# EloDoyard/movie-recommender-system

Hardware: AMD Instinct MI355X
Metric: test-set predictions/sec (kNN k=300, fit+predict+MAE) (higher is better)
Workload: dtype fp16 MFMA similarity filter (fp32 acc) + f64 exact re-rank/prediction

## Files before the change

### movie-recommender-system_amd/csrc/api.cpp

```cpp
#include <math.h>
#include <stdio.h>
#include <string.h>

#include <algorithm>
#include <vector>

#include "engine.h"

using namespace knncf;

namespace knncf {
void launch_first_rows(int64_t n, const int32_t* d_du, const int32_t* d_di, int32_t own_lo, int32_t own_hi,
                       uint32_t* d_first, hipStream_t st);
void launch_length_keys(int32_t count, const int32_t* d_list, const int64_t* d_u_ptr, int32_t max_len, uint64_t* d_key, hipStream_t st);
void launch_collect_new(int32_t U, const uint32_t* d_first, int64_t* d_seq, int64_t epoch, int32_t own_lo, int32_t own_hi,
                        int32_t* d_list, int32_t* d_count, hipStream_t st);
void launch_fallback_keys(int32_t U, const double* d_exact, uint64_t* d_keys, uint32_t* d_vals, hipStream_t st);
void launch_fallback_write(int32_t user, int32_t take, int32_t kcap, const uint32_t* d_sorted_vals,
                           const double* d_exact, int32_t* nbr_idx, double* nbr_sim, int32_t* nbr_cnt,
                           hipStream_t st);
void launch_jaccard_pair(const Train& tr, int32_t u, int32_t v, double* d_out, hipStream_t st);
}

struct StageTimer {
    hipEvent_t a, b;
    double* acc;
};

struct knncf_handle {
    knncf_config cfg{};
    hipStream_t stream = nullptr;
    std::string err;
    Train tr;
    PrepScratch prep;
    bool fitted = false, committed = false;
    int8_t short_rows = -1;
    NeighborTable nt;
    int64_t epoch = 1;
    int64_t U_pad = 0, K_pad = 0;
    DArr<bf16_t> Bpanel;
    bool b_ready = false;
    int32_t head = 0;
    double tail_pairs_full = 0.0;
    DArr<int32_t> colmap;
    DArr<int32_t> te_cnt, te_item;
    DArr<float> te_x, row_tail_abs, row_head_sq;
    DArr<float> row_len;
    hipStream_t stream2 = nullptr;
    DArr<bf16_t> Apanel[2];
    DArr<float> S[2];
    DArr<float> S_full;
    DArr<uint32_t> sym_tiles;
    DArr<int32_t> redo_rows;
    int32_t sym_tiles_n = 0;
    hipEvent_t ev_produced[2] = {nullptr, nullptr}, ev_consumed[2] = {nullptr, nullptr}, ev_ready = nullptr;
    int32_t* pinned_cnt = nullptr;
    size_t pinned_cap = 0;
    SelectScratch sel;
    SliceScratch slices;
    NeighborTable pt;
    bool pt_ready = false;
    PersonalRows prow;
    bool prow_ready = false;
    DArr<int32_t> reco_users, reco_items, reco_out_items;
    DArr<double> reco_pred, reco_out_preds;
    DArr<uint8_t> reco_rated;
    QueryBatchScratch query_batch;
    RecoBatchScratch reco_batch;
    DArr<int32_t> build_list, build_count;
    DArr<uint32_t> first_row;
    DArr<int32_t> t_du, t_di, t_users, t_items;
    DArr<double> t_pred, t_err, t_ratings, t_partial, scalar_out;
    DArr<unsigned long long> scalar_u64;
    DArr<uint8_t> t_owned;
    DArr<int64_t> t_counts;
    DArr<int32_t> sweep_ks;
    std::vector<uint32_t> h_ukeys, h_ikeys;
    std::vector<int32_t> h_uid;
    std::vector<int64_t> h_uptr;
    knncf_timings tm{};
    std::vector<StageTimer> pending;
    std::vector<hipEvent_t> event_pool;
};

namespace {

hipEvent_t get_event(knncf_handle* h) {
    if (!h->event_pool.empty()) {
        hipEvent_t e = h->event_pool.back();
        h->event_pool.pop_back();
        return e;
    }
    hipEvent_t e;
    KN_HIP(hipEventCreate(&e));
    return e;
}

struct Stage {
    knncf_handle* h;
    StageTimer t;
    hipStream_t st;
    Stage(knncf_handle* h_, double* acc, hipStream_t st_ = nullptr) : h(h_), st(st_ ? st_ : h_->stream) {
        t.a = get_event(h);
        t.b = get_event(h);
        t.acc = acc;
        (void)hipEventRecord(t.a, st);
    }
    ~Stage() {
        (void)hipEventRecord(t.b, st);
        h->pending.push_back(t);
    }
};

void resolve_timers(knncf_handle* h) {
    (void)hipStreamSynchronize(h->stream);
    (void)hipStreamSynchronize(h->stream2);
    for (auto& t : h->pending) {
        float ms = 0.f;
        if (hipEventElapsedTime(&ms, t.a, t.b) == hipSuccess) *t.acc += ms;
        h->event_pool.push_back(t.a);
        h->event_pool.push_back(t.b);
    }
    h->pending.clear();
}

template <class F>
int guarded(knncf_handle* h, F&& f) {
    if (!h) return KNNCF_E_INVALID;
    struct DeviceGuard {
        int prev = -1;
        ~DeviceGuard() { if (prev >= 0) (void)hipSetDevice(prev); }
    } guard;
    try {
        int cur = -1;
        if (hipGetDevice(&cur) != hipSuccess) {
            (void)hipGetLastError();
            KN_HIP(hipSetDevice(h->cfg.device));
        } else if (cur != h->cfg.device) {
            guard.prev = cur;
            KN_HIP(hipSetDevice(h->cfg.device));
        }
        f();
        resolve_timers(h);
        return KNNCF_OK;
    } catch (const Error& e) {
        h->err = e.what();
        (void)hipStreamSynchronize(h->stream);
        (void)hipStreamSynchronize(h->stream2);
        (void)hipGetLastError();
        h->pending.clear();
        return e.status;
    } catch (const std::bad_alloc&) {
        h->err = "host allocation failed";
        return KNNCF_E_NOMEM;
    } catch (const std::exception& e) {
        h->err = e.what();
        return KNNCF_E_INVALID;
    }
}

void require_fitted(knncf_handle* h, bool committed = true) {
    KN_REQUIRE(h->fitted, KNNCF_E_STATE, "call knncf_fit first");
    if (committed) KN_REQUIRE(h->committed, KNNCF_E_STATE, "sharded handle: call knncf_shard_commit after the exchange");
}

void load_host_ids(knncf_handle* h) {
    if (!h->h_ukeys.empty() || h->tr.U == 0) return;
    Train& tr = h->tr;
    h->h_ukeys.resize(tr.U);
    h->h_ikeys.resize(tr.I);
    h->h_uid.resize(tr.U);
    KN_HIP(hipMemcpyAsync(h->h_ukeys.data(), tr.ukeys.p, tr.U * sizeof(uint32_t), hipMemcpyDeviceToHost, h->stream));
    KN_HIP(hipMemcpyAsync(h->h_ikeys.data(), tr.ikeys.p, tr.I * sizeof(uint32_t), hipMemcpyDeviceToHost, h->stream));
    KN_HIP(hipMemcpyAsync(h->h_uid.data(), tr.uid.p, tr.U * sizeof(int32_t), hipMemcpyDeviceToHost, h->stream));
    KN_HIP(hipStreamSynchronize(h->stream));
}

int32_t dense_user(knncf_handle* h, int32_t raw) {
    load_host_ids(h);
    return dense_lookup(h->h_ukeys.data(), h->tr.U, raw);
}
int64_t train_row_length(knncf_handle* h, int32_t du) {
    if (h->h_uptr.empty()) {
        h->h_uptr.resize((size_t)h->tr.U + 1);
        KN_HIP(hipMemcpyAsync(h->h_uptr.data(), h->tr.u_ptr.p, h->h_uptr.size() * sizeof(int64_t), hipMemcpyDeviceToHost, h->stream));
        KN_HIP(hipStreamSynchronize(h->stream));
    }
    return h->h_uptr[du + 1] - h->h_uptr[du];
}
int32_t dense_item(knncf_handle* h, int32_t raw) {
    load_host_ids(h);
    return dense_lookup(h->h_ikeys.data(), h->tr.I, raw);
}

void require_shard_numbering(knncf_handle* h) {
    if (h->cfg.shard_count == 1) return;
    if (h->short_rows < 0) {
        Train& tr = h->tr;
        std::vector<int64_t> ptr((size_t)tr.U + 1);
        KN_HIP(hipMemcpyAsync(ptr.data(), tr.u_ptr.p, ptr.size() * sizeof(int64_t), hipMemcpyDeviceToHost, h->stream));
        KN_HIP(hipStreamSynchronize(h->stream));
        h->short_rows = 0;
        for (int32_t u = 0; u < tr.U; ++u)
            if (ptr[u + 1] - ptr[u] <= 4) { h->short_rows = 1; break; }
    }
    KN_REQUIRE(h->short_rows == 0, KNNCF_E_UNSUPPORTED,
               "neighbours: on a shard handle whose train set has a user with <= 4 ratings, a neighbourhood that knncf_mae / "
               "knncf_predict_batch has not built yet cannot be built by a query (its build number would exist on this shard only)");
}

template <class T>
T fetch(knncf_handle* h, const T* d, int64_t idx) {
    T v;
    KN_HIP(hipMemcpyAsync(&v, d + idx, sizeof(T), hipMemcpyDeviceToHost, h->stream));
    KN_HIP(hipStreamSynchronize(h->stream));
    return v;
}

void reset_neighbors(knncf_handle* h) {
    Train& tr = h->tr;
    NeighborTable& nt = h->nt;
    nt.k = h->cfg.k;
    nt.kcap = std::max(0, std::min(nt.k, tr.U - 1));
    size_t cells = (size_t)tr.U * (size_t)std::max(nt.kcap, 1);
    nt.idx.ensure(cells);
    nt.sim.ensure(cells);
    nt.by_id_valid = false;
    nt.cnt.ensure(tr.U);
    nt.seq.ensure(tr.U);
    KN_HIP(hipMemsetAsync(nt.cnt.p, 0, tr.U * sizeof(int32_t), h->stream));
    KN_HIP(hipMemsetAsync(nt.seq.p, 0xff, tr.U * sizeof(int64_t), h->stream));
    h->epoch = 1;
}

float gemm_eps_operand(bool fp16) {
    const double u = ldexp(1.0, fp16 ? -11 : -8) * 1.001;
    return (float)(2 * u + u * u);
}
float gemm_eps_rest(bool fp16) {
    return (float)(4e-7 + (fp16 ? 6e-6 : 0.0) + 8e-6);
}

int32_t shortlist_cap(int32_t k, int32_t U) {
    int64_t want = std::max<int64_t>(16384, 4 * (int64_t)k);
    int64_t cap = 64;
    while (cap < want) cap <<= 1;
    int64_t upper = 64;
    while (upper < U) upper <<= 1;
    return (int32_t)std::min(cap, upper);
}

int32_t choose_head(knncf_handle* h, int32_t rows_total, bool symmetric) {
    Train& tr = h->tr;
    const int32_t I = tr.I;
    const std::vector<int64_t>& c = tr.pop_count;
    std::vector<double> tail_sq((size_t)I + 1, 0.0);
    for (int32_t j = I - 1; j >= 0; --j) tail_sq[j] = tail_sq[j + 1] + (double)c[j] * (double)c[j];
    int32_t H;
    if (h->cfg.head_items == KNNCF_HEAD_ALL) {
        H = I;
    } else if (h->cfg.head_items > 0) {
        H = (int32_t)std::min<int64_t>(h->cfg.head_items, I);
    } else {
        const double RATE_DENSE = symmetric ? 2.8e15 : 1.2e15;
        const double RATE_SPARSE = 2.3e12;
        const double frac = (double)rows_total / (double)tr.U;
        const double U_pad = (double)round_up(tr.U, 256);
        double best = 1e300;
        H = I;
        for (int64_t cand = 64;; cand += 64) {
            int32_t hc = (int32_t)std::min<int64_t>(cand, I);
            double cost = 2.0 * rows_total * U_pad * (double)round_up(hc, 64) / RATE_DENSE + tail_sq[hc] * frac / RATE_SPARSE;
            if (cost < best) { best = cost; H = hc; }
            if (hc == I) break;
        }
        if (tr.jaccard && (h->cfg.flags & KNNCF_FLAG_F32_PANEL) == 0) H = std::min(H, 2048);
    }
    h->tail_pairs_full = tail_sq[H];
    return H;
}

void build_neighbors(knncf_handle* h, int32_t count) {
    Train& tr = h->tr;
    NeighborTable& nt = h->nt;
    if (count <= 0 || nt.kcap <= 0) return;
    KN_REQUIRE(h->cfg.similarity != KNNCF_SIM_ONE, KNNCF_E_UNSUPPORTED,
               "kNN neighbourhoods with similarityOne: every similarity is 1.0, the neighbourhood is the first k users in Set order — not built");
    hipStream_t st = h->stream;
    if (count > 256) {
        PrepScratch& sc = h->prep;
        sc.k64_a.ensure(count); sc.k64_b.ensure(count); sc.v32_b.ensure(count);
        launch_length_keys(count, h->build_list.p, tr.u_ptr.p, tr.I, sc.k64_a.p, st);
        sort_pairs_u64_u32(sc.sort, sc.k64_a.p, sc.k64_b.p, reinterpret_cast<const uint32_t*>(h->build_list.p), sc.v32_b.p, count, bits_for((uint64_t)tr.I), st);
        KN_HIP(hipMemcpyAsync(h->build_list.p, sc.v32_b.p, (size_t)count * sizeof(int32_t), hipMemcpyDeviceToDevice, st));
    }
    const bool fp16 = (h->cfg.flags & KNNCF_FLAG_BF16_FILTER) == 0;
    const bool s_fp16 = (h->cfg.flags & KNNCF_FLAG_F32_PANEL) == 0;
    h->U_pad = round_up(tr.U, 256);
    const int64_t U_pad = h->U_pad;
    size_t free_b = 0, total_b = 0;
    KN_HIP(hipMemGetInfo(&free_b, &total_b));
    const int64_t s_elem = s_fp16 ? 2 : 4;
    const size_t sym_bytes = (size_t)U_pad * (size_t)U_pad * (size_t)s_elem;
    size_t own = h->S_full.bytes() + h->sel.cand_idx.bytes() + h->sel.cand_approx.bytes() + h->sel.grp_v0.bytes() + h->sel.grp_x.bytes();
    for (int s = 0; s < 2; ++s) own += h->S[s].bytes() + h->Apanel[s].bytes();
    bool use_sym = h->cfg.shard_count == 1 && (int64_t)count * 2 >= tr.U && U_pad / 256 < 65536 &&
                   sym_bytes <= (free_b + own) / 3 && !getenv("KNNCF_DEBUG_NO_SYMMETRIC_GEMM");
    if (use_sym) {
        try {
            h->S_full.ensure((sym_bytes + 3) / 4);
        } catch (const Error& e) {
            if (e.status != KNNCF_E_NOMEM) throw;
            (void)hipGetLastError();
            use_sym = false;
        }
    }
    if (!h->b_ready) {
        h->head = choose_head(h, count, use_sym);
        h->K_pad = round_up(h->head, 64);
        size_t need = (size_t)U_pad * h->K_pad * sizeof(bf16_t);
        KN_REQUIRE(need < free_b + h->Bpanel.bytes(), KNNCF_E_UNSUPPORTED,
                   "dense bf16 user panel does not fit in HBM; lower head_items");
        Stage s(h, &h->tm.densify_ms);
        h->colmap.ensure(tr.I);
        launch_colmap(tr, h->head, h->colmap.p, st);
        h->Bpanel.ensure((size_t)U_pad * h->K_pad);
        launch_densify(tr, nullptr, 0, tr.U, h->colmap.p, h->Bpanel.p, h->K_pad, U_pad, fp16, st);
        if (tr.jaccard) {
            KN_REQUIRE(!s_fp16 || h->head <= 2048, KNNCF_E_UNSUPPORTED, "Jaccard: more than 2048 dense head items need KNNCF_FLAG_F32_PANEL");
            h->row_len.ensure((size_t)row_len_size(tr.U));
            launch_row_len(tr, h->row_len.p, st);
        }
        if (h->head < tr.I) {
            h->te_cnt.ensure(tr.U); h->te_item.ensure(tr.n); h->te_x.ensure(tr.n);
            h->row_tail_abs.ensure(tr.U); h->row_head_sq.ensure(tr.U);
            launch_tail_entries(tr, h->colmap.p, h->te_cnt.p, h->te_item.p, h->te_x.p, h->row_tail_abs.p, h->row_head_sq.p, st);
        }
        h->b_ready = true;
        KN_HIP(hipMemGetInfo(&free_b, &total_b));
    }
    const int64_t K_pad = h->K_pad;
    const int32_t head = h->head;
    h->tm.head_items = head;
    if (use_sym) {
        const int32_t n_tiles = (int32_t)(U_pad / 256);
        if (h->sym_tiles_n != n_tiles) {
            std::vector<uint32_t> list;
            gemm_sym_tile_list(n_tiles, list);
            h->sym_tiles.ensure(list.size());
            KN_HIP(hipMemcpyAsync(h->sym_tiles.p, list.data(), list.size() * sizeof(uint32_t), hipMemcpyHostToDevice, st));
            KN_HIP(hipStreamSynchronize(st));
            h->sym_tiles_n = n_tiles;
        }
        const int64_t n_listed = (int64_t)n_tiles * (n_tiles + 1) / 2;
        Stage s(h, &h->tm.gemm_ms);
        launch_gemm_sym(h->Bpanel.p, h->S_full.p, s_fp16, U_pad, h->K_pad, h->K_pad, U_pad, fp16, !tr.jaccard, h->sym_tiles.p, n_listed, st);
        h->tm.gemm_launches += 1;
        h->tm.gemm_flops_executed += 2.0 * 256.0 * 256.0 * (double)n_listed * (double)h->K_pad;
        h->tm.gemm_flops_algorithmic += 2.0 * (double)count * (double)(tr.U - 1) * (double)h->head;
        KN_HIP(hipMemGetInfo(&free_b, &total_b));
    } else {
        h->S_full.release();
    }
    size_t held = 0;
    for (int s = 0; s < 2; ++s) held += h->S[s].bytes() + h->Apanel[s].bytes();
    held += h->sel.cand_idx.bytes() + h->sel.cand_approx.bytes() + h->sel.grp_v0.bytes() + h->sel.grp_x.bytes();
    int64_t budget = h->cfg.workspace_bytes > 0 ? h->cfg.workspace_bytes / 2
                                                : (int64_t)std::min<size_t>((size_t)48 << 30, (free_b + held) / 4);
    int64_t per_row = (use_sym ? 0 : U_pad * s_elem + K_pad * 2) + (int64_t)shortlist_cap(nt.k, tr.U) * 8 + (int64_t)select_gcap(nt.k) * 36;
    if (h->cfg.workspace_bytes <= 0) {
        const int64_t whole = round_up(count, 256) * per_row;
        if (whole <= (int64_t)std::min<size_t>((size_t)96 << 30, (free_b + held) / 3)) budget = std::max(budget, whole);
    }
    int64_t R = std::max<int64_t>(256, (budget / per_row) / 256 * 256);
    R = std::min<int64_t>(R, round_up(count, 256));
    const int64_t n_blocks = ceil_div(count, R);
    R = round_up(ceil_div(count, n_blocks), 256);
    const bool overlap = (h->cfg.flags & KNNCF_FLAG_OVERLAP) != 0;
    const int slots = (overlap && n_blocks > 1 && !use_sym) ? 2 : 1;
    for (int s = 0; s < slots && !use_sym; ++s) {
        h->S[s].ensure((size_t)(R * U_pad * s_elem + 3) / 4);
        h->Apanel[s].ensure((size_t)R * K_pad);
    }
    const int32_t cap = shortlist_cap(nt.k, tr.U);
    const bool verify = (h->cfg.flags & KNNCF_FLAG_VERIFY_BOUND) != 0;
    h->sel.cand_idx.ensure((size_t)R * cap);
    h->sel.cand_approx.ensure((size_t)R * cap);
    h->sel.cand_cnt.ensure(R);
    h->sel.cand_eps.ensure(R);
    h->sel.row_entries.ensure(R);
    h->sel.grp_v0.ensure((size_t)R * select_gcap(nt.k));
    h->sel.grp_x.ensure((size_t)R * select_gcap(nt.k) * 8);
    h->sel.stats.ensure(4);
    KN_HIP(hipMemsetAsync(h->sel.stats.p, 0, 4 * sizeof(double), st));
    if (h->pinned_cap < (size_t)count) {
        if (h->pinned_cnt) KN_HIP(hipHostFree(h->pinned_cnt));
        h->pinned_cnt = nullptr;
        h->pinned_cap = 0;
        KN_HIP(hipHostMalloc((void**)&h->pinned_cnt, (size_t)count * sizeof(int32_t), hipHostMallocDefault));
        h->pinned_cap = (size_t)count;
    }
    const float eps_opnd = gemm_eps_operand(fp16);
    const float eps_rest = gemm_eps_rest(fp16) + (s_fp16 ? 2.45e-4f : 0.f);
    hipStream_t sp = slots > 1 ? h->stream2 : h->stream;
    hipStream_t sc = h->stream;
    KN_HIP(hipEventRecord(h->ev_ready, sc));
    KN_HIP(hipStreamWaitEvent(sp, h->ev_ready, 0));
    std::vector<int32_t> h_rows;
    auto need_h_rows = [&] {
        if (!h_rows.empty()) return;
        h_rows.resize(count);
        KN_HIP(hipMemcpyAsync(h_rows.data(), h->build_list.p, (size_t)count * sizeof(int32_t), hipMemcpyDeviceToHost, st));
        KN_HIP(hipStreamSynchronize(st));
    };
    auto redo_marked = [&](const std::vector<int32_t>& marked, const void* Sp, bool by_user, int64_t rb) {
        need_h_rows();
        std::vector<int32_t> users(marked.size()), srow(marked.size());
        for (size_t j = 0; j < marked.size(); ++j) {
            users[j] = h_rows[marked[j]];
            srow[j] = (int32_t)(marked[j] - rb);
        }
        TailEntries te{h->te_cnt.p, h->te_item.p, h->te_x.p, h->row_tail_abs.p, h->row_head_sq.p, h->row_len.p};
        const int64_t chunk = std::min<int64_t>((int64_t)marked.size(), R);
        h->redo_rows.ensure(2 * (size_t)chunk);
        for (size_t j0 = 0; j0 < marked.size(); j0 += (size_t)R) {
            const int32_t m = (int32_t)std::min<size_t>((size_t)R, marked.size() - j0);
            KN_HIP(hipMemcpyAsync(h->redo_rows.p, users.data() + j0, (size_t)m * sizeof(int32_t), hipMemcpyHostToDevice, st));
            KN_HIP(hipMemcpyAsync(h->redo_rows.p + chunk, srow.data() + j0, (size_t)m * sizeof(int32_t), hipMemcpyHostToDevice, st));
            {
                Stage s(h, &h->tm.select_ms);
                launch_tail_select(tr, h->colmap.p, te, head < tr.I, Sp, by_user, s_fp16, U_pad, m, h->redo_rows.p, nt.k, eps_opnd, eps_rest, cap,
                                   h->sel.cand_idx.p, h->sel.cand_approx.p, h->sel.cand_cnt.p, h->sel.cand_eps.p, h->sel.grp_v0.p, h->sel.grp_x.p,
                                   select_gcap(nt.k), st, false, by_user ? nullptr : h->redo_rows.p + chunk);
                h->tm.select_launches += 1;
            }
            {
                Stage s(h, &h->tm.rerank_ms);
                launch_rerank(tr, nt, m, h->redo_rows.p, cap, h->sel.cand_idx.p, h->sel.cand_approx.p, h->sel.cand_cnt.p, h->sel.cand_eps.p,
                              h->sel.stats.p, h->sel.row_entries.p, verify, st);
            }
            std::vector<int32_t> again(m);
            KN_HIP(hipMemcpyAsync(again.data(), h->sel.cand_cnt.p, (size_t)m * sizeof(int32_t), hipMemcpyDeviceToHost, st));
            KN_HIP(hipStreamSynchronize(st));
            for (int32_t j = 0; j < m; ++j) h->pinned_cnt[marked[j0 + j]] = again[j];
        }
    };
    const bool per_block_redo = !use_sym && n_blocks > 1;
    for (int64_t b = 0; b < n_blocks; ++b) {
        const int64_t rb = b * R;
        const int32_t rows = (int32_t)std::min<int64_t>(R, count - rb);
        const int64_t M = round_up(rows, 256);
        const int32_t* d_rows = h->build_list.p + rb;
        const int slot = (int)(b % slots);
        if (b >= slots) KN_HIP(hipStreamWaitEvent(sp, h->ev_consumed[slot], 0));
        if (!use_sym) {
            Stage s(h, &h->tm.densify_ms, sp);
            launch_densify(tr, d_rows, 0, rows, h->colmap.p, h->Apanel[slot].p, K_pad, M, fp16, sp);
        }
        if (!use_sym) {
            Stage s(h, &h->tm.gemm_ms, sp);
            launch_gemm_nt(h->Apanel[slot].p, h->Bpanel.p, h->S[slot].p, s_fp16, M, U_pad, K_pad, K_pad, K_pad, U_pad, fp16, !tr.jaccard, sp);
            h->tm.gemm_launches += 1;
            h->tm.gemm_flops_executed += 2.0 * (double)M * (double)U_pad * (double)K_pad;
            h->tm.gemm_flops_algorithmic += 2.0 * (double)rows * (double)(tr.U - 1) * (double)head;
        }
        KN_HIP(hipEventRecord(h->ev_produced[slot], sp));
        KN_HIP(hipStreamWaitEvent(sc, h->ev_produced[slot], 0));
        TailEntries te{h->te_cnt.p, h->te_item.p, h->te_x.p, h->row_tail_abs.p, h->row_head_sq.p, h->row_len.p};
        h->prep.join_commit(sc);
        const void* Sblk = use_sym ? (const void*)h->S_full.p : (const void*)h->S[slot].p;
        const int32_t gcap = select_gcap(nt.k);
        auto select_rows = [&](int32_t r0, int32_t nr) {
            Stage s(h, &h->tm.select_ms, sc);
            const void* Sp = use_sym ? Sblk : (const void*)(static_cast<const char*>(Sblk) + (size_t)r0 * (size_t)U_pad * (size_t)s_elem);
            launch_tail_select(tr, h->colmap.p, te, head < tr.I, Sp, use_sym, s_fp16, U_pad, nr, d_rows + r0, nt.k, eps_opnd, eps_rest, cap,
                               h->sel.cand_idx.p + (size_t)r0 * cap, h->sel.cand_approx.p + (size_t)r0 * cap, h->sel.cand_cnt.p + r0, h->sel.cand_eps.p + r0,
                               h->sel.grp_v0.p + (size_t)r0 * gcap, h->sel.grp_x.p + (size_t)r0 * gcap * 8, gcap, sc);
            h->tm.select_launches += 1;
            h->tm.tail_pair_updates += h->tail_pairs_full * ((double)nr / (double)tr.U);
            h->tm.select_row_bytes += (double)s_elem * (double)nr * (double)tr.U;
        };
        const int32_t slices = std::min<int32_t>(8, 8192 / std::max<int32_t>(nt.kcap, 1));
        const char* force_slices = getenv("KNNCF_DEBUG_SLICE_ROWS");
        const int32_t n_heavy = slices < 2                         ? 0
                                : force_slices                     ? std::max<int32_t>(0, std::min<int32_t>(rows, atoi(force_slices)))
                                : (rows >= 4096 && rows <= 65536)  ? std::max<int32_t>(16, rows / 512)
                                                                   : 0;
        select_rows(0, rows);
        if (overlap && !per_block_redo) KN_HIP(hipEventRecord(h->ev_consumed[slot], sc));
        {
            Stage s(h, &h->tm.rerank_ms, sc);
            launch_rerank(tr, nt, rows, d_rows, cap, h->sel.cand_idx.p, h->sel.cand_approx.p, h->sel.cand_cnt.p, h->sel.cand_eps.p, h->sel.stats.p,
                          h->sel.row_entries.p, verify, sc, n_heavy, slices, &h->slices);
        }
        if (!overlap) KN_HIP(hipEventRecord(h->ev_consumed[slot], sc));
        if (per_block_redo) KN_HIP(hipMemcpyAsync(h->pinned_cnt + rb, h->sel.cand_cnt.p, rows * sizeof(int32_t), hipMemcpyDeviceToHost, sc));
        if (per_block_redo) {
            KN_HIP(hipStreamSynchronize(sc));
            std::vector<int32_t> marked;
            for (int64_t r = rb; r < rb + rows; ++r)
                if (h->pinned_cnt[r] > cap) marked.push_back((int32_t)r);
            if ((int64_t)marked.size() > std::max<int64_t>(64, rows / 200)) {
                redo_marked(marked, h->S[slot].p, false, rb);
            }
            if (overlap) KN_HIP(hipEventRecord(h->ev_consumed[slot], sc));
        }
    }
    const bool summary = !per_block_redo;
    unsigned long long four[4] = {0, 0, 0, 0};
    nt.by_id_valid = false;
    if (summary) KN_HIP(hipMemcpyAsync(four, h->sel.stats.p, sizeof(four), hipMemcpyDeviceToHost, sc));
    KN_HIP(hipStreamSynchronize(sc));
    KN_HIP(hipStreamSynchronize(sp));
    auto take_stats = [&](const unsigned long long* w) {
        h->tm.rerank_row_bytes += 12.0 * (double)w[1];
        if (verify && w[0] != 0) {
            double shifted;
            memcpy(&shifted, &w[0], sizeof(double));
            h->tm.max_bound_violation = std::max(h->tm.max_bound_violation, shifted - 4.0);
        }
    };
    if (summary && four[3] == 0) {
        h->tm.shortlist_total += (double)four[2];
        take_stats(four);
        return;
    }
    if (summary) {
        KN_HIP(hipMemcpyAsync(h->pinned_cnt, h->sel.cand_cnt.p, (size_t)count * sizeof(int32_t), hipMemcpyDeviceToHost, st));
        KN_HIP(hipStreamSynchronize(st));
    }
    if (summary) {
        std::vector<int32_t> marked;
        for (int64_t r = 0; r < count; ++r)
            if (h->pinned_cnt[r] > cap) marked.push_back((int32_t)r);
        if ((int64_t)marked.size() > std::max<int64_t>(64, count / 200)) redo_marked(marked, use_sym ? (const void*)h->S_full.p : (const void*)h->S[0].p, use_sym, 0);
    }
    for (int64_t r = 0; r < count; ++r) {
        h->tm.shortlist_total += std::min(h->pinned_cnt[r], cap);
        if (h->pinned_cnt[r] > cap) {
            need_h_rows();
            Stage s(h, &h->tm.rerank_ms);
            int32_t u = h_rows[r];
            h->sel.row_exact.ensure(tr.U);
            h->sel.fb_keys_a.ensure(tr.U); h->sel.fb_keys_b.ensure(tr.U);
            h->sel.fb_vals_a.ensure(tr.U); h->sel.fb_vals_b.ensure(tr.U);
            int64_t seq_u = fetch(h, nt.seq.p, u);
            launch_exact_row(tr, nt, u, seq_u, h->sel.row_exact.p, st);
            launch_fallback_keys(tr.U, h->sel.row_exact.p, h->sel.fb_keys_a.p, h->sel.fb_vals_a.p, st);
            sort_pairs_u64_u32(h->prep.sort, h->sel.fb_keys_a.p, h->sel.fb_keys_b.p, h->sel.fb_vals_a.p,
                               h->sel.fb_vals_b.p, tr.U, 64, st);
            launch_fallback_write(u, nt.kcap, nt.kcap, h->sel.fb_vals_b.p, h->sel.row_exact.p, nt.idx.p, nt.sim.p,
                                  nt.cnt.p, st);
            h->tm.fallback_rows += 1;
        }
    }
    {
        unsigned long long two[2] = {0, 0};
        KN_HIP(hipMemcpyAsync(two, h->sel.stats.p, sizeof(two), hipMemcpyDeviceToHost, st));
        KN_HIP(hipStreamSynchronize(st));
        take_stats(two);
    }
}

void ensure_test_scratch(knncf_handle* h, int64_t n) {
    h->t_du.ensure(n); h->t_di.ensure(n); h->t_pred.ensure(n); h->t_err.ensure(n); h->t_owned.ensure(n);
    h->t_partial.ensure(1024); h->t_counts.ensure(1024);
}

void ensure_neighbors_for_rows(knncf_handle* h, int64_t n) {
    Train& tr = h->tr;
    if (tr.U < 2 || h->nt.kcap <= 0) return;
    KN_REQUIRE(n < (int64_t)0xffffffffll, KNNCF_E_UNSUPPORTED, "more than 2^32-1 test rows");
    hipStream_t st = h->stream;
    h->first_row.ensure(tr.U);
    h->build_list.ensure(tr.U);
    h->build_count.ensure(1);
    KN_HIP(hipMemsetAsync(h->first_row.p, 0xff, tr.U * sizeof(uint32_t), st));
    KN_HIP(hipMemsetAsync(h->build_count.p, 0, sizeof(int32_t), st));
    launch_first_rows(n, h->t_du.p, h->t_di.p, 0, tr.U, h->first_row.p, st);
    launch_collect_new(tr.U, h->first_row.p, h->nt.seq.p, h->epoch, tr.own_lo, tr.own_hi, h->build_list.p, h->build_count.p, st);
    h->epoch += 1;
    int32_t count = fetch(h, h->build_count.p, 0);
    build_neighbors(h, count);
}

bool personalized_streams(const knncf_handle* h) { return h->tr.U > 2048 || getenv("KNNCF_DEBUG_PERSONALIZED_STREAM"); }

void require_personalized(knncf_handle* h) {
    Train& tr = h->tr;
    KN_REQUIRE(h->cfg.shard_count == 1, KNNCF_E_UNSUPPORTED, "PERSONALIZED is not sharded");
    if (h->cfg.similarity == KNNCF_SIM_COSINE) {
        std::vector<int64_t> ptr((size_t)tr.U + 1);
        KN_HIP(hipMemcpyAsync(ptr.data(), tr.u_ptr.p, ptr.size() * sizeof(int64_t), hipMemcpyDeviceToHost, h->stream));
        KN_HIP(hipStreamSynchronize(h->stream));
        for (int32_t u = 0; u < tr.U; ++u)
            KN_REQUIRE(ptr[u + 1] - ptr[u] > 4, KNNCF_E_UNSUPPORTED,
                       "PERSONALIZED with the adjusted cosine: a user with <= 4 ratings makes the reference's summation order depend on its memo history pair by pair (SURVEY N6); not modelled");
    }
}

void ensure_personalized_table(knncf_handle* h) {
    if (h->pt_ready) return;
    Train& tr = h->tr;
    require_personalized(h);
    NeighborTable& pt = h->pt;
    pt.k = pt.kcap = tr.U;
    const size_t cells = (size_t)tr.U * (size_t)tr.U;
    pt.uidx.ensure(cells);
    pt.usim.ensure(cells);
    pt.cnt.ensure(tr.U);
    launch_full_rows(tr, h->cfg.similarity == KNNCF_SIM_JACCARD, pt.uidx.p, pt.usim.p, pt.cnt.p, h->stream);
    pt.by_id_valid = true;
    h->pt_ready = true;
}

void ensure_personal_rows(knncf_handle* h) {
    if (h->prow_ready) return;
    require_personalized(h);
    Stage s(h, &h->tm.prep_ms);
    h->prep.join_commit(h->stream);
    personalized_prepare(h->tr, h->prep, h->prow, h->stream);
    h->prow_ready = true;
}

void predict_personal_rows(knncf_handle* h, const double* d_ratings, int64_t n, double* d_pred) {
    Train& tr = h->tr;
    PersonalRows& pr = h->prow;
    PrepScratch& sc = h->prep;
    hipStream_t st = h->stream;
    KN_REQUIRE(n < (int64_t)0xffffffffll, KNNCF_E_UNSUPPORTED, "more than 2^32-1 test rows");
    sc.k64_a.ensure(n); sc.k64_b.ensure(n); sc.v32_a.ensure(n); sc.v32_b.ensure(n);
    const int ibits = bits_for((uint64_t)tr.I);
    std::vector<uint64_t> keys((size_t)n);
    {
        Stage s(h, &h->tm.predict_ms);
        launch_personal_row_keys(tr, n, h->t_du.p, h->t_di.p, sc.k64_a.p, sc.v32_a.p, st);
        sort_pairs_u64_u32(sc.sort, sc.k64_a.p, sc.k64_b.p, sc.v32_a.p, sc.v32_b.p, n, ibits + bits_for((uint64_t)tr.U), st);
        KN_HIP(hipMemcpyAsync(keys.data(), sc.k64_b.p, (size_t)n * sizeof(uint64_t), hipMemcpyDeviceToHost, st));
        KN_HIP(hipStreamSynchronize(st));
    }
    std::vector<int32_t> users;
    std::vector<int64_t> first_row;
    for (int64_t r = 0; r < n; ++r) {
        const uint64_t u = keys[r] >> ibits, i = keys[r] & ((1ull << ibits) - 1ull);
        if (u < (uint64_t)tr.U && i < (uint64_t)tr.I && (users.empty() || users.back() != (int32_t)u)) {
            users.push_back((int32_t)u);
            first_row.push_back(r);
        }
    }
    const int64_t nu = (int64_t)users.size();
    int64_t R = 1;
    if (nu > 0) {
        size_t free_b = 0, total_b = 0;
        KN_HIP(hipMemGetInfo(&free_b, &total_b));
        const int64_t row_bytes = (int64_t)tr.U * 8;
        const int64_t budget = h->cfg.workspace_bytes > 0 ? h->cfg.workspace_bytes / 2
                                                          : (int64_t)std::min<size_t>((size_t)48 << 30, (free_b + pr.S.bytes()) / 4);
        R = std::min<int64_t>(std::max<int64_t>(1, budget / row_bytes), nu);
        R = ceil_div(nu, ceil_div(nu, R));
        pr.S.ensure((size_t)R * tr.U);
        std::vector<int32_t> slot((size_t)tr.U, -1);
        for (int64_t k = 0; k < nu; ++k) slot[users[k]] = (int32_t)(k % R);
        pr.users.ensure(nu);
        pr.slot.ensure(tr.U);
        KN_HIP(hipMemcpyAsync(pr.users.p, users.data(), (size_t)nu * sizeof(int32_t), hipMemcpyHostToDevice, st));
        KN_HIP(hipMemcpyAsync(pr.slot.p, slot.data(), (size_t)tr.U * sizeof(int32_t), hipMemcpyHostToDevice, st));
        KN_HIP(hipStreamSynchronize(st));
    }
    const int64_t n_blocks = std::max<int64_t>(1, ceil_div(nu, R));
    for (int64_t b = 0; b < n_blocks; ++b) {
        const int64_t u0 = b * R, u1 = std::min<int64_t>(nu, u0 + R);
        const int64_t r0 = b == 0 ? 0 : first_row[u0], r1 = b + 1 < n_blocks ? first_row[u1] : n;
        if (u1 > u0) {
            Stage s(h, &h->tm.rerank_ms);
            launch_sim_rows(tr, pr, pr.users.p + u0, (int32_t)(u1 - u0), pr.S.p, st);
        }
        Stage s(h, &h->tm.predict_ms);
        launch_fold_rows(tr, pr, r1 - r0, sc.v32_b.p + r0, h->t_du.p, h->t_di.p, d_ratings, pr.slot.p, pr.S.p, d_pred, h->t_err.p,
                         h->t_owned.p, st);
    }
}

void ensure_item_stats(knncf_handle* h) {
    if (h->tr.item_stats_ready) return;
    Stage s(h, &h->tm.prep_ms);
    h->prep.join_commit(h->stream);
    prep_item_stats(h->tr, h->prep, h->stream);
}

int64_t order_test_rows(knncf_handle* h, int64_t n, bool by_item, int32_t cols) {
    Train& tr = h->tr;
    hipStream_t st = h->stream;
    PrepScratch& sc = h->prep;
    sc.k64_a.ensure(n); sc.k64_b.ensure(n); sc.v32_a.ensure(n); sc.v32_b.ensure(n);
    const uint32_t key_limit = (uint32_t)(by_item ? tr.I : tr.U);
    if (h->cfg.shard_count > 1) {
        h->scalar_u64.ensure(1);
        KN_HIP(hipMemsetAsync(h->scalar_u64.p, 0, sizeof(unsigned long long), st));
        KN_HIP(hipMemsetAsync(h->t_err.p, 0, (size_t)cols * (size_t)n * sizeof(double), st));
        KN_HIP(hipMemsetAsync(h->t_owned.p, 0, (size_t)n, st));
        launch_owned_keys(n, by_item ? h->t_di.p : h->t_du.p, h->t_du.p, tr.own_lo, tr.own_hi, h->cfg.shard_rank == 0, key_limit,
                          sc.k64_a.p, sc.v32_a.p, h->scalar_u64.p, st);
        sort_pairs_u64_u32(sc.sort, sc.k64_a.p, sc.k64_b.p, sc.v32_a.p, sc.v32_b.p, n, bits_for((uint64_t)key_limit + 1), st);
        return (int64_t)fetch(h, h->scalar_u64.p, 0);
    }
    launch_user_keys(n, by_item ? h->t_di.p : h->t_du.p, key_limit, sc.k64_a.p, sc.v32_a.p, st);
    sort_pairs_u64_u32(sc.sort, sc.k64_a.p, sc.k64_b.p, sc.v32_a.p, sc.v32_b.p, n, bits_for((uint64_t)key_limit), st);
    return n;
}

void reduce_errors(knncf_handle* h, int64_t n, int32_t cols, double* sums, int64_t* count) {
    hipStream_t st = h->stream;
    const int32_t nb = 1024;
    h->t_partial.ensure((size_t)nb * cols);
    h->t_counts.ensure((size_t)nb * cols);
    for (int32_t c = 0; c < cols; ++c)
        launch_reduce_err(h->t_err.p + (size_t)c * n, h->t_owned.p, n, h->t_partial.p + (size_t)c * nb, h->t_counts.p + (size_t)c * nb, nb, st);
    std::vector<double> hp((size_t)nb * cols);
    std::vector<int64_t> hc((size_t)nb * cols);
    KN_HIP(hipMemcpyAsync(hp.data(), h->t_partial.p, hp.size() * sizeof(double), hipMemcpyDeviceToHost, st));
    KN_HIP(hipMemcpyAsync(hc.data(), h->t_counts.p, hc.size() * sizeof(int64_t), hipMemcpyDeviceToHost, st));
    KN_HIP(hipStreamSynchronize(st));
    for (int32_t c = 0; c < cols; ++c) {
        double s_ = 0.0;
        int64_t c_ = 0;
        for (int32_t b = 0; b < nb; ++b) { s_ += hp[(size_t)c * nb + b]; c_ += hc[(size_t)c * nb + b]; }
        if (sums) sums[c] = s_;
        if (count && c == 0) *count = c_;
    }
}

void run_predict(knncf_handle* h, int predictor, const int32_t* d_users, const int32_t* d_items,
                 const double* d_ratings, int64_t n, double* sum_abs_err, int64_t* count, double* d_pred_out) {
    require_fitted(h);
    Train& tr = h->tr;
    hipStream_t st = h->stream;
    KN_REQUIRE(n >= 0, KNNCF_E_INVALID, "negative row count");
    if (sum_abs_err) *sum_abs_err = 0.0;
    if (count) *count = 0;
    if (n == 0) return;
    KN_REQUIRE(d_users && d_items, KNNCF_E_INVALID, "null test arrays");
    int kind = predictor;
    NeighborTable* table = &h->nt;
    bool stream = false;
    if (predictor == KNNCF_PRED_PERSONALIZED) {
        if (h->cfg.similarity == KNNCF_SIM_ONE) {
            kind = KNNCF_PRED_BASELINE_RDD;
        } else if (personalized_streams(h)) {
            ensure_personal_rows(h);
            stream = true;
        } else {
            ensure_personalized_table(h);
            kind = KNNCF_PRED_KNN;
            table = &h->pt;
        }
    }
    KN_REQUIRE(stream || (kind >= KNNCF_PRED_GLOBAL_AVG && kind <= KNNCF_PRED_KNN), KNNCF_E_INVALID, "unknown predictor");
    if (kind == KNNCF_PRED_ITEM_AVG || kind == KNNCF_PRED_BASELINE || kind == KNNCF_PRED_BASELINE_RDD) ensure_item_stats(h);
    ensure_test_scratch(h, n);
    {
        Stage s(h, &h->tm.predict_ms);
        launch_dense_ids(tr, d_users, d_items, n, h->t_du.p, h->t_di.p, st);
    }
    if (kind == KNNCF_PRED_KNN && table == &h->nt) ensure_neighbors_for_rows(h, n);
    h->prep.join_commit(st);
    double* pred = d_pred_out ? d_pred_out : h->t_pred.p;
    if (stream) predict_personal_rows(h, d_ratings, n, pred);
    {
        Stage s(h, &h->tm.predict_ms);
        const uint32_t* d_order = nullptr;
        const bool by_item = tr.ib_words > 0 && lds_bitmap_fits(tr.ib_words);
        int64_t n_rows = n;
        if (kind == KNNCF_PRED_KNN) {
            n_rows = order_test_rows(h, n, by_item, 1);
            d_order = h->prep.v32_b.p;
        }
        if (n_rows > 0 && !stream)
            launch_predict(tr, table, kind, n_rows, h->t_du.p, h->t_di.p, d_ratings, d_order, by_item, pred, h->t_err.p, h->t_owned.p,
                           h->cfg.shard_rank == 0, st);
        if (sum_abs_err || count) reduce_errors(h, n, 1, sum_abs_err, count);
    }
}

void check_sweep_ks(const int32_t* ks, int32_t n_k) {
    KN_REQUIRE(ks && n_k >= 1 && n_k <= 64, KNNCF_E_INVALID, "sweep: 1 .. 64 values of k");
    for (int32_t q = 0; q < n_k; ++q)
        KN_REQUIRE(ks[q] >= 1 && ks[q] <= 2048 && (q == 0 || ks[q] > ks[q - 1]), KNNCF_E_INVALID,
                   "sweep: k must be strictly ascending in [1, 2048]");
}

void run_mae_sweep(knncf_handle* h, const int32_t* ks, int32_t n_k, const int32_t* d_users, const int32_t* d_items,
                   const double* d_ratings, int64_t n, double* sums, int64_t* count, double* d_pred) {
    check_sweep_ks(ks, n_k);
    require_fitted(h);
    KN_REQUIRE(h->cfg.similarity != KNNCF_SIM_ONE, KNNCF_E_UNSUPPORTED,
               "kNN neighbourhoods with similarityOne: every similarity is 1.0, the neighbourhood is the first k users in Set order — not built");
    KN_REQUIRE(n >= 0, KNNCF_E_INVALID, "negative row count");
    for (int32_t q = 0; q < n_k; ++q) sums[q] = 0.0;
    *count = 0;
    if (n == 0) return;
    KN_REQUIRE(d_users && d_items && d_ratings, KNNCF_E_INVALID, "null test arrays");
    Train& tr = h->tr;
    hipStream_t st = h->stream;
    struct Restore {
        knncf_handle* h;
        int32_t k;
        ~Restore() {
            h->cfg.k = k;
            try { reset_neighbors(h); } catch (const Error&) {}
        }
    } restore{h, h->cfg.k};
    h->cfg.k = ks[n_k - 1];
    reset_neighbors(h);
    ensure_test_scratch(h, n);
    h->t_err.ensure((size_t)n_k * n);
    {
        Stage s(h, &h->tm.predict_ms);
        launch_dense_ids(tr, d_users, d_items, n, h->t_du.p, h->t_di.p, st);
    }
    ensure_neighbors_for_rows(h, n);
    h->prep.join_commit(st);
    std::vector<int32_t> hk(ks, ks + n_k);
    h->sweep_ks.ensure(64);
    KN_HIP(hipMemcpyAsync(h->sweep_ks.p, hk.data(), (size_t)n_k * sizeof(int32_t), hipMemcpyHostToDevice, st));
    {
        Stage s(h, &h->tm.predict_ms);
        const int64_t n_rows = order_test_rows(h, n, true, n_k);
        if (n_rows > 0)
            launch_predict_sweep(tr, h->nt, h->sweep_ks.p, n_k, n_rows, n, h->t_du.p, h->t_di.p, d_ratings, h->prep.v32_b.p, d_pred,
                                 h->t_err.p, h->t_owned.p, h->cfg.shard_rank == 0, st);
        reduce_errors(h, n, n_k, sums, count);
    }
}

void do_fit_device(knncf_handle* h, const int32_t* d_users, const int32_t* d_items, const double* d_ratings, int64_t n) {
    KN_REQUIRE(n > 0 && d_users && d_items && d_ratings, KNNCF_E_INVALID, "fit: null or empty input");
    Train& tr = h->tr;
    hipStream_t st = h->stream;
    h->fitted = h->committed = false;
    h->short_rows = -1;
    h->b_ready = false;
    h->pt_ready = false;
    h->prow_ready = false;
    h->h_ukeys.clear(); h->h_ikeys.clear(); h->h_uid.clear(); h->h_uptr.clear();
    tr.n = n;
    tr.jaccard = h->cfg.similarity == KNNCF_SIM_JACCARD;
    {
        Stage s(h, &h->tm.prep_ms);
        if (tr.user_raw.p != d_users) {
            tr.user_raw.alloc(n); tr.item_raw.alloc(n); tr.rating.alloc(n);
            KN_HIP(hipMemcpyAsync(tr.user_raw.p, d_users, n * sizeof(int32_t), hipMemcpyDeviceToDevice, st));
            KN_HIP(hipMemcpyAsync(tr.item_raw.p, d_items, n * sizeof(int32_t), hipMemcpyDeviceToDevice, st));
            KN_HIP(hipMemcpyAsync(tr.rating.p, d_ratings, n * sizeof(double), hipMemcpyDeviceToDevice, st));
        }
        prep_fit(tr, h->prep, h->cfg.shard_rank, h->cfg.shard_count, st);
    }
    h->fitted = true;
    reset_neighbors(h);
    if (h->cfg.shard_count == 1) {
        Stage s(h, &h->tm.prep_ms);
        prep_commit(tr, h->prep, st);
        h->committed = true;
    }
}

void do_recommend(knncf_handle* h, int predictor, int32_t user, int32_t n, int32_t* out_items, double* out_preds, int32_t* count) {
    require_fitted(h);
    KN_REQUIRE(count && n >= 0 && (n == 0 || (out_items && out_preds)), KNNCF_E_INVALID, "bad arguments");
    *count = 0;
    Train& tr = h->tr;
    if (n == 0 || tr.I == 0) return;
    hipStream_t st = h->stream;
    const int32_t du = dense_user(h, user);
    KN_REQUIRE(du < 0 ? h->cfg.shard_rank == 0 : (du >= tr.own_lo && du < tr.own_hi), KNNCF_E_STATE,
               "recommend: the user belongs to another shard");
    const int32_t I = tr.I;
    h->reco_users.ensure(I); h->reco_items.ensure(I); h->reco_pred.ensure(I); h->reco_rated.ensure(I);
    launch_reco_rows(tr, user, du, h->reco_users.p, h->reco_items.p, h->reco_rated.p, st);
    run_predict(h, predictor, h->reco_users.p, h->reco_items.p, nullptr, I, nullptr, nullptr, h->reco_pred.p);
    PrepScratch& sc = h->prep;
    sc.k64_a.ensure(I); sc.k64_b.ensure(I); sc.v32_a.ensure(I); sc.v32_b.ensure(I);
    launch_reco_order(tr, sc.sort, h->reco_pred.p, h->reco_rated.p, sc.k64_a.p, sc.k64_b.p, sc.v32_a.p, sc.v32_b.p, st);
    int64_t n_rated = 0;
    if (du >= 0) {
        int64_t two[2];
        KN_HIP(hipMemcpyAsync(two, tr.u_ptr.p + du, 2 * sizeof(int64_t), hipMemcpyDeviceToHost, st));
        KN_HIP(hipStreamSynchronize(st));
        n_rated = two[1] - two[0];
    }
    const int32_t m = (int32_t)std::min<int64_t>(n, (int64_t)I - n_rated);
    if (m <= 0) return;
    h->reco_out_items.ensure(m); h->reco_out_preds.ensure(m);
    launch_reco_take(tr, m, sc.v32_b.p, h->reco_pred.p, h->reco_out_items.p, h->reco_out_preds.p, st);
    KN_HIP(hipMemcpyAsync(out_items, h->reco_out_items.p, (size_t)m * sizeof(int32_t), hipMemcpyDeviceToHost, st));
    KN_HIP(hipMemcpyAsync(out_preds, h->reco_out_preds.p, (size_t)m * sizeof(double), hipMemcpyDeviceToHost, st));
    KN_HIP(hipStreamSynchronize(st));
    *count = m;
}

constexpr int64_t QUERY_MAX_RATINGS = 65536;
enum QueryBatchMode { QB_NEIGHBORS, QB_PREDICT, QB_RECOMMEND };
enum QueryFamily { QF_FOLD_IN, QF_UPDATE, QF_REVISE };

void require_query_support(knncf_handle* h, int predictor) {
    KN_REQUIRE(predictor == KNNCF_PRED_KNN, KNNCF_E_UNSUPPORTED, "query: only KNNCF_PRED_KNN");
    KN_REQUIRE(h->cfg.similarity != KNNCF_SIM_ONE, KNNCF_E_UNSUPPORTED, "query: adjusted cosine or Jaccard");
    KN_REQUIRE(h->cfg.shard_count == 1, KNNCF_E_UNSUPPORTED, "query: single-shard handles only");
    KN_REQUIRE(h->tr.U >= 5, KNNCF_E_UNSUPPORTED, "query: fewer than 5 train users (the user set changes iteration class)");
}

int64_t query_batch_chunk(knncf_handle* h) {
    const Train& tr = h->tr;
    int64_t budget = h->cfg.workspace_bytes / 2;
    if (h->cfg.workspace_bytes <= 0) {
        size_t free_b = 0, total_b = 0;
        KN_HIP(hipMemGetInfo(&free_b, &total_b));
        budget = (int64_t)std::min<size_t>((size_t)48 << 30, free_b / 4);
    }
    int64_t C = std::min<int64_t>(QB_MAX_CHUNK, budget / query_batch_bytes(tr.U, tr.I));
    C = std::min<int64_t>(C, (int64_t)0x7fffffff / std::max(tr.U, tr.I));
    return std::max<int64_t>(C, 1);
}

struct QueryFailure {
    int64_t query = -1;
    const char* reason = "";
};

QueryFailure run_query_chunks(knncf_handle* h, QueryFamily family, QueryBatchMode mode, int64_t chunk, const int32_t* users,
                              const int64_t* removed_offsets, const int32_t* removed_items,
                              const int64_t* offsets, const int32_t* items, const double* ratings, int64_t B, int32_t width, const int64_t* pred_offsets,
                              const int32_t* pred_items, int32_t* out_i, double* out_d, int32_t* counts, int32_t* statuses) {
    h->prep.join_commit(h->stream);
    const Train& tr = h->tr;
    QueryBatchScratch& bs = h->query_batch;
    hipStream_t st = h->stream;
    const int32_t take = std::max(0, std::min(h->cfg.k, tr.U));
    QueryFailure first;
    auto fail = [&](int64_t b, int status, const char* why) {
        statuses[b] = status;
        if (counts) counts[b] = 0;
        if (first.query < 0 || b < first.query) first = {b, why};
    };
    const bool update = family != QF_FOLD_IN, revise = family == QF_REVISE;
    std::vector<int64_t> slot_query, qo, ao, ro, ebase;
    std::vector<int32_t> s_users, s_items, s_self, s_removed, h_idx, h_items, pick_slot, pick_items;
    std::vector<double> s_ratings, h_vals;
    std::vector<long long> info;
    for (int64_t c0 = 0; c0 < B; c0 += chunk) {
        const int64_t c1 = std::min(B, c0 + chunk);
        slot_query.clear(); s_users.clear(); s_items.clear(); s_ratings.clear(); s_self.clear(); s_removed.clear();
        qo.assign(1, 0);
        ao.assign(1, 0);
        ro.assign(1, 0);
        for (int64_t b = c0; b < c1; ++b) {
            const int64_t nb = offsets[b + 1] - offsets[b];
            const int64_t nr = revise ? removed_offsets[b + 1] - removed_offsets[b] : 0;
            const int32_t du = dense_user(h, users[b]);
            const int64_t seeded = nb + (update && du >= 0 ? train_row_length(h, du) : 0);
            if (nr > 0 && du < 0) { fail(b, KNNCF_E_INVALID, "a removed item for a user that is not in the training set"); continue; }
            if (nr > seeded - nb) { fail(b, KNNCF_E_INVALID, "more removed items than the user has train rows (one is not rated in train or listed twice)"); continue; }
            const int64_t rows = seeded - nr;
            if (rows <= 0) { fail(b, KNNCF_E_INVALID, nr > 0 ? "the removals leave the user without a row" : "null ratings or n_ratings <= 0"); continue; }
            if (seeded > QUERY_MAX_RATINGS) { fail(b, KNNCF_E_UNSUPPORTED, "more than 65536 ratings"); continue; }
            if (!update && du >= 0) { fail(b, KNNCF_E_INVALID, "the user occurs in the training set"); continue; }
            if (nr > 0) s_removed.insert(s_removed.end(), removed_items + removed_offsets[b], removed_items + removed_offsets[b + 1]);
            ro.push_back((int64_t)s_removed.size());
            slot_query.push_back(b);
            s_users.push_back(users[b]);
            s_self.push_back(du);
            s_items.insert(s_items.end(), items + offsets[b], items + offsets[b + 1]);
            s_ratings.insert(s_ratings.end(), ratings + offsets[b], ratings + offsets[b + 1]);
            ao.push_back((int64_t)s_items.size());
            qo.push_back(qo.back() + rows);
        }
        const int32_t C = (int32_t)slot_query.size();
        if (C == 0) continue;
        info.assign((size_t)4 * C, 0);
        foldin_batch_neighbors(tr, bs, h->prep.sort, C, s_users.data(), qo.data(), s_items.data(), s_ratings.data(),
                               update ? s_self.data() : nullptr, update ? ao.data() : nullptr, h->cfg.k, info.data(), st,
                               revise ? ro.data() : nullptr, revise ? s_removed.data() : nullptr);
        auto take_of = [&](int32_t s) { return update && s_self[s] >= 0 ? std::min(take, tr.U - 1) : take; };
        int32_t good = 0;
        for (int32_t s = 0; s < C; ++s) {
            const uint64_t bits = (uint64_t)info[4 * s];
            const int64_t b = slot_query[s];
            if (bits & QUERY_ST_RM_UNRATED) fail(b, KNNCF_E_INVALID, "a removed item that the user did not rate in train");
            else if (bits & QUERY_ST_RM_TWICE) fail(b, KNNCF_E_INVALID, "a removed item listed twice");
            else if (bits & ST_DUPLICATE) fail(b, KNNCF_E_DUPLICATE, "the ratings repeat an item");
            else if (bits & ST_NONFINITE) fail(b, KNNCF_E_NONFINITE, "scale() == 0 gives a non-finite deviation");
            else if (bits & QUERY_ST_NEG_MEAN) fail(b, KNNCF_E_UNSUPPORTED, "a negative mean rating (the predictor would answer aug's global average)");
            else { statuses[b] = KNNCF_OK; ++good; }
        }
        if (good == 0) continue;
        if (mode == QB_NEIGHBORS) {
            const int32_t c = std::min(take, width);
            if (c > 0) {
                h_idx.resize((size_t)C * take); h_vals.resize((size_t)C * take);
                KN_HIP(hipMemcpyAsync(h_idx.data(), bs.nbr_idx.p, h_idx.size() * sizeof(int32_t), hipMemcpyDeviceToHost, st));
                KN_HIP(hipMemcpyAsync(h_vals.data(), bs.nbr_sim.p, h_vals.size() * sizeof(double), hipMemcpyDeviceToHost, st));
                KN_HIP(hipStreamSynchronize(st));
                load_host_ids(h);
            }
            for (int32_t s = 0; s < C; ++s) {
                const int64_t b = slot_query[s];
                if (statuses[b] != KNNCF_OK) continue;
                for (int32_t j = 0; j < std::min(c, take_of(s)); ++j) {
                    out_i[b * width + j] = h->h_uid[h_idx[(size_t)s * take + j]];
                    out_d[b * width + j] = h_vals[(size_t)s * take + j];
                }
                counts[b] = take_of(s);
            }
            continue;
        }
        ebase.assign((size_t)C + 1, 0);
        for (int32_t s = 0; s < C; ++s) ebase[s + 1] = ebase[s] + info[4 * s + 2];
        if (mode == QB_PREDICT) {
            pick_slot.clear(); pick_items.clear();
            for (int32_t s = 0; s < C; ++s) {
                const int64_t b = slot_query[s];
                if (statuses[b] != KNNCF_OK) continue;
                pick_items.insert(pick_items.end(), pred_items + pred_offsets[b], pred_items + pred_offsets[b + 1]);
                pick_slot.insert(pick_slot.end(), (size_t)(pred_offsets[b + 1] - pred_offsets[b]), s);
            }
            const int64_t m = (int64_t)pick_items.size();
            if (m == 0) continue;
            foldin_batch_predictions(tr, bs, h->prep.sort, C, take, ebase.data(), st);
            bs.pick_items.ensure(m); bs.pick_slot.ensure(m); bs.pick_out.ensure(m);
            KN_HIP(hipMemcpyAsync(bs.pick_items.p, pick_items.data(), (size_t)m * sizeof(int32_t), hipMemcpyHostToDevice, st));
            KN_HIP(hipMemcpyAsync(bs.pick_slot.p, pick_slot.data(), (size_t)m * sizeof(int32_t), hipMemcpyHostToDevice, st));
            foldin_batch_pick(tr, bs, bs.pick_items.p, bs.pick_slot.p, m, bs.pick_out.p, st);
            h_vals.resize((size_t)m);
            KN_HIP(hipMemcpyAsync(h_vals.data(), bs.pick_out.p, (size_t)m * sizeof(double), hipMemcpyDeviceToHost, st));
            KN_HIP(hipStreamSynchronize(st));
            int64_t at = 0;
            for (int32_t s = 0; s < C; ++s) {
                const int64_t b = slot_query[s];
                if (statuses[b] != KNNCF_OK) continue;
                const int64_t mb = pred_offsets[b + 1] - pred_offsets[b];
                std::copy(h_vals.begin() + at, h_vals.begin() + at + mb, out_d + pred_offsets[b]);
                at += mb;
            }
            continue;
        }
        int32_t widest = 0;
        for (int32_t s = 0; s < C; ++s) {
            const int64_t b = slot_query[s];
            if (statuses[b] != KNNCF_OK) continue;
            counts[b] = (int32_t)std::max<int64_t>(0, std::min<int64_t>(width, (int64_t)tr.I - info[4 * s + 1]));
            widest = std::max(widest, counts[b]);
        }
        if (widest == 0) continue;
        foldin_batch_predictions(tr, bs, h->prep.sort, C, take, ebase.data(), st);
        const size_t cells = (size_t)C * widest;
        bs.out_items.ensure(cells); bs.out_preds.ensure(cells);
        foldin_batch_recommend(tr, bs, h->prep.sort, C, widest, bs.out_items.p, bs.out_preds.p, st);
        h_items.resize(cells); h_vals.resize(cells);
        KN_HIP(hipMemcpyAsync(h_items.data(), bs.out_items.p, cells * sizeof(int32_t), hipMemcpyDeviceToHost, st));
        KN_HIP(hipMemcpyAsync(h_vals.data(), bs.out_preds.p, cells * sizeof(double), hipMemcpyDeviceToHost, st));
        KN_HIP(hipStreamSynchronize(st));
        for (int32_t s = 0; s < C; ++s) {
            const int64_t b = slot_query[s];
            if (statuses[b] != KNNCF_OK) continue;
            std::copy(h_items.begin() + (size_t)s * widest, h_items.begin() + (size_t)s * widest + counts[b], out_i + b * width);
            std::copy(h_vals.begin() + (size_t)s * widest, h_vals.begin() + (size_t)s * widest + counts[b], out_d + b * width);
        }
    }
    return first;
}

void do_query_batch(knncf_handle* h, QueryFamily family, QueryBatchMode mode, int predictor, const int32_t* users,
                    const int64_t* removed_offsets, const int32_t* removed_items, const int64_t* offsets, const int32_t* items, const double* ratings, int64_t B, int32_t width, const int64_t* pred_offsets,
                    const int32_t* pred_items, int32_t* out_i, double* out_d, int32_t* counts, int32_t* statuses) {
    require_fitted(h, false);
    KN_REQUIRE(B >= 0, KNNCF_E_INVALID, "query batch: n_queries < 0");
    KN_REQUIRE(mode == QB_PREDICT || width >= 0, KNNCF_E_INVALID, "query batch: cap or n < 0");
    require_query_support(h, predictor);
    if (B == 0) return;
    KN_REQUIRE(users && offsets && statuses && (mode == QB_PREDICT || counts), KNNCF_E_INVALID, "query batch: null argument");
    KN_REQUIRE(offsets[0] == 0, KNNCF_E_INVALID, "query batch: offsets[0] != 0");
    for (int64_t b = 0; b < B; ++b) KN_REQUIRE(offsets[b] <= offsets[b + 1], KNNCF_E_INVALID, "query batch: offsets decrease");
    KN_REQUIRE(offsets[B] < ((int64_t)1 << 31), KNNCF_E_INVALID, "query batch: 2^31 or more ratings in one call");
    KN_REQUIRE(offsets[B] == 0 || (items && ratings), KNNCF_E_INVALID, "query batch: null ratings");
    if (family == QF_REVISE) {
        KN_REQUIRE(removed_offsets && removed_offsets[0] == 0, KNNCF_E_INVALID, "query batch: removed_offsets null or not starting at 0");
        for (int64_t b = 0; b < B; ++b)
            KN_REQUIRE(removed_offsets[b] <= removed_offsets[b + 1], KNNCF_E_INVALID, "query batch: removed_offsets decrease");
        KN_REQUIRE(removed_offsets[B] < ((int64_t)1 << 31), KNNCF_E_INVALID, "query batch: 2^31 or more removed items in one call");
        KN_REQUIRE(removed_offsets[B] == 0 || removed_items, KNNCF_E_INVALID, "query batch: null removed items");
    }
    if (mode == QB_PREDICT) {
        KN_REQUIRE(pred_offsets && pred_offsets[0] == 0, KNNCF_E_INVALID, "query batch: pred_offsets null or not starting at 0");
        for (int64_t b = 0; b < B; ++b)
            KN_REQUIRE(pred_offsets[b] <= pred_offsets[b + 1], KNNCF_E_INVALID, "query batch: pred_offsets decrease");
        KN_REQUIRE(pred_offsets[B] == 0 || (pred_items && out_d), KNNCF_E_INVALID, "query batch: null prediction arguments");
    } else {
        KN_REQUIRE(width == 0 || (out_i && out_d), KNNCF_E_INVALID, "query batch: null output");
    }
    const QueryFailure f = run_query_chunks(h, family, mode, query_batch_chunk(h), users, removed_offsets, removed_items, offsets, items,
                                            ratings, B, width, pred_offsets, pred_items, out_i, out_d, counts, statuses);
    if (f.query >= 0) h->err = "query batch: query " + std::to_string(f.query) + ": " + f.reason;
}

void do_query_single(knncf_handle* h, QueryFamily family, QueryBatchMode mode, int predictor, int32_t user,
                     const int32_t* removed_items, int64_t n_removed, const int32_t* items, const double* ratings, int64_t n_ratings, int32_t width, const int32_t* pred_items, int64_t m, int32_t* out_i,
                     double* out_d, int32_t* count) {
    require_fitted(h, false);
    if (family == QF_REVISE)
        KN_REQUIRE(n_removed >= 0 && (n_removed == 0 || removed_items), KNNCF_E_INVALID, "query: null removed items or n_removed < 0");
    if (family != QF_FOLD_IN) {
        KN_REQUIRE(n_ratings >= 0 && (n_ratings == 0 || (items && ratings)), KNNCF_E_INVALID, "query: null ratings or n_ratings < 0");
    } else {
        KN_REQUIRE(items && ratings && n_ratings > 0, KNNCF_E_INVALID, "query: null ratings or n_ratings <= 0");
    }
    require_query_support(h, predictor);
    const int64_t offsets[2] = {0, n_ratings}, pred_offsets[2] = {0, m}, removed_offsets[2] = {0, family == QF_REVISE ? n_removed : 0};
    int32_t status = KNNCF_OK, c = 0;
    const QueryFailure f = run_query_chunks(h, family, mode, 1, &user, removed_offsets, removed_items, offsets, items, ratings, 1, width, pred_offsets, pred_items,
                                            out_i, out_d, &c, &status);
    if (f.query >= 0) throw Error(status, std::string("query: ") + f.reason);
    if (count) *count = c;
}

struct NbrFileHeader {
    char magic[8];
    int32_t U, kcap, k, similarity;
    int64_t n;
    uint64_t fingerprint;
    int64_t epoch;
};

uint64_t fit_fingerprint(knncf_handle* h) {
    Train& tr = h->tr;
    std::vector<int32_t> uid(tr.U), iid(tr.I), col((size_t)tr.n);
    std::vector<int64_t> ptr((size_t)tr.U + 1);
    std::vector<double> avg(tr.U), rating((size_t)tr.n);
    KN_HIP(hipMemcpyAsync(uid.data(), tr.uid.p, (size_t)tr.U * sizeof(int32_t), hipMemcpyDeviceToHost, h->stream));
    KN_HIP(hipMemcpyAsync(ptr.data(), tr.u_ptr.p, ((size_t)tr.U + 1) * sizeof(int64_t), hipMemcpyDeviceToHost, h->stream));
    KN_HIP(hipMemcpyAsync(avg.data(), tr.user_avg.p, (size_t)tr.U * sizeof(double), hipMemcpyDeviceToHost, h->stream));
    KN_HIP(hipMemcpyAsync(iid.data(), tr.iid.p, (size_t)tr.I * sizeof(int32_t), hipMemcpyDeviceToHost, h->stream));
    KN_HIP(hipMemcpyAsync(col.data(), tr.s_col.p, (size_t)tr.n * sizeof(int32_t), hipMemcpyDeviceToHost, h->stream));
    KN_HIP(hipMemcpyAsync(rating.data(), tr.s_rating.p, (size_t)tr.n * sizeof(double), hipMemcpyDeviceToHost, h->stream));
    KN_HIP(hipStreamSynchronize(h->stream));
    uint64_t x = 1469598103934665603ull;
    auto mix = [&](const void* p, size_t bytes) {
        const unsigned char* c = static_cast<const unsigned char*>(p);
        for (size_t i = 0; i < bytes; ++i) { x ^= c[i]; x *= 1099511628211ull; }
    };
    mix(uid.data(), uid.size() * sizeof(int32_t));
    mix(ptr.data(), ptr.size() * sizeof(int64_t));
    mix(avg.data(), avg.size() * sizeof(double));
    for (size_t p = 0; p < col.size(); ++p) {
        const int32_t item = iid[col[p]];
        mix(&item, sizeof item);
        mix(&rating[p], sizeof(double));
    }
    return x;
}

void do_neighbors_save(knncf_handle* h, const char* path) {
    require_fitted(h);
    KN_REQUIRE(path, KNNCF_E_INVALID, "null path");
    KN_REQUIRE(h->cfg.shard_count == 1, KNNCF_E_UNSUPPORTED, "neighbour checkpoints are written by unsharded handles");
    Train& tr = h->tr;
    NeighborTable& nt = h->nt;
    NbrFileHeader hd{};
    memcpy(hd.magic, "KNNCFNB2", 8);
    hd.U = tr.U; hd.kcap = nt.kcap; hd.k = nt.k; hd.similarity = h->cfg.similarity; hd.n = tr.n;
    hd.fingerprint = fit_fingerprint(h);
    hd.epoch = h->epoch;
    const size_t cells = (size_t)tr.U * (size_t)std::max(nt.kcap, 1);
    std::vector<int32_t> cnt(tr.U), idx(cells);
    std::vector<int64_t> seq(tr.U);
    std::vector<double> sim(cells);
    KN_HIP(hipMemcpyAsync(cnt.data(), nt.cnt.p, cnt.size() * sizeof(int32_t), hipMemcpyDeviceToHost, h->stream));
    KN_HIP(hipMemcpyAsync(seq.data(), nt.seq.p, seq.size() * sizeof(int64_t), hipMemcpyDeviceToHost, h->stream));
    KN_HIP(hipMemcpyAsync(idx.data(), nt.idx.p, idx.size() * sizeof(int32_t), hipMemcpyDeviceToHost, h->stream));
    KN_HIP(hipMemcpyAsync(sim.data(), nt.sim.p, sim.size() * sizeof(double), hipMemcpyDeviceToHost, h->stream));
    KN_HIP(hipStreamSynchronize(h->stream));
    FILE* f = fopen(path, "wb");
    KN_REQUIRE(f, KNNCF_E_INVALID, std::string("cannot create ") + path);
    bool ok = fwrite(&hd, sizeof hd, 1, f) == 1 && fwrite(cnt.data(), sizeof(int32_t), cnt.size(), f) == cnt.size() &&
              fwrite(seq.data(), sizeof(int64_t), seq.size(), f) == seq.size() &&
              fwrite(idx.data(), sizeof(int32_t), idx.size(), f) == idx.size() &&
              fwrite(sim.data(), sizeof(double), sim.size(), f) == sim.size();
    ok = (fclose(f) == 0) && ok;
    KN_REQUIRE(ok, KNNCF_E_INVALID, std::string("short write to ") + path);
}

void do_neighbors_load(knncf_handle* h, const char* path) {
    require_fitted(h);
    KN_REQUIRE(path, KNNCF_E_INVALID, "null path");
    KN_REQUIRE(h->cfg.shard_count == 1, KNNCF_E_UNSUPPORTED, "neighbour checkpoints are read by unsharded handles");
    Train& tr = h->tr;
    NeighborTable& nt = h->nt;
    FILE* f = fopen(path, "rb");
    KN_REQUIRE(f, KNNCF_E_INVALID, std::string("cannot open ") + path);
    NbrFileHeader hd{};
    bool ok = fread(&hd, sizeof hd, 1, f) == 1 && memcmp(hd.magic, "KNNCFNB2", 8) == 0;
    if (!ok) {
        const bool v1 = memcmp(hd.magic, "KNNCFNB1", 8) == 0;
        fclose(f);
        throw Error(KNNCF_E_INVALID, std::string(path) + (v1 ? ": neighbour checkpoint of the older format (its fingerprint does not cover the ratings): rebuild it"
                                                               : ": not a neighbour checkpoint"));
    }
    if (hd.U != tr.U || hd.kcap != nt.kcap || hd.k != nt.k || hd.similarity != h->cfg.similarity || hd.n != tr.n ||
        hd.fingerprint != fit_fingerprint(h)) {
        fclose(f);
        throw Error(KNNCF_E_STATE, std::string(path) + ": checkpoint of a different fit (users, ratings, k or similarity differ)");
    }
    const size_t cells = (size_t)tr.U * (size_t)std::max(nt.kcap, 1);
    std::vector<int32_t> cnt(tr.U), idx(cells);
    std::vector<int64_t> seq(tr.U);
    std::vector<double> sim(cells);
    ok = fread(cnt.data(), sizeof(int32_t), cnt.size(), f) == cnt.size() && fread(seq.data(), sizeof(int64_t), seq.size(), f) == seq.size() &&
         fread(idx.data(), sizeof(int32_t), idx.size(), f) == idx.size() && fread(sim.data(), sizeof(double), sim.size(), f) == sim.size();
    fclose(f);
    KN_REQUIRE(ok, KNNCF_E_INVALID, std::string(path) + ": truncated checkpoint");
    hipStream_t st = h->stream;
    KN_HIP(hipMemcpyAsync(nt.cnt.p, cnt.data(), cnt.size() * sizeof(int32_t), hipMemcpyHostToDevice, st));
    KN_HIP(hipMemcpyAsync(nt.seq.p, seq.data(), seq.size() * sizeof(int64_t), hipMemcpyHostToDevice, st));
    KN_HIP(hipMemcpyAsync(nt.idx.p, idx.data(), idx.size() * sizeof(int32_t), hipMemcpyHostToDevice, st));
    KN_HIP(hipMemcpyAsync(nt.sim.p, sim.data(), sim.size() * sizeof(double), hipMemcpyHostToDevice, st));
    nt.by_id_valid = false;
    KN_HIP(hipStreamSynchronize(st));
    h->epoch = std::max<int64_t>(hd.epoch, 1);
}

}

extern "C" {

const char* knncf_version(void) { return "knncf 0.1 (gfx950)"; }

const char* knncf_status_string(int st) {
    switch (st) {
        case KNNCF_OK: return "ok";
        case KNNCF_E_INVALID: return "invalid argument";
        case KNNCF_E_NONFINITE: return "non-finite normalized deviation";
        case KNNCF_E_DUPLICATE: return "duplicate (user,item) rating";
        case KNNCF_E_NOMEM: return "out of memory";
        case KNNCF_E_HIP: return "HIP runtime error";
        case KNNCF_E_STATE: return "invalid call order";
        case KNNCF_E_UNSUPPORTED: return "unsupported configuration";
        case KNNCF_E_NODEVICE: return "no usable gfx950 device";
        case KNNCF_E_RCCL: return "RCCL error";
        default: return "unknown status";
    }
}

int knncf_create(const knncf_config* cfg, knncf_handle** out) {
    if (!cfg || !out || cfg->struct_size != sizeof(knncf_config)) return KNNCF_E_INVALID;
    if (cfg->shard_count < 1 || cfg->shard_rank < 0 || cfg->shard_rank >= cfg->shard_count || cfg->k < 0)
        return KNNCF_E_INVALID;
    if (cfg->similarity < KNNCF_SIM_COSINE || cfg->similarity > KNNCF_SIM_JACCARD) return KNNCF_E_INVALID;
    int ndev = 0;
    if (hipGetDeviceCount(&ndev) != hipSuccess || ndev <= 0 || cfg->device < 0 || cfg->device >= ndev) {
        (void)hipGetLastError();
        return KNNCF_E_NODEVICE;
    }
    hipDeviceProp_t prop;
    if (hipGetDeviceProperties(&prop, cfg->device) != hipSuccess) return KNNCF_E_NODEVICE;
    if (strncmp(prop.gcnArchName, "gfx950", 6) != 0) return KNNCF_E_NODEVICE;
    knncf_handle* h = new (std::nothrow) knncf_handle();
    if (!h) return KNNCF_E_NOMEM;
    h->cfg = *cfg;
    if (hipSetDevice(cfg->device) != hipSuccess || hipStreamCreateWithFlags(&h->stream, hipStreamNonBlocking) != hipSuccess ||
        hipStreamCreateWithFlags(&h->stream2, hipStreamNonBlocking) != hipSuccess) {
        delete h;
        return KNNCF_E_HIP;
    }
    bool ok = hipEventCreateWithFlags(&h->ev_ready, hipEventDisableTiming) == hipSuccess;
    for (int s = 0; s < 2; ++s) {
        ok = ok && hipEventCreateWithFlags(&h->ev_produced[s], hipEventDisableTiming) == hipSuccess;
        ok = ok && hipEventCreateWithFlags(&h->ev_consumed[s], hipEventDisableTiming) == hipSuccess;
    }
    if (!ok) {
        knncf_destroy(h);
        return KNNCF_E_HIP;
    }
    *out = h;
    return KNNCF_OK;
}

void knncf_destroy(knncf_handle* h) {
    if (!h) return;
    (void)hipSetDevice(h->cfg.device);
    (void)hipStreamSynchronize(h->stream);
    for (auto& t : h->pending) { (void)hipEventDestroy(t.a); (void)hipEventDestroy(t.b); }
    for (auto e : h->event_pool) (void)hipEventDestroy(e);
    if (h->stream2) (void)hipStreamSynchronize(h->stream2);
    if (h->ev_ready) (void)hipEventDestroy(h->ev_ready);
    for (int s = 0; s < 2; ++s) {
        if (h->ev_produced[s]) (void)hipEventDestroy(h->ev_produced[s]);
        if (h->ev_consumed[s]) (void)hipEventDestroy(h->ev_consumed[s]);
    }
    if (h->pinned_cnt) (void)hipHostFree(h->pinned_cnt);
    if (h->stream2) (void)hipStreamDestroy(h->stream2);
    (void)hipStreamDestroy(h->stream);
    delete h;
}

const char* knncf_last_error(const knncf_handle* h) { return h ? h->err.c_str() : "null handle"; }

int knncf_fit_device(knncf_handle* h, const int32_t* d_users, const int32_t* d_items, const double* d_ratings, int64_t n) {
    return guarded(h, [&] { do_fit_device(h, d_users, d_items, d_ratings, n); });
}

int knncf_fit(knncf_handle* h, const int32_t* users, const int32_t* items, const double* ratings, int64_t n) {
    return guarded(h, [&] {
        KN_REQUIRE(n > 0 && users && items && ratings, KNNCF_E_INVALID, "fit: null or empty input");
        Train& tr = h->tr;
        tr.user_raw.alloc(n); tr.item_raw.alloc(n); tr.rating.alloc(n);
        KN_HIP(hipMemcpyAsync(tr.user_raw.p, users, n * sizeof(int32_t), hipMemcpyHostToDevice, h->stream));
        KN_HIP(hipMemcpyAsync(tr.item_raw.p, items, n * sizeof(int32_t), hipMemcpyHostToDevice, h->stream));
        KN_HIP(hipMemcpyAsync(tr.rating.p, ratings, n * sizeof(double), hipMemcpyHostToDevice, h->stream));
        do_fit_device(h, tr.user_raw.p, tr.item_raw.p, tr.rating.p, n);
    });
}

int knncf_num_users(const knncf_handle* h, int32_t* out) {
    if (!h || !out || !h->fitted) return KNNCF_E_STATE;
    *out = h->tr.U;
    return KNNCF_OK;
}
int knncf_num_items(const knncf_handle* h, int32_t* out) {
    if (!h || !out || !h->fitted) return KNNCF_E_STATE;
    *out = h->tr.I;
    return KNNCF_OK;
}

int knncf_global_avg(knncf_handle* h, double* out) {
    return guarded(h, [&] {
        require_fitted(h, false);
        KN_REQUIRE(out, KNNCF_E_INVALID, "null out");
        *out = h->tr.global_avg;
    });
}

int knncf_user_avg(knncf_handle* h, int32_t user, double* out) {
    return guarded(h, [&] {
        require_fitted(h);
        KN_REQUIRE(out, KNNCF_E_INVALID, "null out");
        int32_t d = dense_user(h, user);
        *out = d >= 0 ? fetch(h, h->tr.user_avg.p, d) : h->tr.global_avg;
    });
}

int knncf_item_avg(knncf_handle* h, int32_t item, double* out) {
    return guarded(h, [&] {
        require_fitted(h);
        KN_REQUIRE(out, KNNCF_E_INVALID, "null out");
        ensure_item_stats(h);
        int32_t d = dense_item(h, item);
        *out = d >= 0 ? fetch(h, h->tr.item_avg.p, d) : h->tr.global_avg;
    });
}

int knncf_item_avg_dev(knncf_handle* h, int32_t item, double* out) {
    return guarded(h, [&] {
        require_fitted(h);
        KN_REQUIRE(out, KNNCF_E_INVALID, "null out");
        ensure_item_stats(h);
        int32_t d = dense_item(h, item);
        *out = d >= 0 ? fetch(h, h->tr.item_dev_hash.p, d) : 0.0;
    });
}

int knncf_item_avg_dev_rdd(knncf_handle* h, int32_t item, double* out) {
    return guarded(h, [&] {
        require_fitted(h);
        KN_REQUIRE(out, KNNCF_E_INVALID, "null out");
        ensure_item_stats(h);
        int32_t d = dense_item(h, item);
        *out = d >= 0 ? fetch(h, h->tr.item_dev_file.p, d) : 0.0;
    });
}

int knncf_similarity(knncf_handle* h, int32_t u, int32_t v, double* out) {
    return guarded(h, [&] {
        require_fitted(h);
        KN_REQUIRE(out, KNNCF_E_INVALID, "null out");
        if (h->cfg.similarity == KNNCF_SIM_ONE) { *out = 1.0; return; }
        int32_t du = dense_user(h, u), dv = dense_user(h, v);
        h->scalar_out.ensure(1);
        if (h->cfg.similarity == KNNCF_SIM_JACCARD) {
            launch_jaccard_pair(h->tr, du, dv, h->scalar_out.p, h->stream);
        } else {
            if (du < 0 || dv < 0) { *out = 0.0; return; }
            launch_exact_pair(h->tr, du, dv, h->scalar_out.p, h->stream);
        }
        *out = fetch(h, h->scalar_out.p, 0);
    });
}

static void neighbors_of(knncf_handle* h, int32_t du, std::vector<int32_t>& ids, std::vector<double>& sims) {
    NeighborTable& nt = h->nt;
    Train& tr = h->tr;
    ids.clear(); sims.clear();
    if (tr.U < 2 || nt.kcap <= 0) return;
    int64_t seq = fetch(h, nt.seq.p, du);
    if (seq < 0) {
        require_shard_numbering(h);
        h->build_list.ensure(tr.U);
        int64_t new_seq = h->epoch << 32;
        h->epoch += 1;
        KN_HIP(hipMemcpyAsync(nt.seq.p + du, &new_seq, sizeof(int64_t), hipMemcpyHostToDevice, h->stream));
        KN_HIP(hipMemcpyAsync(h->build_list.p, &du, sizeof(int32_t), hipMemcpyHostToDevice, h->stream));
        KN_HIP(hipStreamSynchronize(h->stream));
        build_neighbors(h, 1);
    }
    int32_t cnt = fetch(h, nt.cnt.p, du);
    ids.resize(cnt); sims.resize(cnt);
    if (cnt > 0) {
        KN_HIP(hipMemcpyAsync(ids.data(), nt.idx.p + (int64_t)du * nt.kcap, cnt * sizeof(int32_t), hipMemcpyDeviceToHost, h->stream));
        KN_HIP(hipMemcpyAsync(sims.data(), nt.sim.p + (int64_t)du * nt.kcap, cnt * sizeof(double), hipMemcpyDeviceToHost, h->stream));
        KN_HIP(hipStreamSynchronize(h->stream));
    }
}

int knncf_neighbors(knncf_handle* h, int32_t u, int32_t cap, int32_t* ids, double* sims, int32_t* count) {
    return guarded(h, [&] {
        require_fitted(h);
        KN_REQUIRE(count && cap >= 0 && (cap == 0 || (ids && sims)), KNNCF_E_INVALID, "bad output arguments");
        KN_REQUIRE(h->cfg.similarity != KNNCF_SIM_ONE, KNNCF_E_UNSUPPORTED, "neighbourhoods: adjusted cosine or Jaccard");
        int32_t du = dense_user(h, u);
        load_host_ids(h);
        if (du < 0) {
            int32_t c = std::min(h->nt.k, h->tr.U);
            for (int32_t j = 0; j < c && j < cap; ++j) { ids[j] = h->h_uid[j]; sims[j] = 0.0; }
            *count = c;
            return;
        }
        KN_REQUIRE(du >= h->tr.own_lo && du < h->tr.own_hi, KNNCF_E_INVALID, "user belongs to another shard");
        std::vector<int32_t> di;
        std::vector<double> ds;
        neighbors_of(h, du, di, ds);
        for (size_t j = 0; j < di.size() && (int32_t)j < cap; ++j) { ids[j] = h->h_uid[di[j]]; sims[j] = ds[j]; }
        *count = (int32_t)di.size();
    });
}

static void build_missing_neighbors(knncf_handle* h, const std::vector<int32_t>& du) {
    Train& tr = h->tr;
    NeighborTable& nt = h->nt;
    hipStream_t st = h->stream;
    if (tr.U < 2 || nt.kcap <= 0) return;
    const int64_t n = (int64_t)du.size();
    std::vector<int64_t> seq((size_t)tr.U);
    KN_HIP(hipMemcpyAsync(seq.data(), nt.seq.p, seq.size() * sizeof(int64_t), hipMemcpyDeviceToHost, st));
    KN_HIP(hipStreamSynchronize(st));
    std::vector<int32_t> fresh;
    for (int64_t j = 0; j < n; ++j)
        if (du[j] >= 0 && seq[du[j]] < 0) {
            seq[du[j]] = (h->epoch << 32) | (int64_t)std::min<int64_t>(j, 0xffffffffll);
            fresh.push_back(du[j]);
        }
    if (fresh.empty()) return;
    require_shard_numbering(h);
    h->epoch += 1;
    h->build_list.ensure(tr.U);
    KN_HIP(hipMemcpyAsync(nt.seq.p, seq.data(), seq.size() * sizeof(int64_t), hipMemcpyHostToDevice, st));
    KN_HIP(hipMemcpyAsync(h->build_list.p, fresh.data(), fresh.size() * sizeof(int32_t), hipMemcpyHostToDevice, st));
    KN_HIP(hipStreamSynchronize(st));
    build_neighbors(h, (int32_t)fresh.size());
}

static void do_neighbors_batch(knncf_handle* h, const int32_t* users, int64_t n, int32_t cap, int32_t* ids, double* sims, int32_t* counts) {
    require_fitted(h);
    KN_REQUIRE(n >= 0 && cap >= 0 && (n == 0 || (users && counts)) && (n == 0 || cap == 0 || (ids && sims)), KNNCF_E_INVALID, "bad arguments");
    KN_REQUIRE(h->cfg.similarity != KNNCF_SIM_ONE, KNNCF_E_UNSUPPORTED, "neighbourhoods: adjusted cosine or Jaccard");
    if (n == 0) return;
    Train& tr = h->tr;
    NeighborTable& nt = h->nt;
    hipStream_t st = h->stream;
    load_host_ids(h);
    std::vector<int32_t> du((size_t)n);
    for (int64_t j = 0; j < n; ++j) {
        du[j] = dense_lookup(h->h_ukeys.data(), tr.U, users[j]);
        KN_REQUIRE(du[j] < 0 || (du[j] >= tr.own_lo && du[j] < tr.own_hi), KNNCF_E_INVALID, "user belongs to another shard");
    }
    const bool have_lists = tr.U >= 2 && nt.kcap > 0;
    build_missing_neighbors(h, du);
    const size_t kc = (size_t)std::max(nt.kcap, 1);
    std::vector<int32_t> h_cnt, h_idx;
    std::vector<double> h_sim;
    const bool whole = have_lists && n > 1024;
    if (have_lists) {
        h_cnt.resize(tr.U);
        KN_HIP(hipMemcpyAsync(h_cnt.data(), nt.cnt.p, h_cnt.size() * sizeof(int32_t), hipMemcpyDeviceToHost, st));
        if (whole) {
            h_idx.resize((size_t)tr.U * kc);
            h_sim.resize((size_t)tr.U * kc);
            KN_HIP(hipMemcpyAsync(h_idx.data(), nt.idx.p, h_idx.size() * sizeof(int32_t), hipMemcpyDeviceToHost, st));
            KN_HIP(hipMemcpyAsync(h_sim.data(), nt.sim.p, h_sim.size() * sizeof(double), hipMemcpyDeviceToHost, st));
        }
        KN_HIP(hipStreamSynchronize(st));
    }
    std::vector<int32_t> row_idx(kc);
    std::vector<double> row_sim(kc);
    for (int64_t j = 0; j < n; ++j) {
        int32_t* oi = ids + (size_t)j * cap;
        double* os = sims + (size_t)j * cap;
        if (du[j] < 0) {
            const int32_t c = std::min(nt.k, tr.U);
            for (int32_t q = 0; q < c && q < cap; ++q) { oi[q] = h->h_uid[q]; os[q] = 0.0; }
            counts[j] = c;
            continue;
        }
        const int32_t c = have_lists ? h_cnt[du[j]] : 0;
        const int32_t* src_i = nullptr;
        const double* src_s = nullptr;
        if (whole) {
            src_i = h_idx.data() + (size_t)du[j] * kc;
            src_s = h_sim.data() + (size_t)du[j] * kc;
        } else if (c > 0) {
            KN_HIP(hipMemcpyAsync(row_idx.data(), nt.idx.p + (size_t)du[j] * kc, c * sizeof(int32_t), hipMemcpyDeviceToHost, st));
            KN_HIP(hipMemcpyAsync(row_sim.data(), nt.sim.p + (size_t)du[j] * kc, c * sizeof(double), hipMemcpyDeviceToHost, st));
            KN_HIP(hipStreamSynchronize(st));
            src_i = row_idx.data();
            src_s = row_sim.data();
        }
        for (int32_t q = 0; q < c && q < cap; ++q) { oi[q] = h->h_uid[src_i[q]]; os[q] = src_s[q]; }
        counts[j] = c;
    }
}

int knncf_neighbors_batch(knncf_handle* h, const int32_t* users, int64_t n, int32_t cap, int32_t* ids, double* sims, int32_t* counts) {
    return guarded(h, [&] { do_neighbors_batch(h, users, n, cap, ids, sims, counts); });
}

static int64_t recommend_batch_chunk(knncf_handle* h) {
    int64_t budget = h->cfg.workspace_bytes / 2;
    if (h->cfg.workspace_bytes <= 0) {
        size_t free_b = 0, total_b = 0;
        KN_HIP(hipMemGetInfo(&free_b, &total_b));
        budget = (int64_t)std::min<size_t>((size_t)48 << 30, free_b / 4);
    }
    int64_t C = std::min<int64_t>(RB_MAX_CHUNK, budget / reco_batch_bytes(h->tr.I));
    C = std::min<int64_t>(C, (int64_t)0x7fffffff / h->tr.I);
    return std::max<int64_t>(C, 1);
}

static void do_recommend_batch(knncf_handle* h, int predictor, const int32_t* users, int64_t B, int32_t n, int32_t* out_items,
                               double* out_preds, int32_t* counts) {
    require_fitted(h);
    KN_REQUIRE(B >= 0 && n >= 0, KNNCF_E_INVALID, "recommend batch: n_users or n < 0");
    if (B == 0) return;
    KN_REQUIRE(users && counts && (n == 0 || (out_items && out_preds)), KNNCF_E_INVALID, "recommend batch: null argument");
    if (n == 0) {
        std::fill(counts, counts + B, 0);
        return;
    }
    KN_REQUIRE(predictor >= KNNCF_PRED_GLOBAL_AVG && predictor <= KNNCF_PRED_PERSONALIZED, KNNCF_E_INVALID, "unknown predictor");
    Train& tr = h->tr;
    NeighborTable& nt = h->nt;
    hipStream_t st = h->stream;
    const int32_t I = tr.I;
    load_host_ids(h);
    std::vector<int32_t> du((size_t)B);
    bool any_known = false;
    for (int64_t b = 0; b < B; ++b) {
        du[b] = dense_lookup(h->h_ukeys.data(), tr.U, users[b]);
        KN_REQUIRE(du[b] < 0 ? h->cfg.shard_rank == 0 : (du[b] >= tr.own_lo && du[b] < tr.own_hi), KNNCF_E_STATE,
                   "recommend batch: a user belongs to another shard");
        any_known = any_known || du[b] >= 0;
    }
    const bool knn = predictor == KNNCF_PRED_KNN;
    if (knn && any_known && tr.U >= 2 && nt.kcap > 0) {
        KN_REQUIRE(h->cfg.similarity != KNNCF_SIM_ONE, KNNCF_E_UNSUPPORTED,
                   "kNN neighbourhoods with similarityOne: every similarity is 1.0, the neighbourhood is the first k users in Set order — not built");
        build_missing_neighbors(h, du);
    }
    const bool fold = knn && h->cfg.similarity != KNNCF_SIM_ONE && nt.kcap <= RB_MAX_K && tr.n < (int64_t)0xffffffffll;
    const bool fast_select = n <= RB_FAST_N;
    const int32_t width = (int32_t)std::min<int64_t>(n, I);
    QueryBatchScratch& bs = h->query_batch;
    RecoBatchScratch& rb = h->reco_batch;
    h->prep.join_commit(st);
    const int64_t chunk = recommend_batch_chunk(h);
    if (fast_select) {
        Stage s(h, &h->tm.predict_ms);
        reco_batch_id_rank(tr, bs, rb, h->prep.sort, st);
    }
    std::vector<int32_t> h_items, h_counts;
    std::vector<double> h_preds;
    for (int64_t c0 = 0; c0 < B; c0 += chunk) {
        const int32_t C = (int32_t)std::min<int64_t>(chunk, B - c0);
        const size_t cells = (size_t)C * (size_t)I;
        rb.slot_user.ensure(C); rb.slot_raw.ensure(C); rb.counts.ensure(C);
        bs.pred.ensure(cells); bs.rated.ensure(cells); bs.info.ensure((size_t)4 * C);
        bs.out_items.ensure((size_t)C * width); bs.out_preds.ensure((size_t)C * width);
        KN_HIP(hipMemcpyAsync(rb.slot_user.p, du.data() + c0, (size_t)C * sizeof(int32_t), hipMemcpyHostToDevice, st));
        KN_HIP(hipMemcpyAsync(rb.slot_raw.p, users + c0, (size_t)C * sizeof(int32_t), hipMemcpyHostToDevice, st));
        if (fold) {
            Stage s(h, &h->tm.predict_ms);
            reco_batch_fold(tr, nt, rb, C, bs.pred.p, st);
        } else {
            rb.row_users.ensure(cells); rb.row_items.ensure(cells);
            reco_batch_rows(tr, rb, C, rb.row_users.p, rb.row_items.p, st);
            const int64_t epoch = h->epoch;
            run_predict(h, predictor, rb.row_users.p, rb.row_items.p, nullptr, (int64_t)cells, nullptr, nullptr, bs.pred.p);
            if (knn) h->epoch = epoch;
        }
        {
            Stage s(h, &h->tm.predict_ms);
            reco_batch_mark(tr, rb, C, n, bs.rated.p, (long long*)bs.info.p, st);
            if (fast_select) {
                reco_batch_select(tr, rb, C, width, bs.pred.p, bs.rated.p, bs.out_items.p, bs.out_preds.p, st);
            } else {
                bs.k64_a.ensure(cells); bs.k64_b.ensure(cells); bs.v32_a.ensure(cells); bs.v32_b.ensure(cells);
                bs.s32_a.ensure(cells); bs.s32_b.ensure(cells);
                foldin_batch_recommend(tr, bs, h->prep.sort, C, width, bs.out_items.p, bs.out_preds.p, st);
            }
        }
        h_items.resize((size_t)C * width); h_preds.resize((size_t)C * width); h_counts.resize(C);
        KN_HIP(hipMemcpyAsync(h_items.data(), bs.out_items.p, h_items.size() * sizeof(int32_t), hipMemcpyDeviceToHost, st));
        KN_HIP(hipMemcpyAsync(h_preds.data(), bs.out_preds.p, h_preds.size() * sizeof(double), hipMemcpyDeviceToHost, st));
        KN_HIP(hipMemcpyAsync(h_counts.data(), rb.counts.p, (size_t)C * sizeof(int32_t), hipMemcpyDeviceToHost, st));
        KN_HIP(hipStreamSynchronize(st));
        for (int32_t s = 0; s < C; ++s) {
            const int64_t b = c0 + s;
            const int32_t m = h_counts[s];
            std::copy(h_items.begin() + (size_t)s * width, h_items.begin() + (size_t)s * width + m, out_items + b * n);
            std::copy(h_preds.begin() + (size_t)s * width, h_preds.begin() + (size_t)s * width + m, out_preds + b * n);
            counts[b] = m;
        }
    }
}

int knncf_recommend_batch(knncf_handle* h, int predictor, const int32_t* users, int64_t n_users, int32_t n, int32_t* out_items,
                          double* out_preds, int32_t* counts) {
    return guarded(h, [&] { do_recommend_batch(h, predictor, users, n_users, n, out_items, out_preds, counts); });
}

int knncf_knn_similarity(knncf_handle* h, int32_t u, int32_t v, double* out) {
    return guarded(h, [&] {
        require_fitted(h);
        KN_REQUIRE(out, KNNCF_E_INVALID, "null out");
        KN_REQUIRE(h->cfg.similarity != KNNCF_SIM_ONE, KNNCF_E_UNSUPPORTED, "neighbourhoods: adjusted cosine or Jaccard");
        int32_t du = dense_user(h, u), dv = dense_user(h, v);
        *out = 0.0;
        if (du < 0 || dv < 0) return;
        KN_REQUIRE(du >= h->tr.own_lo && du < h->tr.own_hi, KNNCF_E_INVALID, "user belongs to another shard");
        std::vector<int32_t> di;
        std::vector<double> ds;
        neighbors_of(h, du, di, ds);
        for (size_t j = 0; j < di.size(); ++j)
            if (di[j] == dv) { *out = 0.0 + ds[j]; break; }
    });
}

int knncf_predict_batch_device(knncf_handle* h, int predictor, const int32_t* d_users, const int32_t* d_items,
                               int64_t n, double* d_out) {
    return guarded(h, [&] {
        KN_REQUIRE(d_out || n == 0, KNNCF_E_INVALID, "null output");
        run_predict(h, predictor, d_users, d_items, nullptr, n, nullptr, nullptr, d_out);
    });
}

int knncf_predict_batch(knncf_handle* h, int predictor, const int32_t* users, const int32_t* items, int64_t n, double* out) {
    return guarded(h, [&] {
        KN_REQUIRE(n >= 0 && (n == 0 || (users && items && out)), KNNCF_E_INVALID, "bad arguments");
        if (n == 0) return;
        h->t_users.ensure(n); h->t_items.ensure(n); h->t_pred.ensure(n);
        KN_HIP(hipMemcpyAsync(h->t_users.p, users, n * sizeof(int32_t), hipMemcpyHostToDevice, h->stream));
        KN_HIP(hipMemcpyAsync(h->t_items.p, items, n * sizeof(int32_t), hipMemcpyHostToDevice, h->stream));
        run_predict(h, predictor, h->t_users.p, h->t_items.p, nullptr, n, nullptr, nullptr, nullptr);
        KN_HIP(hipMemcpyAsync(out, h->t_pred.p, n * sizeof(double), hipMemcpyDeviceToHost, h->stream));
        KN_HIP(hipStreamSynchronize(h->stream));
    });
}

int knncf_predict(knncf_handle* h, int predictor, int32_t user, int32_t item, double* out) {
    return knncf_predict_batch(h, predictor, &user, &item, 1, out);
}

int knncf_recommend(knncf_handle* h, int predictor, int32_t user, int32_t n, int32_t* items, double* predictions, int32_t* count) {
    return guarded(h, [&] { do_recommend(h, predictor, user, n, items, predictions, count); });
}

int knncf_query_neighbors(knncf_handle* h, int32_t user, const int32_t* items, const double* ratings, int64_t n_ratings,
                          int32_t cap, int32_t* ids, double* sims, int32_t* count) {
    return guarded(h, [&] {
        KN_REQUIRE(count && cap >= 0 && (cap == 0 || (ids && sims)), KNNCF_E_INVALID, "bad output arguments");
        do_query_single(h, QF_FOLD_IN, QB_NEIGHBORS, KNNCF_PRED_KNN, user, nullptr, 0, items, ratings, n_ratings, cap, nullptr, 0, ids, sims, count);
    });
}

int knncf_query_predict(knncf_handle* h, int predictor, int32_t user, const int32_t* items, const double* ratings,
                        int64_t n_ratings, const int32_t* pred_items, int64_t m, double* out) {
    return guarded(h, [&] {
        KN_REQUIRE(m >= 0 && (m == 0 || (pred_items && out)), KNNCF_E_INVALID, "bad prediction arguments");
        do_query_single(h, QF_FOLD_IN, QB_PREDICT, predictor, user, nullptr, 0, items, ratings, n_ratings, 0, pred_items, m, nullptr, out, nullptr);
    });
}

int knncf_query_neighbors_batch(knncf_handle* h, const int32_t* users, const int64_t* offsets, const int32_t* items,
                                const double* ratings, int64_t n_queries, int32_t cap, int32_t* ids, double* sims, int32_t* counts,
                                int32_t* statuses) {
    return guarded(h, [&] {
        do_query_batch(h, QF_FOLD_IN, QB_NEIGHBORS, KNNCF_PRED_KNN, users, nullptr, nullptr, offsets, items, ratings, n_queries, cap, nullptr, nullptr, ids, sims,
                       counts, statuses);
    });
}

int knncf_query_predict_batch(knncf_handle* h, int predictor, const int32_t* users, const int64_t* offsets, const int32_t* items,
                              const double* ratings, int64_t n_queries, const int64_t* pred_offsets, const int32_t* pred_items,
                              double* out, int32_t* statuses) {
    return guarded(h, [&] {
        do_query_batch(h, QF_FOLD_IN, QB_PREDICT, predictor, users, nullptr, nullptr, offsets, items, ratings, n_queries, 0, pred_offsets, pred_items, nullptr, out,
                       nullptr, statuses);
    });
}

int knncf_query_recommend_batch(knncf_handle* h, int predictor, const int32_t* users, const int64_t* offsets, const int32_t* items,
                                const double* ratings, int64_t n_queries, int32_t n, int32_t* out_items, double* out_preds,
                                int32_t* counts, int32_t* statuses) {
    return guarded(h, [&] {
        do_query_batch(h, QF_FOLD_IN, QB_RECOMMEND, predictor, users, nullptr, nullptr, offsets, items, ratings, n_queries, n, nullptr, nullptr, out_items,
                       out_preds, counts, statuses);
    });
}

int knncf_query_recommend(knncf_handle* h, int predictor, int32_t user, const int32_t* items, const double* ratings,
                          int64_t n_ratings, int32_t n, int32_t* out_items, double* out_preds, int32_t* count) {
    return guarded(h, [&] {
        KN_REQUIRE(count && n >= 0 && (n == 0 || (out_items && out_preds)), KNNCF_E_INVALID, "bad arguments");
        *count = 0;
        do_query_single(h, QF_FOLD_IN, QB_RECOMMEND, predictor, user, nullptr, 0, items, ratings, n_ratings, n, nullptr, 0, out_items, out_preds, count);
    });
}

int knncf_update_neighbors(knncf_handle* h, int32_t user, const int32_t* items, const double* ratings, int64_t n_ratings,
                           int32_t cap, int32_t* ids, double* sims, int32_t* count) {
    return guarded(h, [&] {
        KN_REQUIRE(count && cap >= 0 && (cap == 0 || (ids && sims)), KNNCF_E_INVALID, "bad output arguments");
        do_query_single(h, QF_UPDATE, QB_NEIGHBORS, KNNCF_PRED_KNN, user, nullptr, 0, items, ratings, n_ratings, cap, nullptr, 0, ids, sims, count);
    });
}

int knncf_update_predict(knncf_handle* h, int predictor, int32_t user, const int32_t* items, const double* ratings,
                         int64_t n_ratings, const int32_t* pred_items, int64_t m, double* out) {
    return guarded(h, [&] {
        KN_REQUIRE(m >= 0 && (m == 0 || (pred_items && out)), KNNCF_E_INVALID, "bad prediction arguments");
        do_query_single(h, QF_UPDATE, QB_PREDICT, predictor, user, nullptr, 0, items, ratings, n_ratings, 0, pred_items, m, nullptr, out, nullptr);
    });
}

int knncf_update_neighbors_batch(knncf_handle* h, const int32_t* users, const int64_t* offsets, const int32_t* items,
                                 const double* ratings, int64_t n_queries, int32_t cap, int32_t* ids, double* sims, int32_t* counts,
                                 int32_t* statuses) {
    return guarded(h, [&] {
        do_query_batch(h, QF_UPDATE, QB_NEIGHBORS, KNNCF_PRED_KNN, users, nullptr, nullptr, offsets, items, ratings, n_queries, cap, nullptr, nullptr, ids, sims,
                       counts, statuses);
    });
}

int knncf_update_predict_batch(knncf_handle* h, int predictor, const int32_t* users, const int64_t* offsets, const int32_t* items,
                               const double* ratings, int64_t n_queries, const int64_t* pred_offsets, const int32_t* pred_items,
                               double* out, int32_t* statuses) {
    return guarded(h, [&] {
        do_query_batch(h, QF_UPDATE, QB_PREDICT, predictor, users, nullptr, nullptr, offsets, items, ratings, n_queries, 0, pred_offsets, pred_items, nullptr, out,
                       nullptr, statuses);
    });
}

int knncf_update_recommend_batch(knncf_handle* h, int predictor, const int32_t* users, const int64_t* offsets, const int32_t* items,
                                 const double* ratings, int64_t n_queries, int32_t n, int32_t* out_items, double* out_preds,
                                 int32_t* counts, int32_t* statuses) {
    return guarded(h, [&] {
        do_query_batch(h, QF_UPDATE, QB_RECOMMEND, predictor, users, nullptr, nullptr, offsets, items, ratings, n_queries, n, nullptr, nullptr, out_items,
                       out_preds, counts, statuses);
    });
}

int knncf_update_recommend(knncf_handle* h, int predictor, int32_t user, const int32_t* items, const double* ratings,
                           int64_t n_ratings, int32_t n, int32_t* out_items, double* out_preds, int32_t* count) {
    return guarded(h, [&] {
        KN_REQUIRE(count && n >= 0 && (n == 0 || (out_items && out_preds)), KNNCF_E_INVALID, "bad arguments");
        *count = 0;
        do_query_single(h, QF_UPDATE, QB_RECOMMEND, predictor, user, nullptr, 0, items, ratings, n_ratings, n, nullptr, 0, out_items, out_preds, count);
    });
}

int knncf_revise_neighbors(knncf_handle* h, int32_t user, const int32_t* removed_items, int64_t n_removed, const int32_t* items,
                           const double* ratings, int64_t n_ratings, int32_t cap, int32_t* ids, double* sims, int32_t* count) {
    return guarded(h, [&] {
        KN_REQUIRE(count && cap >= 0 && (cap == 0 || (ids && sims)), KNNCF_E_INVALID, "bad output arguments");
        do_query_single(h, QF_REVISE, QB_NEIGHBORS, KNNCF_PRED_KNN, user, removed_items, n_removed, items, ratings, n_ratings, cap, nullptr, 0,
                        ids, sims, count);
    });
}

int knncf_revise_predict(knncf_handle* h, int predictor, int32_t user, const int32_t* removed_items, int64_t n_removed,
                         const int32_t* items, const double* ratings, int64_t n_ratings, const int32_t* pred_items, int64_t m, double* out) {
    return guarded(h, [&] {
        KN_REQUIRE(m >= 0 && (m == 0 || (pred_items && out)), KNNCF_E_INVALID, "bad prediction arguments");
        do_query_single(h, QF_REVISE, QB_PREDICT, predictor, user, removed_items, n_removed, items, ratings, n_ratings, 0, pred_items, m,
                        nullptr, out, nullptr);
    });
}

int knncf_revise_recommend(knncf_handle* h, int predictor, int32_t user, const int32_t* removed_items, int64_t n_removed,
                           const int32_t* items, const double* ratings, int64_t n_ratings, int32_t n, int32_t* out_items,
                           double* out_preds, int32_t* count) {
    return guarded(h, [&] {
        KN_REQUIRE(count && n >= 0 && (n == 0 || (out_items && out_preds)), KNNCF_E_INVALID, "bad arguments");
        *count = 0;
        do_query_single(h, QF_REVISE, QB_RECOMMEND, predictor, user, removed_items, n_removed, items, ratings, n_ratings, n, nullptr, 0,
                        out_items, out_preds, count);
    });
}

int knncf_revise_neighbors_batch(knncf_handle* h, const int32_t* users, const int64_t* removed_offsets, const int32_t* removed_items,
                                 const int64_t* offsets, const int32_t* items, const double* ratings, int64_t n_queries, int32_t cap,
                                 int32_t* ids, double* sims, int32_t* counts, int32_t* statuses) {
    return guarded(h, [&] {
        do_query_batch(h, QF_REVISE, QB_NEIGHBORS, KNNCF_PRED_KNN, users, removed_offsets, removed_items, offsets, items, ratings, n_queries,
                       cap, nullptr, nullptr, ids, sims, counts, statuses);
    });
}

int knncf_revise_predict_batch(knncf_handle* h, int predictor, const int32_t* users, const int64_t* removed_offsets,
                               const int32_t* removed_items, const int64_t* offsets, const int32_t* items, const double* ratings,
                               int64_t n_queries, const int64_t* pred_offsets, const int32_t* pred_items, double* out, int32_t* statuses) {
    return guarded(h, [&] {
        do_query_batch(h, QF_REVISE, QB_PREDICT, predictor, users, removed_offsets, removed_items, offsets, items, ratings, n_queries, 0,
                       pred_offsets, pred_items, nullptr, out, nullptr, statuses);
    });
}

int knncf_revise_recommend_batch(knncf_handle* h, int predictor, const int32_t* users, const int64_t* removed_offsets,
                                 const int32_t* removed_items, const int64_t* offsets, const int32_t* items, const double* ratings,
                                 int64_t n_queries, int32_t n, int32_t* out_items, double* out_preds, int32_t* counts, int32_t* statuses) {
    return guarded(h, [&] {
        do_query_batch(h, QF_REVISE, QB_RECOMMEND, predictor, users, removed_offsets, removed_items, offsets, items, ratings, n_queries, n,
                       nullptr, nullptr, out_items, out_preds, counts, statuses);
    });
}

int knncf_neighbors_save(knncf_handle* h, const char* path) {
    return guarded(h, [&] { do_neighbors_save(h, path); });
}

int knncf_neighbors_load(knncf_handle* h, const char* path) {
    return guarded(h, [&] { do_neighbors_load(h, path); });
}

int knncf_mae_device(knncf_handle* h, int predictor, const int32_t* d_users, const int32_t* d_items,
                     const double* d_ratings, int64_t n, double* sum_abs_err, int64_t* count, double* d_pred) {
    return guarded(h, [&] {
        KN_REQUIRE(sum_abs_err && count && (n == 0 || d_ratings), KNNCF_E_INVALID, "bad arguments");
        run_predict(h, predictor, d_users, d_items, d_ratings, n, sum_abs_err, count, d_pred);
    });
}

int knncf_mae(knncf_handle* h, int predictor, const int32_t* users, const int32_t* items, const double* ratings,
              int64_t n, double* mae) {
    return guarded(h, [&] {
        KN_REQUIRE(mae && n >= 0 && (n == 0 || (users && items && ratings)), KNNCF_E_INVALID, "bad arguments");
        KN_REQUIRE(h->cfg.shard_count == 1, KNNCF_E_STATE, "sharded handle: use knncf_mae_device and all-reduce the partial sums");
        if (n == 0) { *mae = NAN; return; }
        h->t_users.ensure(n); h->t_items.ensure(n); h->t_ratings.ensure(n);
        KN_HIP(hipMemcpyAsync(h->t_users.p, users, n * sizeof(int32_t), hipMemcpyHostToDevice, h->stream));
        KN_HIP(hipMemcpyAsync(h->t_items.p, items, n * sizeof(int32_t), hipMemcpyHostToDevice, h->stream));
        KN_HIP(hipMemcpyAsync(h->t_ratings.p, ratings, n * sizeof(double), hipMemcpyHostToDevice, h->stream));
        double s = 0.0;
        int64_t c = 0;
        run_predict(h, predictor, h->t_users.p, h->t_items.p, h->t_ratings.p, n, &s, &c, nullptr);
        *mae = s / (double)n;
    });
}

int knncf_mae_sweep_device(knncf_handle* h, const int32_t* ks, int32_t n_k, const int32_t* d_users, const int32_t* d_items,
                           const double* d_ratings, int64_t n, double* sum_abs_err, int64_t* count, double* d_pred) {
    return guarded(h, [&] {
        KN_REQUIRE(sum_abs_err && count, KNNCF_E_INVALID, "bad arguments");
        run_mae_sweep(h, ks, n_k, d_users, d_items, d_ratings, n, sum_abs_err, count, d_pred);
    });
}

int knncf_mae_sweep(knncf_handle* h, const int32_t* ks, int32_t n_k, const int32_t* users, const int32_t* items,
                    const double* ratings, int64_t n, double* maes, double* predictions) {
    return guarded(h, [&] {
        check_sweep_ks(ks, n_k);
        KN_REQUIRE(maes && n >= 0 && (n == 0 || (users && items && ratings)), KNNCF_E_INVALID, "bad arguments");
        KN_REQUIRE(h->cfg.shard_count == 1, KNNCF_E_STATE, "sharded handle: use knncf_mae_sweep_device and all-reduce the partial sums");
        require_fitted(h);
        KN_REQUIRE(h->cfg.similarity != KNNCF_SIM_ONE, KNNCF_E_UNSUPPORTED, "kNN predictor with similarityOne");
        if (n == 0) {
            for (int32_t q = 0; q < n_k; ++q) maes[q] = NAN;
            return;
        }
        h->t_users.ensure(n); h->t_items.ensure(n); h->t_ratings.ensure(n);
        KN_HIP(hipMemcpyAsync(h->t_users.p, users, n * sizeof(int32_t), hipMemcpyHostToDevice, h->stream));
        KN_HIP(hipMemcpyAsync(h->t_items.p, items, n * sizeof(int32_t), hipMemcpyHostToDevice, h->stream));
        KN_HIP(hipMemcpyAsync(h->t_ratings.p, ratings, n * sizeof(double), hipMemcpyHostToDevice, h->stream));
        if (predictions) h->t_pred.ensure((size_t)n_k * n);
        std::vector<double> s(n_k);
        int64_t c = 0;
        run_mae_sweep(h, ks, n_k, h->t_users.p, h->t_items.p, h->t_ratings.p, n, s.data(), &c, predictions ? h->t_pred.p : nullptr);
        for (int32_t q = 0; q < n_k; ++q) maes[q] = s[q] / (double)n;
        if (predictions) {
            KN_HIP(hipMemcpyAsync(predictions, h->t_pred.p, (size_t)n_k * n * sizeof(double), hipMemcpyDeviceToHost, h->stream));
            KN_HIP(hipStreamSynchronize(h->stream));
        }
    });
}

int knncf_shard_view_get(knncf_handle* h, knncf_shard_view* out) {
    return guarded(h, [&] {
        require_fitted(h, false);
        KN_REQUIRE(out, KNNCF_E_INVALID, "null out");
        Train& tr = h->tr;
        out->user_begin = tr.own_lo;
        out->user_end = tr.own_hi;
        out->nnz_begin = tr.own_p0;
        out->nnz_end = tr.own_p1;
        out->num_users = tr.U;
        out->num_ratings = tr.n;
        out->d_user_avg = tr.user_avg.p;
        out->d_user_norm = tr.user_norm.p;
        out->d_dev = tr.s_dev.p;
        out->d_pre = tr.s_pre.p;
    });
}

int knncf_shard_commit(knncf_handle* h) {
    return guarded(h, [&] {
        require_fitted(h, false);
        if (h->committed) return;
        Stage s(h, &h->tm.prep_ms);
        if (h->cfg.shard_count > 1) prep_complete_rows(h->tr, h->prep, h->stream);
        prep_commit(h->tr, h->prep, h->stream);
        h->committed = true;
    });
}

int knncf_get_timings(const knncf_handle* h, knncf_timings* out) {
    if (!h || !out) return KNNCF_E_INVALID;
    *out = h->tm;
    return KNNCF_OK;
}

int knncf_reset_timings(knncf_handle* h) {
    if (!h) return KNNCF_E_INVALID;
    h->tm = knncf_timings{};
    return KNNCF_OK;
}

int knncf_reset_neighbors(knncf_handle* h) {
    return guarded(h, [&] {
        require_fitted(h, false);
        reset_neighbors(h);
    });
}

int knncf_set_k(knncf_handle* h, int32_t k) {
    return guarded(h, [&] {
        KN_REQUIRE(k >= 0, KNNCF_E_INVALID, "negative k");
        h->cfg.k = k;
        if (h->fitted) reset_neighbors(h);
    });
}

}
```

### movie-recommender-system_amd/csrc/engine.h

```cpp
#pragma once

#include <string>
#include <vector>

#include "common.h"

namespace knncf {

typedef __bf16 bf16_t;

inline int32_t select_gcap(int32_t k) { return 8192 * (int32_t)((k + 511) / 512 > 1 ? (k + 511) / 512 : 1); }
static constexpr int SELECT_TCOLS = 16384;
static_assert(SELECT_TCOLS <= 16384 && (SELECT_TCOLS & (SELECT_TCOLS - 1)) == 0, "it_pack: 16-bit cell byte address");

struct SortWorkspace {
    DArr<char> tmp;
    DArr<size_t> count;
};
void sort_pairs_u64_u32(SortWorkspace& ws, const uint64_t* kin, uint64_t* kout, const uint32_t* vin,
                        uint32_t* vout, size_t n, int end_bit, hipStream_t st);
void sort_keys_u32(SortWorkspace& ws, const uint32_t* kin, uint32_t* kout, size_t n, hipStream_t st);
void sort_pairs_u32_u32(SortWorkspace& ws, const uint32_t* kin, uint32_t* kout, const uint32_t* vin, uint32_t* vout, size_t n,
                        int end_bit, hipStream_t st);
size_t unique_u32(SortWorkspace& ws, const uint32_t* sorted_in, uint32_t* out, size_t n, hipStream_t st);

struct Train {
    int64_t n = 0;
    int32_t U = 0, I = 0;
    DArr<int32_t> user_raw, item_raw;
    DArr<double> rating;
    DArr<uint32_t> ukeys, ikeys;
    DArr<int32_t> uid, iid;
    DArr<int32_t> u_table, i_table;
    int32_t u_table_n = 0, i_table_n = 0;
    DArr<int64_t> u_ptr;
    DArr<int32_t> s_user;
    DArr<int32_t> s_col;
    DArr<uint32_t> s_t;
    DArr<double> s_rating;
    DArr<double> s_dev;
    DArr<double> s_pre;
    DArr<uint32_t> perm_uf;
    DArr<uint32_t> perm_uh;
    DArr<int64_t> i_ptr;
    DArr<double> user_avg, user_norm;
    DArr<double> item_avg, item_dev_hash, item_dev_file;
    bool item_stats_ready = false;
    DArr<int32_t> it_user;
    DArr<uint32_t> it_pack;
    DArr<double> it_dev;
    DArr<uint32_t> it_t;
    int64_t ib_words = 0;
    DArr<uint64_t> item_bits;
    DArr<uint32_t> item_rank;
    int32_t tile_stride = 0;
    DArr<uint32_t> it_tile;
    DArr<int32_t> pop_item;
    std::vector<int64_t> pop_count;
    double global_avg = 0.0;
    int32_t own_lo = 0, own_hi = 0;
    int64_t own_p0 = 0, own_p1 = 0;
    bool jaccard = false;
};

enum : uint32_t { ST_NONFINITE = 1u, ST_DUPLICATE = 2u, ST_NOT_DYADIC = 4u, ST_LONG_ROW = 16u };

struct PrepScratch {
    SortWorkspace sort;
    DArr<uint64_t> k64_a, k64_b;
    DArr<uint32_t> v32_a, v32_b, k32_a, k32_b;
    DArr<int32_t> du_row, di_row;
    DArr<uint32_t> perm_f;
    DArr<uint32_t> status;
    DArr<int32_t> idrange;
    DArr<uint32_t> ucnt, utile;
    DArr<int32_t> long_rows;
    DArr<double> dsum;
    DArr<uint4> rec;
    hipStream_t aux = nullptr;
    hipEvent_t ev_fork = nullptr, ev_join = nullptr, ev_commit = nullptr;
    bool commit_pending = false;
    DArr<uint32_t> perm_iu;
    void join_commit(hipStream_t st);
    void ensure_aux();
    void release_all();
    PrepScratch() = default;
    PrepScratch(const PrepScratch&) = delete;
    PrepScratch& operator=(const PrepScratch&) = delete;
    ~PrepScratch();
};

void prep_fit(Train& tr, PrepScratch& sc, int32_t shard_rank, int32_t shard_count, hipStream_t st);
void prep_complete_rows(Train& tr, PrepScratch& sc, hipStream_t st);
void prep_commit(Train& tr, PrepScratch& sc, hipStream_t st);
void prep_item_stats(Train& tr, PrepScratch& sc, hipStream_t st);

void launch_dense_ids(const Train& tr, const int32_t* d_users, const int32_t* d_items, int64_t n,
                      int32_t* d_du, int32_t* d_di, hipStream_t st);

void launch_densify(const Train& tr, const int32_t* d_rows, int32_t row_begin, int32_t n_rows,
                    const int32_t* d_colmap, bf16_t* panel, int64_t ld, int64_t panel_rows, bool fp16,
                    hipStream_t st);
void launch_colmap(const Train& tr, int32_t H, int32_t* d_colmap, hipStream_t st);
void launch_gemm_nt(const bf16_t* A, const bf16_t* B, void* C, bool c_fp16, int64_t M, int64_t N, int64_t K,
                    int64_t lda, int64_t ldb, int64_t ldc, bool fp16, bool clamp, hipStream_t st);

void gemm_sym_tile_list(int32_t n_tiles, std::vector<uint32_t>& out);
void launch_gemm_sym(const bf16_t* B, void* C, bool c_fp16, int64_t N, int64_t K, int64_t ldb, int64_t ldc, bool fp16, bool clamp,
                     const uint32_t* d_tile_list, int64_t n_listed, hipStream_t st);

struct NeighborTable {
    int32_t k = 0;
    int32_t kcap = 0;
    DArr<int32_t> idx;
    DArr<double> sim;
    DArr<int32_t> uidx;
    DArr<double> usim;
    bool by_id_valid = false;
    DArr<int32_t> cnt;
    DArr<int64_t> seq;
};

struct SelectScratch {
    DArr<int32_t> cand_idx;
    DArr<float> cand_approx;
    DArr<int32_t> cand_cnt;
    DArr<float> cand_eps;
    DArr<int32_t> grp_v0;
    DArr<float> grp_x;
    DArr<double> stats;
    DArr<uint32_t> row_entries;
    DArr<double> row_exact;
    DArr<uint64_t> fb_keys_a, fb_keys_b;
    DArr<uint32_t> fb_vals_a, fb_vals_b;
};

struct TailEntries {
    const int32_t* cnt = nullptr;
    const int32_t* item = nullptr;
    const float* x = nullptr;
    const float* tail_abs = nullptr;
    const float* head_sq = nullptr;
    const float* row_len = nullptr;
};
int64_t row_len_size(int32_t U);
void launch_row_len(const Train& tr, float* d_out, hipStream_t st);
void launch_tail_entries(const Train& tr, const int32_t* d_colmap, int32_t* te_cnt, int32_t* te_item, float* te_x,
                         float* row_tail_abs, float* row_head_sq, hipStream_t st);
void launch_tail_select(const Train& tr, const int32_t* d_colmap, const TailEntries& te, bool has_tail, const void* S, bool s_by_user, bool s_fp16, int64_t lds,
                        int32_t n_rows, const int32_t* d_row_user, int32_t k, float eps_opnd, float eps_rest, int32_t cap,
                        int32_t* cand_idx, float* cand_approx, int32_t* cand_cnt, float* cand_eps, int32_t* grp_v0, float* grp_x,
                        int32_t gcap, hipStream_t st, bool anticipate = true, const int32_t* d_row_srow = nullptr);
struct SliceScratch {
    DArr<int32_t> part_idx, part_cnt;
    DArr<uint32_t> entries;
    DArr<double> part_sim;
};
struct Slices {
    int32_t n_heavy, P;
    int32_t* part_idx;
    double* part_sim;
    int32_t* part_cnt;
    uint32_t* entries;
};
void launch_rerank(const Train& tr, NeighborTable& nt, int32_t n_rows, const int32_t* d_row_user,
                   int32_t cap, const int32_t* cand_idx, const float* cand_approx,
                   const int32_t* cand_cnt, const float* cand_eps, double* d_stats, uint32_t* d_row_entries, bool verify,
                   hipStream_t st, int32_t n_heavy = 0, int32_t slices = 1, SliceScratch* sc = nullptr);
void launch_exact_row(const Train& tr, const NeighborTable& nt, int32_t user, int64_t user_seq,
                      double* d_out, hipStream_t st);
void launch_full_rows(const Train& tr, bool jaccard, int32_t* d_idx, double* d_sim, int32_t* d_cnt, hipStream_t st);
void launch_exact_pair(const Train& tr, int32_t u, int32_t v, double* d_out, hipStream_t st);

void launch_sort_neighbors(NeighborTable& nt, int32_t U, int32_t n_rows, const int32_t* d_row_user, hipStream_t st);
void launch_predict(const Train& tr, NeighborTable* nt, int predictor, int64_t n,
                    const int32_t* d_du, const int32_t* d_di, const double* d_ratings,
                    const uint32_t* d_order, bool order_by_item, double* d_pred, double* d_abs_err, uint8_t* d_owned,
                    bool unknown_users_owned, hipStream_t st);
void launch_user_keys(int64_t n, const int32_t* d_du, uint32_t limit, uint64_t* d_key, uint32_t* d_val, hipStream_t st);
void launch_owned_keys(int64_t n, const int32_t* d_src, const int32_t* d_du, int32_t own_lo, int32_t own_hi, bool unknown_owned, uint32_t limit,
                       uint64_t* d_key, uint32_t* d_val, unsigned long long* d_n_owned, hipStream_t st);
void launch_reduce_err(const double* d_abs_err, const uint8_t* d_owned, int64_t n, double* d_partials,
                       int64_t* d_counts, int32_t n_blocks, hipStream_t st);

void launch_predict_sweep(const Train& tr, const NeighborTable& nt, const int32_t* d_ks, int32_t n_k, int64_t n_rows, int64_t n_total,
                          const int32_t* d_du, const int32_t* d_di, const double* d_ratings, const uint32_t* d_order,
                          double* d_pred, double* d_abs_err, uint8_t* d_owned, bool unknown_users_owned, hipStream_t st);

static constexpr int PERSONAL_TCOLS = 8192;
struct PersonalRows {
    DArr<double> pi_pre;
    DArr<int32_t> pf_user;
    DArr<double> pf_dev;
    int32_t tiles = 0;
    DArr<uint32_t> tile;
    DArr<double> S;
    DArr<int32_t> users;
    DArr<int32_t> slot;
};
void personalized_prepare(const Train& tr, PrepScratch& sc, PersonalRows& pr, hipStream_t st);
void launch_personal_row_keys(const Train& tr, int64_t n, const int32_t* d_du, const int32_t* d_di, uint64_t* d_key,
                              uint32_t* d_val, hipStream_t st);
void launch_sim_rows(const Train& tr, const PersonalRows& pr, const int32_t* d_users, int32_t n_users, double* d_S, hipStream_t st);
void launch_fold_rows(const Train& tr, const PersonalRows& pr, int64_t n_rows, const uint32_t* d_order, const int32_t* d_du,
                      const int32_t* d_di, const double* d_ratings, const int32_t* d_slot, const double* d_S, double* d_pred,
                      double* d_abs_err, uint8_t* d_owned, hipStream_t st);

void launch_reco_rows(const Train& tr, int32_t user_raw, int32_t du, int32_t* d_users, int32_t* d_items, uint8_t* d_rated, hipStream_t st);
void launch_reco_order(const Train& tr, SortWorkspace& ws, const double* d_pred, const uint8_t* d_rated, uint64_t* k_a, uint64_t* k_b,
                       uint32_t* v_a, uint32_t* v_b, hipStream_t st);
void launch_reco_id_order(const Train& tr, SortWorkspace& ws, uint64_t* k_a, uint64_t* k_b, uint32_t* v_a, uint32_t* by_id, hipStream_t st);
void launch_reco_take(const Train& tr, int32_t m, const uint32_t* d_order, const double* d_pred, int32_t* d_items, double* d_preds, hipStream_t st);

static constexpr uint32_t QUERY_ST_NEG_MEAN = 1u << 8;
static constexpr uint32_t QUERY_ST_RM_UNRATED = 1u << 9, QUERY_ST_RM_TWICE = 1u << 10;
static constexpr int QB_MAX_CHUNK = 64;
static constexpr int QB_DUAL_MIN = 32;
inline int64_t query_batch_bytes(int32_t U, int32_t I) { return 64 * (int64_t)U + 96 * (int64_t)I; }
struct QueryBatchScratch {
    DArr<int32_t> users;
    DArr<int64_t> qo;
    DArr<int32_t> items, slot, di, given_d;
    DArr<double> ratings, dev, pre, pre_d, dev_d;
    DArr<int32_t> self;
    DArr<int64_t> ao;
    DArr<int32_t> add_items;
    DArr<double> add_ratings;
    int64_t n_removed = 0;
    DArr<int64_t> ro, so;
    std::vector<int64_t> h_so;
    DArr<int32_t> rm_items, rm_slot, rm_gone;
    DArr<uint32_t> rm_mark;
    DArr<uint64_t> bits;
    DArr<int64_t> rank;
    DArr<uint32_t> tbits, trank;
    DArr<int64_t> info;
    DArr<double> scal;
    DArr<double> sim;
    DArr<uint64_t> k64_a, k64_b;
    DArr<uint32_t> v32_a, v32_b, s32_a, s32_b;
    DArr<int32_t> nbr_idx;
    DArr<double> nbr_sim;
    DArr<int64_t> off, ebase;
    DArr<uint64_t> e_k64_a, e_k64_b;
    DArr<uint32_t> e_v32_a, e_v32_b;
    DArr<double> e_dev, e_sim;
    DArr<double> num, den, pred;
    DArr<uint8_t> rated;
    DArr<uint32_t> by_id;
    DArr<int32_t> pick_items, pick_slot, out_items;
    DArr<double> pick_out, out_preds;
};
void foldin_batch_neighbors(const Train& tr, QueryBatchScratch& bs, SortWorkspace& ws, int32_t C, const int32_t* h_users,
                            const int64_t* h_qo, const int32_t* h_items, const double* h_ratings, const int32_t* h_self,
                            const int64_t* h_ao, int32_t k, long long* h_info, hipStream_t st, const int64_t* h_ro = nullptr,
                            const int32_t* h_removed = nullptr);
void foldin_batch_predictions(const Train& tr, QueryBatchScratch& bs, SortWorkspace& ws, int32_t C, int32_t take,
                              const int64_t* h_ebase, hipStream_t st);
void foldin_batch_pick(const Train& tr, QueryBatchScratch& bs, const int32_t* d_items, const int32_t* d_slot, int64_t m,
                       double* d_out, hipStream_t st);
void foldin_batch_recommend(const Train& tr, QueryBatchScratch& bs, SortWorkspace& ws, int32_t C, int32_t n, int32_t* d_items,
                            double* d_preds, hipStream_t st);

static constexpr int RB_TPB = 256;
static constexpr int RB_TILE = 2048;
static constexpr int RB_CAP = 2560;
static constexpr int RB_MAX_K = 2048;
static constexpr int RB_FAST_N = 32;
static constexpr int RB_MAX_CHUNK = 1024;
inline int64_t reco_batch_bytes(int32_t I) { return 96 * (int64_t)I; }
struct RecoBatchScratch {
    DArr<int32_t> slot_user, slot_raw;
    DArr<int32_t> counts;
    DArr<uint32_t> id_rank;
    DArr<uint64_t> p_key;
    DArr<uint32_t> p_rank, p_item;
    DArr<int32_t> row_users, row_items;
};
void reco_batch_id_rank(const Train& tr, QueryBatchScratch& bs, RecoBatchScratch& rb, SortWorkspace& ws, hipStream_t st);
void reco_batch_fold(const Train& tr, const NeighborTable& nt, const RecoBatchScratch& rb, int32_t C, double* d_pred, hipStream_t st);
void reco_batch_rows(const Train& tr, const RecoBatchScratch& rb, int32_t C, int32_t* d_users, int32_t* d_items, hipStream_t st);
void reco_batch_mark(const Train& tr, const RecoBatchScratch& rb, int32_t C, int32_t n, uint8_t* d_rated, long long* d_info, hipStream_t st);
void reco_batch_select(const Train& tr, RecoBatchScratch& rb, int32_t C, int32_t n, const double* d_pred, const uint8_t* d_rated,
                       int32_t* d_items, double* d_preds, hipStream_t st);

}
```

### movie-recommender-system_amd/csrc/select.hip

```cpp
#include <math.h>

#include <type_traits>
#include <stdio.h>
#include <stdlib.h>
#include <string.h>

#include "engine.h"

namespace knncf {

#ifdef KNNCF_SELECT_PROFILE
__device__ unsigned long long g_phase[16];
#define PH(i) do { if (threadIdx.x == 0) { const long long now_ = clock64(); atomicAdd(&g_phase[i], (unsigned long long)(now_ - ph_t)); ph_t = now_; } } while (0)
#else
#define PH(i) do {} while (0)
#endif

static constexpr int TPB = 512;
static constexpr uint32_t REFRESH_MASK = 0x80008000u;
static constexpr int NBINS = 1024;
static constexpr int TCOLS = SELECT_TCOLS;
static constexpr int CPT = TCOLS / TPB;
static constexpr int NG = CPT / 8;
static_assert(CPT <= 32, "the survivor mask of a thread is one 32-bit word");
static constexpr int EMAX = 256;
static constexpr int PMAX = 1024;
static constexpr int MAXT = 12;
static constexpr int WAVES_PER_EU = 4;
static constexpr int TAIL_G = 8;
static constexpr double TAIL_SCALE = 2147418112.0;
static constexpr float TAIL_FIX = (float)(16777216.0 / TAIL_SCALE);
static constexpr float TAIL_FIX_JAC = 1.0f / 1073741824.0f;
static constexpr float TAIL_UNFIX = 1.0f / 16777216.0f;

static constexpr float HIST_LO = -0.125f;
__device__ __forceinline__ int sim_bin(float x) {
    int b = (int)floorf((x - HIST_LO) * (float)NBINS);
    return min(max(b, 0), NBINS - 1);
}

__device__ __forceinline__ float row_eps(float eps_base, int64_t row_len) {
    return eps_base + (float)row_len * 3.0f * 6.1e-8f;
}

struct TailArgs {
    const int64_t* u_ptr;
    const int32_t* s_col;
    const double* s_pre;
    const int32_t* colmap;
    const int64_t* i_ptr;
    const uint32_t* it_pack;
    uint32_t pack_bytes;
    const uint32_t* it_tile;
    int32_t tile_stride;
    int32_t has_tail;
    const int32_t* te_cnt;
    const int32_t* te_item;
    const float* te_x;
    const float* row_tail_abs;
    const float* row_head_sq;
    const float* row_len;
};

__global__ void k_tail_entries(int32_t u_lo, int32_t U, const int64_t* __restrict__ u_ptr, const int32_t* __restrict__ s_col,
                               const double* __restrict__ s_pre, const int32_t* __restrict__ colmap, int32_t* __restrict__ te_cnt,
                               int32_t* __restrict__ te_item, float* __restrict__ te_x, float* __restrict__ row_tail_abs,
                               float* __restrict__ row_head_sq, int ones) {
    const int32_t u = u_lo + (int32_t)(((int64_t)blockIdx.x * blockDim.x + threadIdx.x) >> 6);
    const int lane = threadIdx.x & 63;
    if (u >= U) return;
    const int64_t ub = u_ptr[u], ue = u_ptr[u + 1];
    float tail_abs = 0.f, head_sq = 0.f;
    int32_t n_out = 0;
    for (int64_t p0 = ub; p0 < ue; p0 += 64) {
        const int64_t p = p0 + lane;
        bool is_tail = false;
        int32_t item = 0;
        float x = 0.f;
        if (p < ue) {
            item = s_col[p];
            x = (float)s_pre[p];
            is_tail = colmap[item] < 0;
            if (is_tail) tail_abs += fabsf(x);
            else head_sq = __builtin_fmaf(x, x, head_sq);
        }
        const unsigned long long m = __ballot(is_tail);
        if (is_tail) {
            const int32_t slot = n_out + __popcll(m & ((1ull << lane) - 1ull));
            te_item[ub + slot] = item;
            te_x[ub + slot] = ones ? TAIL_FIX_JAC : x * TAIL_FIX;
        }
        n_out += __popcll(m);
    }
#pragma unroll
    for (int o = 32; o > 0; o >>= 1) {
        tail_abs += __shfl_xor(tail_abs, o);
        head_sq += __shfl_xor(head_sq, o);
    }
    if (lane == 0) {
        te_cnt[u] = n_out;
        row_tail_abs[u] = tail_abs;
        row_head_sq[u] = head_sq;
    }
}

void launch_tail_entries(const Train& tr, const int32_t* d_colmap, int32_t* te_cnt, int32_t* te_item, float* te_x,
                         float* row_tail_abs, float* row_head_sq, hipStream_t st) {
    const int32_t lo = tr.own_lo, hi = tr.own_hi;
    if (hi <= lo) return;
    k_tail_entries<<<(unsigned)ceil_div((int64_t)(hi - lo) * 64, 256), 256, 0, st>>>(lo, hi, tr.u_ptr.p, tr.s_col.p, tr.s_pre.p, d_colmap, te_cnt,
                                                                                     te_item, te_x, row_tail_abs, row_head_sq, tr.jaccard ? 1 : 0);
    KN_HIP(hipGetLastError());
}

__global__ void k_row_len(int64_t n_out, int32_t U, const int64_t* __restrict__ u_ptr, float* __restrict__ out) {
    const int64_t v = (int64_t)blockIdx.x * blockDim.x + threadIdx.x;
    if (v < n_out) out[v] = v < U ? (float)(u_ptr[v + 1] - u_ptr[v]) : 1.0f;
}

int64_t row_len_size(int32_t U) { return round_up(U, SELECT_TCOLS) + SELECT_TCOLS; }

void launch_row_len(const Train& tr, float* d_out, hipStream_t st) {
    const int64_t n_out = row_len_size(tr.U);
    k_row_len<<<(unsigned)ceil_div(n_out, 256), 256, 0, st>>>(n_out, tr.U, tr.u_ptr.p, d_out);
    KN_HIP(hipGetLastError());
}

__device__ __forceinline__ void block_threshold(const uint32_t* hist, uint32_t* wtot, float* s_thr, int32_t* s_bin, int32_t kk, float eps) {
    constexpr int PER = NBINS / TPB;
    const int lane = threadIdx.x & 63, wave = threadIdx.x >> 6;
    uint32_t h[PER];
    uint32_t mine = 0;
#pragma unroll
    for (int j = 0; j < PER; ++j) {
        h[j] = hist[threadIdx.x * PER + j];
        mine += h[j];
    }
    uint32_t suf = mine;
#pragma unroll
    for (int o = 1; o < 64; o <<= 1) {
        uint32_t up = __shfl_down(suf, o);
        if (lane + o < 64) suf += up;
    }
    if (lane == 0) wtot[wave] = suf;
    if (threadIdx.x == 0) { *s_thr = -INFINITY; *s_bin = 0; }
    __syncthreads();
    uint32_t higher = 0;
    for (int w = wave + 1; w < TPB / 64; ++w) higher += wtot[w];
    const uint32_t incl = suf + higher;
    const uint32_t above = incl - mine;
    if (above < (uint32_t)kk && incl >= (uint32_t)kk) {
        uint32_t c = above;
        int j = PER - 1;
        for (; j > 0; --j) {
            c += h[j];
            if (c >= (uint32_t)kk) break;
        }
        const int b = threadIdx.x * PER + j;
        const float edge = (float)b / (float)NBINS + HIST_LO;
        *s_thr = (b == 0) ? -INFINITY : edge - 2.0f * eps - 1e-6f;
        *s_bin = b;
    }
    __syncthreads();
}

template <class ST>
struct Raw8;
template <>
struct Raw8<float> {
    float4 a, b;
    __device__ __forceinline__ void load(const float* p) {
        a = reinterpret_cast<const float4*>(p)[0];
        b = reinterpret_cast<const float4*>(p)[1];
    }
    __device__ __forceinline__ void zero() { a = make_float4(0.f, 0.f, 0.f, 0.f); b = a; }
    __device__ __forceinline__ void unpack(float* out) const {
        out[0] = a.x; out[1] = a.y; out[2] = a.z; out[3] = a.w; out[4] = b.x; out[5] = b.y; out[6] = b.z; out[7] = b.w;
    }
};
template <>
struct Raw8<_Float16> {
    typedef __attribute__((ext_vector_type(8))) _Float16 h8;
    h8 v;
    __device__ __forceinline__ void load(const _Float16* p) { v = *reinterpret_cast<const h8*>(p); }
    __device__ __forceinline__ void zero() {
#pragma unroll
        for (int i = 0; i < 8; ++i) v[i] = (_Float16)0.f;
    }
    __device__ __forceinline__ void unpack(float* out) const {
#pragma unroll
        for (int i = 0; i < 8; ++i) out[i] = (float)v[i];
    }
};

template <class ST, bool JAC>
__global__ void __launch_bounds__(TPB, WAVES_PER_EU) k_tail_select(const ST* __restrict__ S, int32_t s_by_user, int64_t ld, int32_t n_rows,
                                                     const int32_t* __restrict__ row_user, const int32_t* __restrict__ row_srow, TailArgs T, int32_t U,
                                                     int32_t kk, float eps_opnd, float eps_rest, int32_t cap, int32_t* __restrict__ cand_idx,
                                                     float* __restrict__ cand_approx, int32_t* __restrict__ cand_cnt,
                                                     float* __restrict__ cand_eps, int32_t* __restrict__ grp_v0,
                                                     float* __restrict__ grp_x, int32_t GCAP, float ant_sigma) {
    extern __shared__ __attribute__((aligned(16))) char smem[];
    int32_t* itile = reinterpret_cast<int32_t*>(smem);
    uint32_t* hist = reinterpret_cast<uint32_t*>(itile + TCOLS);
    float* e_x = reinterpret_cast<float*>(hist + NBINS);
    uint32_t* e_b0 = reinterpret_cast<uint32_t*>(e_x + EMAX);
    uint32_t* e_e0 = e_b0 + 2 * EMAX;
    uint32_t* e_ps0 = e_e0 + 2 * EMAX;
    int32_t* e_item = reinterpret_cast<int32_t*>(e_ps0);
    uint16_t* piece_e0 = reinterpret_cast<uint16_t*>(e_ps0 + 2 * EMAX);
    uint32_t* wtot = reinterpret_cast<uint32_t*>(piece_e0 + 2 * PMAX);
    uint32_t* wtot2 = wtot + TPB / 64 + 4;
    uint32_t* e_b = e_b0;
    uint32_t* e_e = e_e0;
    uint32_t* e_ps = e_ps0;
    uint16_t* piece_e = piece_e0;
    float& s_thr = *reinterpret_cast<float*>(wtot + TPB / 64);
    uint32_t& s_count = wtot[TPB / 64 + 1];
    int32_t& s_ne = *reinterpret_cast<int32_t*>(wtot + TPB / 64 + 2);
    int32_t& s_bin = *reinterpret_cast<int32_t*>(wtot2 + TPB / 64);
    const int32_t r = blockIdx.x;
    if (r >= n_rows) return;
#ifdef KNNCF_SELECT_PROFILE
    long long ph_t = clock64();
#endif
    const int32_t u = row_user[r];
    const int lane = threadIdx.x & 63, wave = threadIdx.x >> 6;
    const int64_t ub = T.u_ptr[u], ue = T.u_ptr[u + 1];
    const ST* row = S + (int64_t)(s_by_user ? u : (row_srow ? row_srow[r] : r)) * ld;
    int32_t* out_idx = cand_idx + (int64_t)r * cap;
    float* out_apx = cand_approx + (int64_t)r * cap;
    int32_t* g_v0 = grp_v0 + (int64_t)r * GCAP;
    float4* g_x = reinterpret_cast<float4*>(grp_x + (int64_t)r * GCAP * 8);
    Raw8<ST> raw[NG];
#pragma unroll
    for (int j = 0; j < NG; ++j) {
        const int64_t v0 = 8 * (threadIdx.x + TPB * j);
        if (v0 < ld) raw[j].load(row + v0);
        else raw[j].zero();
    }
    for (int b = threadIdx.x; b < NBINS; b += TPB) hist[b] = 0;
    if (threadIdx.x == 0) { s_count = 0; s_ne = 0; s_thr = -INFINITY; }
    __syncthreads();

    const int32_t n_te = T.has_tail ? T.te_cnt[u] : 0;
    const int n_chunks = (n_te + EMAX - 1) / EMAX;
    const int n_tiles = T.tile_stride - 1;
    const bool reg_counts = n_chunks == 1 && n_tiles <= MAXT;
    auto collect = [&](int ch) {
        const int32_t c0 = ch * EMAX, cn = min(EMAX, n_te - c0);
        for (int32_t j = threadIdx.x; j < cn; j += TPB) {
            e_item[j] = T.te_item[ub + c0 + j];
            e_x[j] = T.te_x[ub + c0 + j];
        }
        if (threadIdx.x == 0) s_ne = cn;
    };
    float tail_abs = 0.f;
    float head_norm = 1.0f;
    if (T.has_tail) {
        tail_abs = T.row_tail_abs[u];
        head_norm = fminf(1.0f, sqrtf(T.row_head_sq[u]) * 1.0001f + 1e-6f);
    }
    if (n_chunks == 1) collect(0);
    __syncthreads();
    const float eps = JAC ? 4e-7f : row_eps(eps_opnd * head_norm + eps_rest, ue - ub) + tail_abs * (1.0001f / 65536.0f);
    if (threadIdx.x == 0) cand_eps[r] = eps;
    const bool any_tail = n_chunks > 0;
    const uint32_t* my_tb = T.it_tile;
    uint32_t cur_b = 0, cw[MAXT / 2];
#pragma unroll
    for (int t = 0; t < MAXT / 2; ++t) cw[t] = 0;
    if (n_chunks == 1 && (int32_t)threadIdx.x < s_ne) {
        my_tb = T.it_tile + (int64_t)e_item[threadIdx.x] * T.tile_stride;
        if (reg_counts) {
            uint32_t tbv[MAXT + 1];
#pragma unroll
            for (int t = 0; t <= MAXT; ++t) tbv[t] = my_tb[min(t, n_tiles)];
            cur_b = tbv[0];
#pragma unroll
            for (int t = 0; t < MAXT; ++t) cw[t >> 1] |= (tbv[t + 1] - tbv[t]) << (16 * (t & 1));
        }
    }
    if (any_tail) {
        for (int32_t c = threadIdx.x; c < TCOLS; c += TPB) itile[c] = 0;
    }
    __syncthreads();

    uint32_t P = 0, p_lo = 0, p_hi = 0, n_here = 0;
    int32_t ne = 0;
    uint32_t d_q = 0, d_xs = 0;
    uint32_t su_np = 0, su_incl = 0;
    auto setup_a = [&](int tile, int buf) {
        ne = s_ne;
        uint32_t np = 0;
        if ((int32_t)threadIdx.x < ne) {
            uint32_t qb, cnt;
            if (reg_counts) {
                cnt = (cw[0] >> (16 * (tile & 1))) & 0xffffu;
                qb = cur_b;
                cur_b += cnt;
                if (tile & 1) {
#pragma unroll
                    for (int t2 = 0; t2 + 1 < MAXT / 2; ++t2) cw[t2] = cw[t2 + 1];
                }
            } else {
                const uint32_t* tb = (n_chunks > 1 ? T.it_tile + (int64_t)e_item[threadIdx.x] * T.tile_stride : my_tb) + tile;
                qb = tb[0];
                cnt = tb[1] - qb;
            }
            e_b0[buf * EMAX + threadIdx.x] = qb;
            e_e0[buf * EMAX + threadIdx.x] = qb + cnt;
            np = (cnt + 63u) >> 6;
        }
        su_np = np;
        su_incl = wave_incl_scan(np);
        if (lane == 63 && wave < EMAX / 64) wtot2[wave] = su_incl;
    };
    auto setup_b = [&](int buf) {
        uint32_t off = 0;
        P = 0;
#pragma unroll
        for (int w2 = 0; w2 < EMAX / 64; ++w2) {
            const uint32_t sw = wtot2[w2];
            P += sw;
            if (w2 < wave) off += sw;
        }
        if ((int32_t)threadIdx.x < ne) {
            const uint32_t excl = off + su_incl - su_np;
            e_ps0[buf * EMAX + threadIdx.x] = excl;
            if (P <= PMAX)
                for (uint32_t k2 = 0; k2 < su_np; ++k2) piece_e0[buf * PMAX + excl + k2] = (uint16_t)threadIdx.x;
        }
        P = __builtin_amdgcn_readfirstlane(P);
        ne = __builtin_amdgcn_readfirstlane(ne);
        const uint32_t wv = __builtin_amdgcn_readfirstlane(wave);
        const uint32_t n_groups = (P + TAIL_G - 1) / TAIL_G;
        p_lo = min(P, (uint32_t)(((uint64_t)n_groups * wv) / (TPB / 64)) * TAIL_G);
        p_hi = min(P, (uint32_t)(((uint64_t)n_groups * (wv + 1)) / (TPB / 64)) * TAIL_G);
    };
    auto use_tables = [&](int buf) {
        e_b = e_b0 + buf * EMAX;
        e_e = e_e0 + buf * EMAX;
        e_ps = e_ps0 + buf * EMAX;
        piece_e = piece_e0 + buf * PMAX;
    };
    auto window = [&](uint32_t pw) {
        n_here = min(64u, p_hi - pw);
        d_q = 0;
        d_xs = 63u;
        if ((uint32_t)lane < n_here) {
            const uint32_t p2 = pw + lane;
            int32_t e;
            if (P <= PMAX) {
                e = piece_e[p2];
            } else {
                int32_t lo = 0, hi = ne - 1;
                while (lo < hi) {
                    const int32_t mid = (lo + hi + 1) >> 1;
                    if (e_ps[mid] <= p2) lo = mid;
                    else hi = mid - 1;
                }
                e = lo;
            }
            d_q = e_b[e] + ((p2 - e_ps[e]) << 6);
            const uint32_t len = min(64u, e_e[e] - d_q);
            d_xs = (__float_as_uint(e_x[e]) & ~63u) | (64u - len);
        }
    };
    typedef __attribute__((ext_vector_type(4))) uint32_t u32x4;
    const uint64_t pack_base = reinterpret_cast<uint64_t>(T.it_pack);
    const u32x4 pack_rsrc = {(uint32_t)pack_base, (uint32_t)(pack_base >> 32) & 0xffffu, T.pack_bytes, 0x00020000u};
    const uint32_t lane4 = (uint32_t)lane << 2;
#ifdef KNNCF_ABL_NOLOAD
#define KN_TAIL_LOAD(W) "v_mov_b32 %[" W "], %[l4]\n\t"
#else
#define KN_TAIL_LOAD(W) "buffer_load_dword %[" W "], %[l4], %[rs], %[sq] offen\n\t"
#endif
#ifdef KNNCF_ABL_NOATOMIC
#define KN_TAIL_ADD "s_nop 0\n\t"
#else
#define KN_TAIL_ADD "ds_add_u32 %[a], %[t]\n\t"
#endif
#ifdef KNNCF_ABL_HOTLOAD
#define KN_TAIL_HOT "s_and_b32 %[sq], %[sq], 0x3ffc\n\t"
#else
#define KN_TAIL_HOT
#endif
#define KN_TAIL_ISSUE(W, OFF)                                              \
    "s_add_u32 %[sj], %[sg], " #OFF "\n\t"                                 \
    "v_readlane_b32 %[sq], %[dq], %[sj]\n\t"                               \
    "s_lshl_b32 %[sq], %[sq], 2\n\t"                                       \
    KN_TAIL_HOT                                                            \
    KN_TAIL_LOAD(W)
#define KN_TAIL_APPLY(W, OFF, N)                                           \
    "s_add_u32 %[sj], %[sg], " #OFF "\n\t"                                 \
    "v_readlane_b32 %[sx], %[dx], %[sj]\n\t"                               \
    "s_waitcnt vmcnt(" #N ")\n\t"                                          \
    "v_cvt_f32_i32_e32 %[t], %[" W "]\n\t"                                 \
    "v_and_b32_e32 %[a], 0xfffc, %[" W "]\n\t"                             \
    "v_mul_f32_e32 %[t], %[sx], %[t]\n\t"                                  \
    "v_cvt_rpi_i32_f32_e32 %[t], %[t]\n\t"                                 \
    "s_lshr_b64 exec, -1, %[sx]\n\t"                                       \
    KN_TAIL_ADD                                                            \
    "s_mov_b64 exec, -1\n\t"
#define KN_TAIL_ISSUE8(S, B)                                                                                       \
    KN_TAIL_ISSUE(S "0", B + 0) KN_TAIL_ISSUE(S "1", B + 1) KN_TAIL_ISSUE(S "2", B + 2) KN_TAIL_ISSUE(S "3", B + 3) \
    KN_TAIL_ISSUE(S "4", B + 4) KN_TAIL_ISSUE(S "5", B + 5) KN_TAIL_ISSUE(S "6", B + 6) KN_TAIL_ISSUE(S "7", B + 7)
#define KN_TAIL_APPLY8(S)                                                                                          \
    KN_TAIL_APPLY(S "0", 0, 15) KN_TAIL_APPLY(S "1", 1, 14) KN_TAIL_APPLY(S "2", 2, 13) KN_TAIL_APPLY(S "3", 3, 12) \
    KN_TAIL_APPLY(S "4", 4, 11) KN_TAIL_APPLY(S "5", 5, 10) KN_TAIL_APPLY(S "6", 6, 9) KN_TAIL_APPLY(S "7", 7, 8)
#define KN_TAIL_APPLY8_LAST(S)                                    \
    KN_TAIL_APPLY(S "0", 0, 7) KN_TAIL_APPLY(S "1", 1, 6) KN_TAIL_APPLY(S "2", 2, 5) KN_TAIL_APPLY(S "3", 3, 4) \
    KN_TAIL_APPLY(S "4", 4, 3) KN_TAIL_APPLY(S "5", 5, 2) KN_TAIL_APPLY(S "6", 6, 1) KN_TAIL_APPLY(S "7", 7, 0)
    auto tail_window = [&](uint32_t n8) {
        uint32_t a0, a1, a2, a3, a4, a5, a6, a7, b0, b1, b2, b3, b4, b5, b6, b7, t, a, sq, sx, sj, sg;
        asm volatile(
            "s_mov_b32 %[sg], 0\n\t"
            KN_TAIL_ISSUE8("a", 0)
            "1:\n\t"
            "s_add_u32 %[sj], %[sg], 8\n\t"
            "s_cmp_ge_u32 %[sj], %[n8]\n\t"
            "s_cbranch_scc1 3f\n\t"
            KN_TAIL_ISSUE8("b", 8)
            KN_TAIL_APPLY8("a")
            "s_add_u32 %[sg], %[sg], 8\n\t"
            "s_add_u32 %[sj], %[sg], 8\n\t"
            "s_cmp_ge_u32 %[sj], %[n8]\n\t"
            "s_cbranch_scc1 4f\n\t"
            KN_TAIL_ISSUE8("a", 8)
            KN_TAIL_APPLY8("b")
            "s_add_u32 %[sg], %[sg], 8\n\t"
            "s_branch 1b\n\t"
            "3:\n\t"
            KN_TAIL_APPLY8_LAST("a")
            "s_branch 5f\n\t"
            "4:\n\t"
            KN_TAIL_APPLY8_LAST("b")
            "5:\n\t"
            : [a0] "=&v"(a0), [a1] "=&v"(a1), [a2] "=&v"(a2), [a3] "=&v"(a3), [a4] "=&v"(a4), [a5] "=&v"(a5), [a6] "=&v"(a6),
              [a7] "=&v"(a7), [b0] "=&v"(b0), [b1] "=&v"(b1), [b2] "=&v"(b2), [b3] "=&v"(b3), [b4] "=&v"(b4), [b5] "=&v"(b5),
              [b6] "=&v"(b6), [b7] "=&v"(b7), [t] "=&v"(t), [a] "=&v"(a), [sq] "=&s"(sq), [sx] "=&s"(sx), [sj] "=&s"(sj),
              [sg] "=&s"(sg)
            : [dq] "v"(d_q), [dx] "v"(d_xs), [n8] "s"(n8), [l4] "v"(lane4), [rs] "s"(pack_rsrc)
            : "memory", "scc");
    };
#undef KN_TAIL_ISSUE8
#undef KN_TAIL_APPLY8
#undef KN_TAIL_APPLY8_LAST
#undef KN_TAIL_ISSUE
#undef KN_TAIL_APPLY
    auto drain = [&](bool) {
#ifdef KNNCF_ABL_NODRAIN
        return;
#endif
        for (uint32_t pw = p_lo; pw < p_hi; pw += 64) {
            window(pw);
            tail_window(__builtin_amdgcn_readfirstlane((n_here + 7u) & ~7u));
        }
    };
    const bool pipelined = any_tail && n_chunks == 1;
    if (pipelined) {
        setup_a(0, 0);
        __syncthreads();
        setup_b(0);
        __syncthreads();
    }
    const int32_t n_tiles_row = (U + TCOLS - 1) / TCOLS;
    auto rank_after = [&](int m) -> int32_t {
        if (ant_sigma < 0.0f || n_tiles_row < 4) return kk;
        const float f = fminf(1.0f, (float)m * (float)TCOLS / (float)U);
        const float mu = (float)kk * f;
        const int32_t rk = (int32_t)ceilf(mu + ant_sigma * sqrtf(mu * (1.0f - f)) + 3.0f);
        return rk < kk ? max(rk, 1) : kk;
    };
    int32_t bin_used = 0;
    uint32_t counted = 0;
    auto count_new_groups = [&](float floor) {
        const uint32_t G = min(s_count, (uint32_t)GCAP);
        for (uint32_t g = counted + threadIdx.x; g < G; g += TPB) {
            const float4 a = g_x[2 * g], b4 = g_x[2 * g + 1];
            const float x8[8] = {a.x, a.y, a.z, a.w, b4.x, b4.y, b4.z, b4.w};
#pragma unroll
            for (int i = 0; i < 8; ++i)
                if (x8[i] >= floor && x8[i] > -INFINITY) atomicAdd(&hist[sim_bin(x8[i])], 1u);
        }
        counted = G;
        __syncthreads();
    };
    PH(0);
    int tile_no = 0;
    uint32_t next_refresh = (uint32_t)GCAP / 4;
    for (int32_t t0 = 0; t0 < U; t0 += TCOLS, ++tile_no) {
        float sx[CPT];
        auto take_panel = [&]() {
#pragma unroll
            for (int j = 0; j < NG; ++j) raw[j].unpack(&sx[8 * j]);
            if (t0 + TCOLS < U) {
#pragma unroll
                for (int j = 0; j < NG; ++j) {
                    const int64_t v0 = (int64_t)t0 + TCOLS + 8 * (threadIdx.x + TPB * j);
                    if (v0 < ld) raw[j].load(row + v0);
                    else raw[j].zero();
                }
            }
            if (t0 + TCOLS > U || (u >= t0 && u < t0 + TCOLS)) {
#pragma unroll
                for (int j = 0; j < NG; ++j) {
                    const int32_t v0 = t0 + 8 * (threadIdx.x + TPB * j);
#pragma unroll
                    for (int i = 0; i < 8; ++i)
                        if (v0 + i >= U || v0 + i == u) sx[8 * j + i] = -INFINITY;
                }
            }
        };
        if (pipelined) {
            use_tables(tile_no & 1);
            drain(false);
            PH(4);
            take_panel();
            const bool more = t0 + TCOLS < U;
            if (more) setup_a(tile_no + 1, (tile_no + 1) & 1);
            __syncthreads();
            PH(5);
            if (more) setup_b((tile_no + 1) & 1);
            else p_lo = p_hi = 0;
        } else if (any_tail) {
            use_tables(0);
            for (int ch = 0; ch < n_chunks; ++ch) {
                if (n_chunks > 1) {
                    __syncthreads();
                    collect(ch);
                    __syncthreads();
                }
                setup_a(tile_no, 0);
                __syncthreads();
                setup_b(0);
                __syncthreads();
                PH(2);
                drain(false);
                PH(4);
                __syncthreads();
                PH(5);
            }
        }
        if (!pipelined) take_panel();
        PH(1);
        if (any_tail) {
#pragma unroll
            for (int j = 0; j < NG; ++j) {
                const int32_t g = threadIdx.x + TPB * j;
                int4* lo4 = reinterpret_cast<int4*>(itile + 4 * g);
                int4* hi4 = reinterpret_cast<int4*>(itile + TCOLS / 2 + 4 * g);
                const int4 a = *lo4, b = *hi4;
                *lo4 = make_int4(0, 0, 0, 0);
                *hi4 = make_int4(0, 0, 0, 0);
                constexpr float UNFIX = JAC ? 1.0f : TAIL_UNFIX;
                sx[8 * j + 0] = __builtin_fmaf((float)a.x, UNFIX, sx[8 * j + 0]); sx[8 * j + 1] = __builtin_fmaf((float)a.y, UNFIX, sx[8 * j + 1]);
                sx[8 * j + 2] = __builtin_fmaf((float)a.z, UNFIX, sx[8 * j + 2]); sx[8 * j + 3] = __builtin_fmaf((float)a.w, UNFIX, sx[8 * j + 3]);
                sx[8 * j + 4] = __builtin_fmaf((float)b.x, UNFIX, sx[8 * j + 4]); sx[8 * j + 5] = __builtin_fmaf((float)b.y, UNFIX, sx[8 * j + 5]);
                sx[8 * j + 6] = __builtin_fmaf((float)b.z, UNFIX, sx[8 * j + 6]); sx[8 * j + 7] = __builtin_fmaf((float)b.w, UNFIX, sx[8 * j + 7]);
            }
        }
        if (JAC) {
            const float nu_f = (float)(ue - ub);
#pragma unroll
            for (int j = 0; j < NG; ++j) {
                const float4* lp = reinterpret_cast<const float4*>(T.row_len + (int64_t)t0 + 8 * (threadIdx.x + TPB * j));
                const float4 la = lp[0], lb = lp[1];
                const float len8[8] = {la.x, la.y, la.z, la.w, lb.x, lb.y, lb.z, lb.w};
#pragma unroll
                for (int i = 0; i < 8; ++i) {
                    const float c = sx[8 * j + i];
                    sx[8 * j + i] = c > -INFINITY ? c / (nu_f + len8[i] - c) : c;
                }
            }
        }
        PH(6);
        float gm[NG];
#pragma unroll
        for (int j = 0; j < NG; ++j) {
            const float* x8 = &sx[8 * j];
            gm[j] = fmaxf(fmaxf(fmaxf(x8[0], x8[1]), fmaxf(x8[2], x8[3])), fmaxf(fmaxf(x8[4], x8[5]), fmaxf(x8[6], x8[7])));
        }
        if (tile_no == 0) {
            const int32_t kk0 = rank_after(1);
            if (NG >= 4 && kk0 <= (TCOLS / 32) / 3) {
#pragma unroll
                for (int j = 0; j + 3 < NG; j += 4) {
                    const float m = fmaxf(fmaxf(gm[j], gm[j + 1]), fmaxf(gm[j + 2], gm[j + 3]));
                    if (m > -INFINITY) atomicAdd(&hist[sim_bin(m)], 1u);
                }
            } else if (kk0 <= (TCOLS / 8) / 3) {
#pragma unroll
                for (int j = 0; j < NG; ++j)
                    if (gm[j] > -INFINITY) atomicAdd(&hist[sim_bin(gm[j])], 1u);
            } else {
#pragma unroll
                for (int i = 0; i < CPT; ++i)
                    if (sx[i] > -INFINITY) atomicAdd(&hist[sim_bin(sx[i])], 1u);
            }
            __syncthreads();
            block_threshold(hist, wtot, &s_thr, &s_bin, kk0, eps);
            bin_used = max(bin_used, s_bin);
            for (int b = threadIdx.x; b < NBINS; b += TPB) hist[b] = 0;
            __syncthreads();
        }
        {
            const float thr = s_thr;
            uint32_t gmask = 0;
#pragma unroll
            for (int j = 0; j < NG; ++j)
                if (gm[j] >= thr && gm[j] > -INFINITY) gmask |= 1u << j;
            const uint32_t cnt = __popc(gmask);
            const uint32_t incl = wave_incl_scan(cnt);
            const uint32_t total = __builtin_amdgcn_readlane(incl, 63);
            if (total > 0) {
                uint32_t base = 0;
                if (lane == 63) base = atomicAdd(&s_count, total);
                base = __builtin_amdgcn_readlane(base, 63);
                const uint32_t first = base + incl - cnt;
#pragma unroll
                for (int j = 0; j < NG; ++j) {
                    if (gmask & (1u << j)) {
                        const uint32_t pos = first + __popc(gmask & ((1u << j) - 1u));
                        if (pos < (uint32_t)GCAP) {
                            g_v0[pos] = t0 + 8 * (threadIdx.x + TPB * j);
                            g_x[2 * pos] = make_float4(sx[8 * j], sx[8 * j + 1], sx[8 * j + 2], sx[8 * j + 3]);
                            g_x[2 * pos + 1] = make_float4(sx[8 * j + 4], sx[8 * j + 5], sx[8 * j + 6], sx[8 * j + 7]);
                        }
                    }
                }
            }
        }
        PH(tile_no == 0 ? 7 : 8);
        __syncthreads();
        PH(9);
        {
            const uint32_t prov = s_count;
            if (((tile_no < 32 && ((REFRESH_MASK >> tile_no) & 1u)) || prov > next_refresh) && prov <= (uint32_t)GCAP && t0 + TCOLS < U) {
                count_new_groups(s_thr);
                block_threshold(hist, wtot, &s_thr, &s_bin, rank_after(tile_no + 1), eps);
                bin_used = max(bin_used, s_bin);
                next_refresh = max(next_refresh, prov + (uint32_t)GCAP / 8);
            }
        }
    }

    if (s_count > (uint32_t)GCAP) {
        if (threadIdx.x == 0) cand_cnt[r] = 0x7fffffff;
        return;
    }
    constexpr int FB = 4;
    const uint32_t G = s_count;
    float4 fxa[FB], fxb[FB];
    int32_t fv0[FB];
#pragma unroll
    for (int q = 0; q < FB; ++q) {
        const uint32_t g = (uint32_t)q * TPB + threadIdx.x;
        fxa[q] = fxb[q] = make_float4(-INFINITY, -INFINITY, -INFINITY, -INFINITY);
        fv0[q] = 0;
        if (g < G) {
            fxa[q] = g_x[2 * g];
            fxb[q] = g_x[2 * g + 1];
            fv0[q] = g_v0[g];
        }
    }
    {
        const float floor = s_thr;
#pragma unroll
        for (int q = 0; q < FB; ++q) {
            const uint32_t g = (uint32_t)q * TPB + threadIdx.x;
            if (g >= counted && g < G) {
                const float x8[8] = {fxa[q].x, fxa[q].y, fxa[q].z, fxa[q].w, fxb[q].x, fxb[q].y, fxb[q].z, fxb[q].w};
#pragma unroll
                for (int i = 0; i < 8; ++i)
                    if (x8[i] >= floor && x8[i] > -INFINITY) atomicAdd(&hist[sim_bin(x8[i])], 1u);
            }
        }
        counted = max(counted, min(G, (uint32_t)FB * TPB));
        count_new_groups(floor);
    }
    block_threshold(hist, wtot, &s_thr, &s_bin, kk, eps);
    PH(10);
    if (s_bin < bin_used) {
        if (threadIdx.x == 0) cand_cnt[r] = 0x7fffffff;
        return;
    }
    {
        const float thr = s_thr;
        uint32_t& s_out = wtot[TPB / 64 + 3];
        if (threadIdx.x == 0) s_out = 0;
        __syncthreads();
        auto emit = [&](uint32_t m, int32_t v0, const float* x8) {
            const uint32_t cnt = __popc(m);
            const uint32_t incl = wave_incl_scan(cnt);
            const uint32_t total = __builtin_amdgcn_readlane(incl, 63);
            if (total > 0) {
                uint32_t base = 0;
                if (lane == 63) base = atomicAdd(&s_out, total);
                base = __builtin_amdgcn_readlane(base, 63);
                uint32_t pos = base + incl - cnt;
#pragma unroll
                for (int i = 0; i < 8; ++i) {
                    if (m & (1u << i)) {
                        if (pos < (uint32_t)cap) {
                            out_idx[pos] = v0 + i;
                            out_apx[pos] = x8[i];
                        }
                        ++pos;
                    }
                }
            }
        };
#pragma unroll
        for (int q = 0; q < FB; ++q) {
            if ((uint32_t)q * TPB >= G) break;
            const float x8[8] = {fxa[q].x, fxa[q].y, fxa[q].z, fxa[q].w, fxb[q].x, fxb[q].y, fxb[q].z, fxb[q].w};
            uint32_t m = 0;
#pragma unroll
            for (int i = 0; i < 8; ++i)
                if (x8[i] >= thr && x8[i] > -INFINITY) m |= 1u << i;
            emit(m, fv0[q], x8);
        }
        for (uint32_t g0 = (uint32_t)FB * TPB; g0 < G; g0 += TPB) {
            const uint32_t g = g0 + threadIdx.x;
            float x8[8] = {0.f, 0.f, 0.f, 0.f, 0.f, 0.f, 0.f, 0.f};
            int32_t v0 = 0;
            uint32_t m = 0;
            if (g < G) {
                v0 = g_v0[g];
                const float4 a = g_x[2 * g], b4 = g_x[2 * g + 1];
                x8[0] = a.x; x8[1] = a.y; x8[2] = a.z; x8[3] = a.w; x8[4] = b4.x; x8[5] = b4.y; x8[6] = b4.z; x8[7] = b4.w;
#pragma unroll
                for (int i = 0; i < 8; ++i)
                    if (x8[i] >= thr && x8[i] > -INFINITY) m |= 1u << i;
            }
            emit(m, v0, x8);
        }
        __syncthreads();
        if (threadIdx.x == 0) cand_cnt[r] = (int32_t)min(s_out, (uint32_t)0x7fffffff);
    }
    PH(11);
    return;
}

#ifdef KNNCF_SELECT_PROFILE
void select_profile_dump() {
    unsigned long long h[16];
    hipMemcpyFromSymbol(h, HIP_SYMBOL(g_phase), sizeof(h));
    unsigned long long tot = 0;
    for (int i = 0; i < 16; ++i) tot += h[i];
    fprintf(stderr, "[select profile] cycles per phase (thread 0 of every block), total %.3e\n", (double)tot);
    for (int i = 0; i <= 11; ++i) fprintf(stderr, "  phase %2d: %6.2f %%\n", i, 100.0 * (double)h[i] / (double)tot);
    memset(h, 0, sizeof(h));
    hipMemcpyToSymbol(HIP_SYMBOL(g_phase), h, sizeof(h));
}
#endif

template <class ST, bool JAC>
static void launch_tail_select_t(const TailArgs& T, const ST* S, bool s_by_user, int64_t lds, int32_t n_rows, const int32_t* d_row_user, const int32_t* d_row_srow,
                                 int32_t U, int32_t kk, float eps_opnd, float eps_rest, int32_t cap, int32_t* cand_idx, float* cand_approx,
                                 int32_t* cand_cnt, float* cand_eps, int32_t* grp_v0, float* grp_x, int32_t gcap, bool anticipate, hipStream_t st) {
    const size_t smem = (size_t)TCOLS * 4 + (size_t)NBINS * 4 + (size_t)EMAX * 4 + 2 * ((size_t)EMAX * 12 + (size_t)PMAX * 2) + (2 * (TPB / 64) + 4 + 64) * 4;
    static PerDeviceState lds_state;
    ensure_dynamic_lds(lds_state, (const void*)k_tail_select<ST, JAC>, smem);
    const char* sg = getenv("KNNCF_DEBUG_ANTICIPATE_SIGMA");
    const float ant_sigma = !anticipate ? -1.0f : sg ? (float)atof(sg) : 7.0f;
    k_tail_select<ST, JAC><<<n_rows, TPB, smem, st>>>(S, s_by_user ? 1 : 0, lds, n_rows, d_row_user, d_row_srow, T, U, kk, eps_opnd, eps_rest, cap, cand_idx, cand_approx, cand_cnt, cand_eps, grp_v0, grp_x, gcap, ant_sigma);
    KN_HIP(hipGetLastError());
#ifdef KNNCF_SELECT_PROFILE
    KN_HIP(hipStreamSynchronize(st));
    select_profile_dump();
#endif
}

void launch_tail_select(const Train& tr, const int32_t* d_colmap, const TailEntries& te, bool has_tail, const void* S, bool s_by_user, bool s_fp16, int64_t lds,
                        int32_t n_rows, const int32_t* d_row_user, int32_t k, float eps_opnd, float eps_rest, int32_t cap,
                        int32_t* cand_idx, float* cand_approx, int32_t* cand_cnt, float* cand_eps, int32_t* grp_v0, float* grp_x,
                        int32_t gcap, hipStream_t st, bool anticipate, const int32_t* d_row_srow) {
    if (n_rows <= 0) return;
    KN_REQUIRE(gcap >= 1024 && gcap % 8 == 0, KNNCF_E_INVALID, "select: group store too small");
    const int32_t U = tr.U;
    int32_t kk = k < U - 1 ? k : U - 1;
    if (kk < 1) kk = 1;
    KN_REQUIRE(!has_tail || tr.tile_stride == (int32_t)ceil_div(U, TCOLS) + 1, KNNCF_E_STATE, "select: tile table missing");
#ifdef KNNCF_ABL_NOTAIL
    has_tail = false;
#endif
    KN_REQUIRE(!has_tail || (te.cnt && te.item && te.x && te.tail_abs && te.head_sq), KNNCF_E_STATE, "select: tail entry lists missing");
    TailArgs T{tr.u_ptr.p, tr.s_col.p, tr.s_pre.p, d_colmap, tr.i_ptr.p, tr.it_pack.p, (uint32_t)(tr.n * 4), tr.it_tile.p, tr.tile_stride, has_tail ? 1 : 0,
               te.cnt, te.item, te.x, te.tail_abs, te.head_sq, te.row_len};
    if (tr.jaccard) {
        KN_REQUIRE(te.row_len != nullptr, KNNCF_E_STATE, "select: row lengths missing");
        if (s_fp16) launch_tail_select_t<_Float16, true>(T, static_cast<const _Float16*>(S), s_by_user, lds, n_rows, d_row_user, d_row_srow, U, kk, eps_opnd, eps_rest, cap, cand_idx, cand_approx, cand_cnt, cand_eps, grp_v0, grp_x, gcap, anticipate, st);
        else launch_tail_select_t<float, true>(T, static_cast<const float*>(S), s_by_user, lds, n_rows, d_row_user, d_row_srow, U, kk, eps_opnd, eps_rest, cap, cand_idx, cand_approx, cand_cnt, cand_eps, grp_v0, grp_x, gcap, anticipate, st);
    } else {
        if (s_fp16) launch_tail_select_t<_Float16, false>(T, static_cast<const _Float16*>(S), s_by_user, lds, n_rows, d_row_user, d_row_srow, U, kk, eps_opnd, eps_rest, cap, cand_idx, cand_approx, cand_cnt, cand_eps, grp_v0, grp_x, gcap, anticipate, st);
        else launch_tail_select_t<float, false>(T, static_cast<const float*>(S), s_by_user, lds, n_rows, d_row_user, d_row_srow, U, kk, eps_opnd, eps_rest, cap, cand_idx, cand_approx, cand_cnt, cand_eps, grp_v0, grp_x, gcap, anticipate, st);
    }
}

}
```

Measured before the change: 85.67 million.

## Precompute tail piece stream on aux stream and consume it in select kernel

Adds count, scan and fill kernels that build a per-row, per-column-tile list of packed tail pieces on an auxiliary stream. In the symmetric path these run concurrently with the GEMM. A new STREAM template variant of the tail-select kernel reads these precomputed records straight from global memory instead of building per-tile tables in LDS, which cuts LDS use and removes in-kernel table setup. In exchange it costs extra device memory for the piece buffer, a host sync to size it, and a fallback to the old path when the budget is exceeded.

```diff
diff --git a/movie-recommender-system_amd/csrc/api.cpp b/movie-recommender-system_amd/csrc/api.cpp
--- a/movie-recommender-system_amd/csrc/api.cpp
+++ b/movie-recommender-system_amd/csrc/api.cpp
@@ -46,6 +46,13 @@
     DArr<int32_t> te_cnt, te_item;
     DArr<float> te_x, row_tail_abs, row_head_sq;
     DArr<float> row_len;
+    DArr<uint2> pieces;
+    DArr<int64_t> piece_ptr;
+    DArr<uint32_t> piece_cnt;
+    DArr<unsigned long long> piece_bsum;
+    DArr<long long> piece_total;
+    long long* pinned_total = nullptr;
+    hipEvent_t ev_pieces_fork = nullptr, ev_pieces_join = nullptr;
     hipStream_t stream2 = nullptr;
     DArr<bf16_t> Apanel[2];
     DArr<float> S[2];
@@ -342,26 +349,20 @@
     const int64_t K_pad = h->K_pad;
     const int32_t head = h->head;
     h->tm.head_items = head;
-    if (use_sym) {
-        const int32_t n_tiles = (int32_t)(U_pad / 256);
-        if (h->sym_tiles_n != n_tiles) {
-            std::vector<uint32_t> list;
-            gemm_sym_tile_list(n_tiles, list);
-            h->sym_tiles.ensure(list.size());
-            KN_HIP(hipMemcpyAsync(h->sym_tiles.p, list.data(), list.size() * sizeof(uint32_t), hipMemcpyHostToDevice, st));
-            KN_HIP(hipStreamSynchronize(st));
-            h->sym_tiles_n = n_tiles;
-        }
-        const int64_t n_listed = (int64_t)n_tiles * (n_tiles + 1) / 2;
-        Stage s(h, &h->tm.gemm_ms);
-        launch_gemm_sym(h->Bpanel.p, h->S_full.p, s_fp16, U_pad, h->K_pad, h->K_pad, U_pad, fp16, !tr.jaccard, h->sym_tiles.p, n_listed, st);
-        h->tm.gemm_launches += 1;
-        h->tm.gemm_flops_executed += 2.0 * 256.0 * 256.0 * (double)n_listed * (double)h->K_pad;
-        h->tm.gemm_flops_algorithmic += 2.0 * (double)count * (double)(tr.U - 1) * (double)h->head;
-        KN_HIP(hipMemGetInfo(&free_b, &total_b));
-    } else {
-        h->S_full.release();
-    }
+    const bool tail_present = head < tr.I;
+    const int32_t n_ctiles = tail_present ? tr.tile_stride - 1 : 0;
+    const char* stream_cap = getenv("KNNCF_DEBUG_PIECE_STREAM_BYTES");
+    const bool stream_wanted = tail_present && n_ctiles >= 1 && n_ctiles <= select_max_stream_tiles() && !(stream_cap && atoll(stream_cap) <= 0);
+    bool stream_forked = false;
+    auto fork_stream = [&] {
+        if (!stream_wanted || stream_forked) return;
+        h->prep.ensure_aux();
+        KN_HIP(hipEventRecord(h->ev_pieces_fork, st));
+        KN_HIP(hipStreamWaitEvent(h->prep.aux, h->ev_pieces_fork, 0));
+        stream_forked = true;
+    };
+    fork_stream();
+    if (!use_sym) h->S_full.release();
     size_t held = 0;
     for (int s = 0; s < 2; ++s) held += h->S[s].bytes() + h->Apanel[s].bytes();
     held += h->sel.cand_idx.bytes() + h->sel.cand_approx.bytes() + h->sel.grp_v0.bytes() + h->sel.grp_x.bytes();
@@ -404,8 +405,86 @@
     const float eps_rest = gemm_eps_rest(fp16) + (s_fp16 ? 2.45e-4f : 0.f);
     hipStream_t sp = slots > 1 ? h->stream2 : h->stream;
     hipStream_t sc = h->stream;
+    int64_t stream_budget = 0;
+    if (stream_wanted) {
+        KN_HIP(hipMemGetInfo(&free_b, &total_b));
+        stream_budget = stream_cap ? atoll(stream_cap)
+                        : h->cfg.workspace_bytes > 0 ? h->cfg.workspace_bytes / 2
+                                                     : (int64_t)std::min<size_t>((size_t)16 << 30, (free_b + h->pieces.bytes()) / 4);
+    }
+    bool stream_on = false;
+    PieceStream ps;
+    bool stream_counted = false;
+    auto count_stream = [&](int32_t rows, const int32_t* d_rows) {
+        stream_on = false;
+        if (!stream_forked || stream_counted) return;
+        stream_counted = true;
+        hipStream_t sx = h->prep.aux;
+        TailEntries te{h->te_cnt.p, h->te_item.p, h->te_x.p, h->row_tail_abs.p, h->row_head_sq.p, h->row_len.p};
+        const int64_t cells = (int64_t)rows * n_ctiles;
+        h->piece_cnt.ensure((size_t)cells);
+        h->piece_bsum.ensure((size_t)piece_scan_blocks(cells));
+        h->piece_ptr.ensure((size_t)cells + 1);
+        h->piece_total.ensure(1);
+        {
+            Stage s(h, &h->tm.densify_ms, sx);
+            launch_piece_count(tr, te, rows, d_rows, h->piece_cnt.p, h->piece_bsum.p, h->piece_ptr.p, h->piece_total.p, sx);
+        }
+        KN_HIP(hipMemcpyAsync(h->pinned_total, h->piece_total.p, sizeof(long long), hipMemcpyDeviceToHost, sx));
+    };
+    auto build_stream = [&](int32_t rows, const int32_t* d_rows) {
+        count_stream(rows, d_rows);
+        if (!stream_counted) {
+            stream_on = false;
+            return;
+        }
+        stream_forked = stream_counted = false;
+        hipStream_t sx = h->prep.aux;
+        TailEntries te{h->te_cnt.p, h->te_item.p, h->te_x.p, h->row_tail_abs.p, h->row_head_sq.p, h->row_len.p};
+        KN_HIP(hipStreamSynchronize(sx));
+        const int64_t records = (int64_t)*h->pinned_total + 64;
+        bool fits = records * (int64_t)sizeof(uint2) <= stream_budget && records < ((int64_t)1 << 32);
+        if (fits) {
+            try {
+                h->pieces.ensure((size_t)records);
+            } catch (const Error& e) {
+                if (e.status != KNNCF_E_NOMEM) throw;
+                (void)hipGetLastError();
+                fits = false;
+            }
+        }
+        if (fits) {
+            Stage s(h, &h->tm.densify_ms, sx);
+            launch_piece_fill(tr, te, rows, d_rows, h->piece_ptr.p, h->pieces.p, sx);
+        }
+        KN_HIP(hipEventRecord(h->ev_pieces_join, sx));
+        KN_HIP(hipStreamWaitEvent(sc, h->ev_pieces_join, 0));
+        stream_on = fits;
+        ps.pieces = h->pieces.p;
+        ps.ptr = h->piece_ptr.p;
+        ps.row_prow = nullptr;
+    };
     KN_HIP(hipEventRecord(h->ev_ready, sc));
     KN_HIP(hipStreamWaitEvent(sp, h->ev_ready, 0));
+    if (use_sym) {
+        count_stream((int32_t)std::min<int64_t>(R, count), h->build_list.p);
+        const int32_t n_tiles = (int32_t)(U_pad / 256);
+        if (h->sym_tiles_n != n_tiles) {
+            std::vector<uint32_t> list;
+            gemm_sym_tile_list(n_tiles, list);
+            h->sym_tiles.ensure(list.size());
+            KN_HIP(hipMemcpyAsync(h->sym_tiles.p, list.data(), list.size() * sizeof(uint32_t), hipMemcpyHostToDevice, st));
+            KN_HIP(hipStreamSynchronize(st));
+            h->sym_tiles_n = n_tiles;
+        }
+        const int64_t n_listed = (int64_t)n_tiles * (n_tiles + 1) / 2;
+        Stage s(h, &h->tm.gemm_ms);
+        launch_gemm_sym(h->Bpanel.p, h->S_full.p, s_fp16, U_pad, h->K_pad, h->K_pad, U_pad, fp16, !tr.jaccard, h->sym_tiles.p, n_listed, st);
+        h->tm.gemm_launches += 1;
+        h->tm.gemm_flops_executed += 2.0 * 256.0 * 256.0 * (double)n_listed * (double)h->K_pad;
+        h->tm.gemm_flops_algorithmic += 2.0 * (double)count * (double)(tr.U - 1) * (double)h->head;
+        KN_HIP(hipMemGetInfo(&free_b, &total_b));
+    }
     std::vector<int32_t> h_rows;
     auto need_h_rows = [&] {
         if (!h_rows.empty()) return;
@@ -413,7 +492,7 @@
         KN_HIP(hipMemcpyAsync(h_rows.data(), h->build_list.p, (size_t)count * sizeof(int32_t), hipMemcpyDeviceToHost, st));
         KN_HIP(hipStreamSynchronize(st));
     };
-    auto redo_marked = [&](const std::vector<int32_t>& marked, const void* Sp, bool by_user, int64_t rb) {
+    auto redo_marked = [&](const std::vector<int32_t>& marked, const void* Sp, bool by_user, int64_t rb, bool with_stream) {
         need_h_rows();
         std::vector<int32_t> users(marked.size()), srow(marked.size());
         for (size_t j = 0; j < marked.size(); ++j) {
@@ -429,9 +508,12 @@
             KN_HIP(hipMemcpyAsync(h->redo_rows.p + chunk, srow.data() + j0, (size_t)m * sizeof(int32_t), hipMemcpyHostToDevice, st));
             {
                 Stage s(h, &h->tm.select_ms);
+                PieceStream ps_redo = ps;
+                ps_redo.row_prow = h->redo_rows.p + chunk;
                 launch_tail_select(tr, h->colmap.p, te, head < tr.I, Sp, by_user, s_fp16, U_pad, m, h->redo_rows.p, nt.k, eps_opnd, eps_rest, cap,
                                    h->sel.cand_idx.p, h->sel.cand_approx.p, h->sel.cand_cnt.p, h->sel.cand_eps.p, h->sel.grp_v0.p, h->sel.grp_x.p,
-                                   select_gcap(nt.k), st, false, by_user ? nullptr : h->redo_rows.p + chunk);
+                                   select_gcap(nt.k), st, false, by_user ? nullptr : h->redo_rows.p + chunk,
+                                   with_stream && stream_on ? &ps_redo : nullptr);
                 h->tm.select_launches += 1;
             }
             {
@@ -453,6 +535,7 @@
         const int32_t* d_rows = h->build_list.p + rb;
         const int slot = (int)(b % slots);
         if (b >= slots) KN_HIP(hipStreamWaitEvent(sp, h->ev_consumed[slot], 0));
+        fork_stream();
         if (!use_sym) {
             Stage s(h, &h->tm.densify_ms, sp);
             launch_densify(tr, d_rows, 0, rows, h->colmap.p, h->Apanel[slot].p, K_pad, M, fp16, sp);
@@ -464,6 +547,7 @@
             h->tm.gemm_flops_executed += 2.0 * (double)M * (double)U_pad * (double)K_pad;
             h->tm.gemm_flops_algorithmic += 2.0 * (double)rows * (double)(tr.U - 1) * (double)head;
         }
+        build_stream(rows, d_rows);
         KN_HIP(hipEventRecord(h->ev_produced[slot], sp));
         KN_HIP(hipStreamWaitEvent(sc, h->ev_produced[slot], 0));
         TailEntries te{h->te_cnt.p, h->te_item.p, h->te_x.p, h->row_tail_abs.p, h->row_head_sq.p, h->row_len.p};
@@ -475,7 +559,8 @@
             const void* Sp = use_sym ? Sblk : (const void*)(static_cast<const char*>(Sblk) + (size_t)r0 * (size_t)U_pad * (size_t)s_elem);
             launch_tail_select(tr, h->colmap.p, te, head < tr.I, Sp, use_sym, s_fp16, U_pad, nr, d_rows + r0, nt.k, eps_opnd, eps_rest, cap,
                                h->sel.cand_idx.p + (size_t)r0 * cap, h->sel.cand_approx.p + (size_t)r0 * cap, h->sel.cand_cnt.p + r0, h->sel.cand_eps.p + r0,
-                               h->sel.grp_v0.p + (size_t)r0 * gcap, h->sel.grp_x.p + (size_t)r0 * gcap * 8, gcap, sc);
+                               h->sel.grp_v0.p + (size_t)r0 * gcap, h->sel.grp_x.p + (size_t)r0 * gcap * 8, gcap, sc, true, nullptr,
+                               stream_on && r0 == 0 ? &ps : nullptr);
             h->tm.select_launches += 1;
             h->tm.tail_pair_updates += h->tail_pairs_full * ((double)nr / (double)tr.U);
             h->tm.select_row_bytes += (double)s_elem * (double)nr * (double)tr.U;
@@ -501,7 +586,7 @@
             for (int64_t r = rb; r < rb + rows; ++r)
                 if (h->pinned_cnt[r] > cap) marked.push_back((int32_t)r);
             if ((int64_t)marked.size() > std::max<int64_t>(64, rows / 200)) {
-                redo_marked(marked, h->S[slot].p, false, rb);
+                redo_marked(marked, h->S[slot].p, false, rb, true);
             }
             if (overlap) KN_HIP(hipEventRecord(h->ev_consumed[slot], sc));
         }
@@ -533,7 +618,7 @@
         std::vector<int32_t> marked;
         for (int64_t r = 0; r < count; ++r)
             if (h->pinned_cnt[r] > cap) marked.push_back((int32_t)r);
-        if ((int64_t)marked.size() > std::max<int64_t>(64, count / 200)) redo_marked(marked, use_sym ? (const void*)h->S_full.p : (const void*)h->S[0].p, use_sym, 0);
+        if ((int64_t)marked.size() > std::max<int64_t>(64, count / 200)) redo_marked(marked, use_sym ? (const void*)h->S_full.p : (const void*)h->S[0].p, use_sym, 0, n_blocks == 1);
     }
     for (int64_t r = 0; r < count; ++r) {
         h->tm.shortlist_total += std::min(h->pinned_cnt[r], cap);
@@ -1271,6 +1356,9 @@
         return KNNCF_E_HIP;
     }
     bool ok = hipEventCreateWithFlags(&h->ev_ready, hipEventDisableTiming) == hipSuccess;
+    ok = ok && hipEventCreateWithFlags(&h->ev_pieces_fork, hipEventDisableTiming) == hipSuccess;
+    ok = ok && hipEventCreateWithFlags(&h->ev_pieces_join, hipEventDisableTiming) == hipSuccess;
+    ok = ok && hipHostMalloc((void**)&h->pinned_total, sizeof(long long), hipHostMallocDefault) == hipSuccess;
     for (int s = 0; s < 2; ++s) {
         ok = ok && hipEventCreateWithFlags(&h->ev_produced[s], hipEventDisableTiming) == hipSuccess;
         ok = ok && hipEventCreateWithFlags(&h->ev_consumed[s], hipEventDisableTiming) == hipSuccess;
@@ -1296,6 +1384,10 @@
         if (h->ev_consumed[s]) (void)hipEventDestroy(h->ev_consumed[s]);
     }
     if (h->pinned_cnt) (void)hipHostFree(h->pinned_cnt);
+    if (h->prep.aux) (void)hipStreamSynchronize(h->prep.aux);
+    if (h->ev_pieces_fork) (void)hipEventDestroy(h->ev_pieces_fork);
+    if (h->ev_pieces_join) (void)hipEventDestroy(h->ev_pieces_join);
+    if (h->pinned_total) (void)hipHostFree(h->pinned_total);
     if (h->stream2) (void)hipStreamDestroy(h->stream2);
     (void)hipStreamDestroy(h->stream);
     delete h;
diff --git a/movie-recommender-system_amd/csrc/engine.h b/movie-recommender-system_amd/csrc/engine.h
--- a/movie-recommender-system_amd/csrc/engine.h
+++ b/movie-recommender-system_amd/csrc/engine.h
@@ -143,6 +143,16 @@
     const float* head_sq = nullptr;
     const float* row_len = nullptr;
 };
+struct PieceStream {
+    const uint2* pieces = nullptr;
+    const int64_t* ptr = nullptr;
+    const int32_t* row_prow = nullptr;
+};
+int select_max_stream_tiles();
+int64_t piece_scan_blocks(int64_t n_cells);
+void launch_piece_count(const Train& tr, const TailEntries& te, int32_t n_rows, const int32_t* d_row_user, uint32_t* cnt, unsigned long long* bsum,
+                        int64_t* ptr, long long* d_total, hipStream_t st);
+void launch_piece_fill(const Train& tr, const TailEntries& te, int32_t n_rows, const int32_t* d_row_user, const int64_t* ptr, uint2* pieces, hipStream_t st);
 int64_t row_len_size(int32_t U);
 void launch_row_len(const Train& tr, float* d_out, hipStream_t st);
 void launch_tail_entries(const Train& tr, const int32_t* d_colmap, int32_t* te_cnt, int32_t* te_item, float* te_x,
@@ -150,7 +160,7 @@
 void launch_tail_select(const Train& tr, const int32_t* d_colmap, const TailEntries& te, bool has_tail, const void* S, bool s_by_user, bool s_fp16, int64_t lds,
                         int32_t n_rows, const int32_t* d_row_user, int32_t k, float eps_opnd, float eps_rest, int32_t cap,
                         int32_t* cand_idx, float* cand_approx, int32_t* cand_cnt, float* cand_eps, int32_t* grp_v0, float* grp_x,
-                        int32_t gcap, hipStream_t st, bool anticipate = true, const int32_t* d_row_srow = nullptr);
+                        int32_t gcap, hipStream_t st, bool anticipate = true, const int32_t* d_row_srow = nullptr, const PieceStream* ps = nullptr);
 struct SliceScratch {
     DArr<int32_t> part_idx, part_cnt;
     DArr<uint32_t> entries;
diff --git a/movie-recommender-system_amd/csrc/select.hip b/movie-recommender-system_amd/csrc/select.hip
--- a/movie-recommender-system_amd/csrc/select.hip
+++ b/movie-recommender-system_amd/csrc/select.hip
@@ -60,6 +60,9 @@
     const float* row_tail_abs;
     const float* row_head_sq;
     const float* row_len;
+    const uint2* pieces;
+    const int64_t* piece_ptr;
+    const int32_t* row_prow;
 };
 
 __global__ void k_tail_entries(int32_t u_lo, int32_t U, const int64_t* __restrict__ u_ptr, const int32_t* __restrict__ s_col,
@@ -113,6 +116,157 @@
     KN_HIP(hipGetLastError());
 }
 
+static constexpr int PIECE_SCAN_PER = 8;
+static constexpr int PIECE_SCAN_TILE = 256 * PIECE_SCAN_PER;
+
+__global__ void __launch_bounds__(256) k_piece_count(int32_t n_rows, int32_t n_tiles, const int32_t* __restrict__ row_user,
+                                                     const int64_t* __restrict__ u_ptr, const int32_t* __restrict__ te_cnt,
+                                                     const int32_t* __restrict__ te_item, const uint32_t* __restrict__ it_tile,
+                                                     int32_t tile_stride, uint32_t* __restrict__ cnt) {
+    const int64_t w = ((int64_t)blockIdx.x * blockDim.x + threadIdx.x) >> 6;
+    const int lane = threadIdx.x & 63;
+    if (w >= (int64_t)n_rows * n_tiles) return;
+    const int32_t r = (int32_t)(w / n_tiles), t = (int32_t)(w - (int64_t)r * n_tiles);
+    const int32_t u = row_user[r];
+    const int64_t ub = u_ptr[u];
+    const int32_t n_te = te_cnt[u];
+    uint32_t np = 0;
+    for (int32_t j = lane; j < n_te; j += 64) {
+        const uint32_t* tb = it_tile + (int64_t)te_item[ub + j] * tile_stride + t;
+        np += (tb[1] - tb[0] + 63u) >> 6;
+    }
+#pragma unroll
+    for (int o = 32; o > 0; o >>= 1) np += __shfl_xor(np, o);
+    if (lane == 0) cnt[w] = (np + (uint32_t)TAIL_G - 1u) & ~((uint32_t)TAIL_G - 1u);
+}
+
+__global__ void __launch_bounds__(256) k_piece_scan_sums(const uint32_t* __restrict__ cnt, int64_t n, unsigned long long* __restrict__ bsum) {
+    __shared__ unsigned long long wsum[4];
+    const int64_t i0 = (int64_t)blockIdx.x * PIECE_SCAN_TILE + (int64_t)threadIdx.x * PIECE_SCAN_PER;
+    unsigned long long s = 0;
+    for (int j = 0; j < PIECE_SCAN_PER; ++j)
+        if (i0 + j < n) s += cnt[i0 + j];
+#pragma unroll
+    for (int o = 32; o > 0; o >>= 1) s += __shfl_xor(s, o);
+    if ((threadIdx.x & 63) == 0) wsum[threadIdx.x >> 6] = s;
+    __syncthreads();
+    if (threadIdx.x == 0) bsum[blockIdx.x] = wsum[0] + wsum[1] + wsum[2] + wsum[3];
+}
+__global__ void __launch_bounds__(1024) k_piece_scan_top(unsigned long long* __restrict__ bsum, int64_t nb, int64_t* __restrict__ ptr_end,
+                                                         long long* __restrict__ total_out) {
+    __shared__ unsigned long long wsum[16];
+    const int lane = threadIdx.x & 63, wave = threadIdx.x >> 6;
+    const int64_t per = (nb + 1023) / 1024;
+    const int64_t b0 = (int64_t)threadIdx.x * per;
+    unsigned long long mine = 0;
+    for (int64_t j = 0; j < per; ++j)
+        if (b0 + j < nb) mine += bsum[b0 + j];
+    unsigned long long incl = mine;
+#pragma unroll
+    for (int o = 1; o < 64; o <<= 1) {
+        const unsigned long long up = __shfl_up(incl, o);
+        if (lane >= o) incl += up;
+    }
+    if (lane == 63) wsum[wave] = incl;
+    __syncthreads();
+    unsigned long long run = incl - mine;
+    for (int w2 = 0; w2 < wave; ++w2) run += wsum[w2];
+    if (threadIdx.x == 1023) {
+        *ptr_end = (int64_t)(run + mine);
+        *total_out = (long long)(run + mine);
+    }
+    for (int64_t j = 0; j < per; ++j)
+        if (b0 + j < nb) {
+            const unsigned long long v = bsum[b0 + j];
+            bsum[b0 + j] = run;
+            run += v;
+        }
+}
+__global__ void __launch_bounds__(256) k_piece_scan_write(const uint32_t* __restrict__ cnt, int64_t n, const unsigned long long* __restrict__ bsum,
+                                                          int64_t* __restrict__ ptr) {
+    __shared__ unsigned long long wsum[4];
+    const int lane = threadIdx.x & 63, wave = threadIdx.x >> 6;
+    const int64_t i0 = (int64_t)blockIdx.x * PIECE_SCAN_TILE + (int64_t)threadIdx.x * PIECE_SCAN_PER;
+    uint32_t c[PIECE_SCAN_PER];
+    unsigned long long mine = 0;
+#pragma unroll
+    for (int j = 0; j < PIECE_SCAN_PER; ++j) {
+        c[j] = i0 + j < n ? cnt[i0 + j] : 0u;
+        mine += c[j];
+    }
+    unsigned long long incl = mine;
+#pragma unroll
+    for (int o = 1; o < 64; o <<= 1) {
+        const unsigned long long up = __shfl_up(incl, o);
+        if (lane >= o) incl += up;
+    }
+    if (lane == 63) wsum[wave] = incl;
+    __syncthreads();
+    unsigned long long run = bsum[blockIdx.x] + incl - mine;
+    for (int w2 = 0; w2 < wave; ++w2) run += wsum[w2];
+#pragma unroll
+    for (int j = 0; j < PIECE_SCAN_PER; ++j) {
+        if (i0 + j < n) ptr[i0 + j] = (int64_t)run;
+        run += c[j];
+    }
+}
+
+__global__ void __launch_bounds__(256) k_piece_fill(int32_t n_rows, int32_t n_tiles, const int32_t* __restrict__ row_user,
+                                                    const int64_t* __restrict__ u_ptr, const int32_t* __restrict__ te_cnt,
+                                                    const int32_t* __restrict__ te_item, const float* __restrict__ te_x,
+                                                    const uint32_t* __restrict__ it_tile, int32_t tile_stride,
+                                                    const int64_t* __restrict__ ptr, uint2* __restrict__ pieces) {
+    const int64_t w = ((int64_t)blockIdx.x * blockDim.x + threadIdx.x) >> 6;
+    const int lane = threadIdx.x & 63;
+    if (w >= (int64_t)n_rows * n_tiles) return;
+    const int32_t r = (int32_t)(w / n_tiles), t = (int32_t)(w - (int64_t)r * n_tiles);
+    const int32_t u = row_user[r];
+    const int64_t ub = u_ptr[u];
+    const int32_t n_te = te_cnt[u];
+    const int64_t base = ptr[w], end = ptr[w + 1];
+    int64_t run = base;
+    for (int32_t j0 = 0; j0 < n_te; j0 += 64) {
+        const int32_t j = j0 + lane;
+        uint32_t qb = 0, cnt = 0, xb = 0;
+        if (j < n_te) {
+            const uint32_t* tb = it_tile + (int64_t)te_item[ub + j] * tile_stride + t;
+            qb = tb[0];
+            cnt = tb[1] - qb;
+            xb = __float_as_uint(te_x[ub + j]) & ~63u;
+        }
+        const uint32_t np = (cnt + 63u) >> 6;
+        const uint32_t incl = wave_incl_scan(np);
+        const int64_t first = run + (incl - np);
+        for (uint32_t k2 = 0; k2 < np; ++k2) {
+            const uint32_t len = min(64u, cnt - (k2 << 6));
+            if (first + k2 < end) pieces[first + k2] = make_uint2(qb + (k2 << 6), xb | (64u - len));
+        }
+        run += (uint32_t)__builtin_amdgcn_readlane((int)incl, 63);
+    }
+    for (int64_t p = run + lane; p < end; p += 64) pieces[p] = make_uint2(0u, 63u);
+}
+
+int64_t piece_scan_blocks(int64_t n_cells) { return ceil_div(n_cells, PIECE_SCAN_TILE); }
+
+void launch_piece_count(const Train& tr, const TailEntries& te, int32_t n_rows, const int32_t* d_row_user, uint32_t* cnt, unsigned long long* bsum,
+                        int64_t* ptr, long long* d_total, hipStream_t st) {
+    const int32_t n_tiles = tr.tile_stride - 1;
+    const int64_t cells = (int64_t)n_rows * n_tiles;
+    const int64_t nb = piece_scan_blocks(cells);
+    k_piece_count<<<(unsigned)ceil_div(cells * 64, 256), 256, 0, st>>>(n_rows, n_tiles, d_row_user, tr.u_ptr.p, te.cnt, te.item, tr.it_tile.p, tr.tile_stride, cnt);
+    KN_HIP(hipGetLastError());
+    k_piece_scan_sums<<<(unsigned)nb, 256, 0, st>>>(cnt, cells, bsum);
+    k_piece_scan_top<<<1, 1024, 0, st>>>(bsum, nb, ptr + cells, d_total);
+    k_piece_scan_write<<<(unsigned)nb, 256, 0, st>>>(cnt, cells, bsum, ptr);
+    KN_HIP(hipGetLastError());
+}
+void launch_piece_fill(const Train& tr, const TailEntries& te, int32_t n_rows, const int32_t* d_row_user, const int64_t* ptr, uint2* pieces, hipStream_t st) {
+    const int32_t n_tiles = tr.tile_stride - 1;
+    const int64_t cells = (int64_t)n_rows * n_tiles;
+    k_piece_fill<<<(unsigned)ceil_div(cells * 64, 256), 256, 0, st>>>(n_rows, n_tiles, d_row_user, tr.u_ptr.p, te.cnt, te.item, te.x, tr.it_tile.p, tr.tile_stride, ptr, pieces);
+    KN_HIP(hipGetLastError());
+}
+
 __global__ void k_row_len(int64_t n_out, int32_t U, const int64_t* __restrict__ u_ptr, float* __restrict__ out) {
     const int64_t v = (int64_t)blockIdx.x * blockDim.x + threadIdx.x;
     if (v < n_out) out[v] = v < U ? (float)(u_ptr[v + 1] - u_ptr[v]) : 1.0f;
@@ -193,7 +347,7 @@
     }
 };
 
-template <class ST, bool JAC>
+template <class ST, bool JAC, bool STREAM>
 __global__ void __launch_bounds__(TPB, WAVES_PER_EU) k_tail_select(const ST* __restrict__ S, int32_t s_by_user, int64_t ld, int32_t n_rows,
                                                      const int32_t* __restrict__ row_user, const int32_t* __restrict__ row_srow, TailArgs T, int32_t U,
                                                      int32_t kk, float eps_opnd, float eps_rest, int32_t cap, int32_t* __restrict__ cand_idx,
@@ -209,7 +363,7 @@
     uint32_t* e_ps0 = e_e0 + 2 * EMAX;
     int32_t* e_item = reinterpret_cast<int32_t*>(e_ps0);
     uint16_t* piece_e0 = reinterpret_cast<uint16_t*>(e_ps0 + 2 * EMAX);
-    uint32_t* wtot = reinterpret_cast<uint32_t*>(piece_e0 + 2 * PMAX);
+    uint32_t* wtot = STREAM ? hist + NBINS : reinterpret_cast<uint32_t*>(piece_e0 + 2 * PMAX);
     uint32_t* wtot2 = wtot + TPB / 64 + 4;
     uint32_t* e_b = e_b0;
     uint32_t* e_e = e_e0;
@@ -244,9 +398,16 @@
     __syncthreads();
 
     const int32_t n_te = T.has_tail ? T.te_cnt[u] : 0;
-    const int n_chunks = (n_te + EMAX - 1) / EMAX;
+    const int n_chunks = STREAM ? (n_te > 0 ? 1 : 0) : (n_te + EMAX - 1) / EMAX;
     const int n_tiles = T.tile_stride - 1;
-    const bool reg_counts = n_chunks == 1 && n_tiles <= MAXT;
+    const bool reg_counts = !STREAM && n_chunks == 1 && n_tiles <= MAXT;
+    int64_t pbase = 0;
+    uint32_t prel = 0;
+    if constexpr (STREAM) {
+        const int64_t* pp = T.piece_ptr + (int64_t)(T.row_prow ? T.row_prow[r] : r) * n_tiles;
+        pbase = pp[0];
+        prel = (uint32_t)(pp[min(lane, n_tiles)] - pbase);
+    }
     auto collect = [&](int ch) {
         const int32_t c0 = ch * EMAX, cn = min(EMAX, n_te - c0);
         for (int32_t j = threadIdx.x; j < cn; j += TPB) {
@@ -261,7 +422,7 @@
         tail_abs = T.row_tail_abs[u];
         head_norm = fminf(1.0f, sqrtf(T.row_head_sq[u]) * 1.0001f + 1e-6f);
     }
-    if (n_chunks == 1) collect(0);
+    if (!STREAM && n_chunks == 1) collect(0);
     __syncthreads();
     const float eps = JAC ? 4e-7f : row_eps(eps_opnd * head_norm + eps_rest, ue - ub) + tail_abs * (1.0001f / 65536.0f);
     if (threadIdx.x == 0) cand_eps[r] = eps;
@@ -270,7 +431,7 @@
     uint32_t cur_b = 0, cw[MAXT / 2];
 #pragma unroll
     for (int t = 0; t < MAXT / 2; ++t) cw[t] = 0;
-    if (n_chunks == 1 && (int32_t)threadIdx.x < s_ne) {
+    if (!STREAM && n_chunks == 1 && (int32_t)threadIdx.x < s_ne) {
         my_tb = T.it_tile + (int64_t)e_item[threadIdx.x] * T.tile_stride;
         if (reg_counts) {
             uint32_t tbv[MAXT + 1];
@@ -412,7 +573,7 @@
 #define KN_TAIL_APPLY8_LAST(S)                                    \
     KN_TAIL_APPLY(S "0", 0, 7) KN_TAIL_APPLY(S "1", 1, 6) KN_TAIL_APPLY(S "2", 2, 5) KN_TAIL_APPLY(S "3", 3, 4) \
     KN_TAIL_APPLY(S "4", 4, 3) KN_TAIL_APPLY(S "5", 5, 2) KN_TAIL_APPLY(S "6", 6, 1) KN_TAIL_APPLY(S "7", 7, 0)
-    auto tail_window = [&](uint32_t n8) {
+    auto tail_window = [&](uint32_t w_q, uint32_t w_xs, uint32_t n8) {
         uint32_t a0, a1, a2, a3, a4, a5, a6, a7, b0, b1, b2, b3, b4, b5, b6, b7, t, a, sq, sx, sj, sg;
         asm volatile(
             "s_mov_b32 %[sg], 0\n\t"
@@ -441,7 +602,7 @@
               [a7] "=&v"(a7), [b0] "=&v"(b0), [b1] "=&v"(b1), [b2] "=&v"(b2), [b3] "=&v"(b3), [b4] "=&v"(b4), [b5] "=&v"(b5),
               [b6] "=&v"(b6), [b7] "=&v"(b7), [t] "=&v"(t), [a] "=&v"(a), [sq] "=&s"(sq), [sx] "=&s"(sx), [sj] "=&s"(sj),
               [sg] "=&s"(sg)
-            : [dq] "v"(d_q), [dx] "v"(d_xs), [n8] "s"(n8), [l4] "v"(lane4), [rs] "s"(pack_rsrc)
+            : [dq] "v"(w_q), [dx] "v"(w_xs), [n8] "s"(n8), [l4] "v"(lane4), [rs] "s"(pack_rsrc)
             : "memory", "scc");
     };
 #undef KN_TAIL_ISSUE8
@@ -455,10 +616,40 @@
 #endif
         for (uint32_t pw = p_lo; pw < p_hi; pw += 64) {
             window(pw);
-            tail_window(__builtin_amdgcn_readfirstlane((n_here + 7u) & ~7u));
-        }
-    };
-    const bool pipelined = any_tail && n_chunks == 1;
+            tail_window(d_q, d_xs, __builtin_amdgcn_readfirstlane((n_here + 7u) & ~7u));
+        }
+    };
+    uint32_t s_lo = 0, s_hi = 0;
+    const uint2* const row_pieces = T.pieces + pbase;
+    auto stream_share = [&](int tile) {
+        const uint32_t a = (uint32_t)__builtin_amdgcn_readlane((int)prel, tile), b = (uint32_t)__builtin_amdgcn_readlane((int)prel, tile + 1);
+        const uint32_t wv = __builtin_amdgcn_readfirstlane(wave);
+        const uint32_t n_groups = (b - a) / TAIL_G;
+        s_lo = a + (uint32_t)(((uint64_t)n_groups * wv) / (TPB / 64)) * TAIL_G;
+        s_hi = a + (uint32_t)(((uint64_t)n_groups * (wv + 1)) / (TPB / 64)) * TAIL_G;
+    };
+    auto stream_window = [&](uint32_t pw) {
+        const uint2 rec = row_pieces[pw + lane];
+        const bool in = pw + (uint32_t)lane < s_hi;
+        d_q = in ? rec.x : 0u;
+        d_xs = in ? rec.y : 63u;
+    };
+    auto drain_stream = [&]() {
+#ifdef KNNCF_ABL_NODRAIN
+        return;
+#endif
+        for (uint32_t pw = s_lo; pw < s_hi; pw += 64) {
+            const uint32_t w_q = d_q, w_xs = d_xs;
+            const uint32_t n8 = min(64u, s_hi - pw);
+            if (pw + 64 < s_hi) stream_window(pw + 64);
+            tail_window(w_q, w_xs, n8);
+        }
+    };
+    const bool pipelined = !STREAM && any_tail && n_chunks == 1;
+    if (STREAM && any_tail) {
+        stream_share(0);
+        stream_window(s_lo);
+    }
     if (pipelined) {
         setup_a(0, 0);
         __syncthreads();
@@ -513,7 +704,17 @@
                 }
             }
         };
-        if (pipelined) {
+        if (STREAM && any_tail) {
+            drain_stream();
+            PH(4);
+            take_panel();
+            if (t0 + TCOLS < U) {
+                stream_share(tile_no + 1);
+                stream_window(s_lo);
+            }
+            __syncthreads();
+            PH(5);
+        } else if (pipelined) {
             use_tables(tile_no & 1);
             drain(false);
             PH(4);
@@ -524,7 +725,7 @@
             PH(5);
             if (more) setup_b((tile_no + 1) & 1);
             else p_lo = p_hi = 0;
-        } else if (any_tail) {
+        } else if (!STREAM && any_tail) {
             use_tables(0);
             for (int ch = 0; ch < n_chunks; ++ch) {
                 if (n_chunks > 1) {
@@ -543,7 +744,7 @@
                 PH(5);
             }
         }
-        if (!pipelined) take_panel();
+        if (!pipelined && !(STREAM && any_tail)) take_panel();
         PH(1);
         if (any_tail) {
 #pragma unroll
@@ -757,16 +958,16 @@
 }
 #endif
 
-template <class ST, bool JAC>
+template <class ST, bool JAC, bool STREAM>
 static void launch_tail_select_t(const TailArgs& T, const ST* S, bool s_by_user, int64_t lds, int32_t n_rows, const int32_t* d_row_user, const int32_t* d_row_srow,
                                  int32_t U, int32_t kk, float eps_opnd, float eps_rest, int32_t cap, int32_t* cand_idx, float* cand_approx,
                                  int32_t* cand_cnt, float* cand_eps, int32_t* grp_v0, float* grp_x, int32_t gcap, bool anticipate, hipStream_t st) {
-    const size_t smem = (size_t)TCOLS * 4 + (size_t)NBINS * 4 + (size_t)EMAX * 4 + 2 * ((size_t)EMAX * 12 + (size_t)PMAX * 2) + (2 * (TPB / 64) + 4 + 64) * 4;
+    const size_t smem = (size_t)TCOLS * 4 + (size_t)NBINS * 4 + (STREAM ? 0 : (size_t)EMAX * 4 + 2 * ((size_t)EMAX * 12 + (size_t)PMAX * 2)) + (2 * (TPB / 64) + 4 + 64) * 4;
     static PerDeviceState lds_state;
-    ensure_dynamic_lds(lds_state, (const void*)k_tail_select<ST, JAC>, smem);
+    ensure_dynamic_lds(lds_state, (const void*)k_tail_select<ST, JAC, STREAM>, smem);
     const char* sg = getenv("KNNCF_DEBUG_ANTICIPATE_SIGMA");
     const float ant_sigma = !anticipate ? -1.0f : sg ? (float)atof(sg) : 7.0f;
-    k_tail_select<ST, JAC><<<n_rows, TPB, smem, st>>>(S, s_by_user ? 1 : 0, lds, n_rows, d_row_user, d_row_srow, T, U, kk, eps_opnd, eps_rest, cap, cand_idx, cand_approx, cand_cnt, cand_eps, grp_v0, grp_x, gcap, ant_sigma);
+    k_tail_select<ST, JAC, STREAM><<<n_rows, TPB, smem, st>>>(S, s_by_user ? 1 : 0, lds, n_rows, d_row_user, d_row_srow, T, U, kk, eps_opnd, eps_rest, cap, cand_idx, cand_approx, cand_cnt, cand_eps, grp_v0, grp_x, gcap, ant_sigma);
     KN_HIP(hipGetLastError());
 #ifdef KNNCF_SELECT_PROFILE
     KN_HIP(hipStreamSynchronize(st));
@@ -777,7 +978,7 @@
 void launch_tail_select(const Train& tr, const int32_t* d_colmap, const TailEntries& te, bool has_tail, const void* S, bool s_by_user, bool s_fp16, int64_t lds,
                         int32_t n_rows, const int32_t* d_row_user, int32_t k, float eps_opnd, float eps_rest, int32_t cap,
                         int32_t* cand_idx, float* cand_approx, int32_t* cand_cnt, float* cand_eps, int32_t* grp_v0, float* grp_x,
-                        int32_t gcap, hipStream_t st, bool anticipate, const int32_t* d_row_srow) {
+                        int32_t gcap, hipStream_t st, bool anticipate, const int32_t* d_row_srow, const PieceStream* ps) {
     if (n_rows <= 0) return;
     KN_REQUIRE(gcap >= 1024 && gcap % 8 == 0, KNNCF_E_INVALID, "select: group store too small");
     const int32_t U = tr.U;
@@ -788,16 +989,32 @@
     has_tail = false;
 #endif
     KN_REQUIRE(!has_tail || (te.cnt && te.item && te.x && te.tail_abs && te.head_sq), KNNCF_E_STATE, "select: tail entry lists missing");
+    const bool stream = has_tail && ps && ps->pieces && ps->ptr;
+    KN_REQUIRE(!stream || tr.tile_stride - 1 <= MAXT, KNNCF_E_STATE, "select: piece stream beyond MAXT tiles");
+    KN_TRACE_DISPATCH("select stream=%d", stream ? 1 : 0);
     TailArgs T{tr.u_ptr.p, tr.s_col.p, tr.s_pre.p, d_colmap, tr.i_ptr.p, tr.it_pack.p, (uint32_t)(tr.n * 4), tr.it_tile.p, tr.tile_stride, has_tail ? 1 : 0,
-               te.cnt, te.item, te.x, te.tail_abs, te.head_sq, te.row_len};
+               te.cnt, te.item, te.x, te.tail_abs, te.head_sq, te.row_len,
+               stream ? ps->pieces : nullptr, stream ? ps->ptr : nullptr, stream ? ps->row_prow : nullptr};
+    KN_REQUIRE(!tr.jaccard || te.row_len != nullptr, KNNCF_E_STATE, "select: row lengths missing");
+#define KN_SELECT_LAUNCH(ST_, JAC_, STREAM_)                                                                                                 \
+    launch_tail_select_t<ST_, JAC_, STREAM_>(T, static_cast<const ST_*>(S), s_by_user, lds, n_rows, d_row_user, d_row_srow, U, kk, eps_opnd, \
+                                             eps_rest, cap, cand_idx, cand_approx, cand_cnt, cand_eps, grp_v0, grp_x, gcap, anticipate, st)
+#define KN_SELECT_LAUNCH_ST(JAC_, STREAM_)                       \
+    do {                                                         \
+        if (s_fp16) KN_SELECT_LAUNCH(_Float16, JAC_, STREAM_);   \
+        else KN_SELECT_LAUNCH(float, JAC_, STREAM_);             \
+    } while (0)
     if (tr.jaccard) {
-        KN_REQUIRE(te.row_len != nullptr, KNNCF_E_STATE, "select: row lengths missing");
-        if (s_fp16) launch_tail_select_t<_Float16, true>(T, static_cast<const _Float16*>(S), s_by_user, lds, n_rows, d_row_user, d_row_srow, U, kk, eps_opnd, eps_rest, cap, cand_idx, cand_approx, cand_cnt, cand_eps, grp_v0, grp_x, gcap, anticipate, st);
-        else launch_tail_select_t<float, true>(T, static_cast<const float*>(S), s_by_user, lds, n_rows, d_row_user, d_row_srow, U, kk, eps_opnd, eps_rest, cap, cand_idx, cand_approx, cand_cnt, cand_eps, grp_v0, grp_x, gcap, anticipate, st);
+        if (stream) KN_SELECT_LAUNCH_ST(true, true);
+        else KN_SELECT_LAUNCH_ST(true, false);
     } else {
-        if (s_fp16) launch_tail_select_t<_Float16, false>(T, static_cast<const _Float16*>(S), s_by_user, lds, n_rows, d_row_user, d_row_srow, U, kk, eps_opnd, eps_rest, cap, cand_idx, cand_approx, cand_cnt, cand_eps, grp_v0, grp_x, gcap, anticipate, st);
-        else launch_tail_select_t<float, false>(T, static_cast<const float*>(S), s_by_user, lds, n_rows, d_row_user, d_row_srow, U, kk, eps_opnd, eps_rest, cap, cand_idx, cand_approx, cand_cnt, cand_eps, grp_v0, grp_x, gcap, anticipate, st);
-    }
-}
-
-}
+        if (stream) KN_SELECT_LAUNCH_ST(false, true);
+        else KN_SELECT_LAUNCH_ST(false, false);
+    }
+#undef KN_SELECT_LAUNCH_ST
+#undef KN_SELECT_LAUNCH
+}
+
+int select_max_stream_tiles() { return MAXT; }
+
+}
```

Result: slower. 82.37 million (-3.9%).
